# yu-changqian/TorchSeg

Measured on AMD Instinct MI355X. Metric: training images/sec (1024x1024) BiSeNet-R18, higher is better.
Workload: dtype bf16

## Files before the change

include/tsg_hip.h:

```cpp
#ifndef TSG_HIP_H
#define TSG_HIP_H

#include <stddef.h>
#include <stdint.h>

#ifdef __cplusplus
extern "C" {
#endif

#define TSG_VERSION 100

enum { TSG_F32 = 0, TSG_BF16 = 1 };
enum { TSG_NCHW = 0, TSG_NHWC = 1 };
enum { TSG_I64 = 0, TSG_U8 = 1 };

#define TSG_E_DTYPE   (-1)
#define TSG_E_LAYOUT  (-2)
#define TSG_E_SHAPE   (-3)
#define TSG_E_ALIGN   (-4)
#define TSG_E_NULL    (-5)
#define TSG_E_WS      (-6)
#define TSG_E_COMM_LIB   (-7)
#define TSG_E_COMM_BASE  (-100)

int tsg_version(void);


int    tsg_bn_num_partials(int layout, int64_t N, int64_t C, int64_t HW);
size_t tsg_bn_partial_ws_bytes(int layout, int64_t N, int64_t C, int64_t HW);

int tsg_bn_stats(const void* x, int dtype, int layout,
                 int64_t N, int64_t C, int64_t HW,
                 float* partial, int* rows, void* stream);

int tsg_bn_collapse(const float* partial, int S, int64_t C, float* sums,
                    void* stream);
int tsg_bn_collapse_count(const float* partial, int S, int64_t C, float* msg, int64_t count, void* stream);


int tsg_bn_finalize(const float* partial, int S, int64_t C, double count,
                    const float* count_dev, float eps, float momentum,
                    const float* gamma, const float* beta,
                    float* running_mean, float* running_var,
                    int64_t* num_batches_tracked,
                    float* mean, float* invstd, float* fwd_pack, void* stream);

int tsg_bn_affine(const float* mean, const float* invstd, const float* gamma,
                  const float* beta, int64_t C, float* fwd_pack, void* stream);

int tsg_bn_apply_fwd(const void* x, const void* residual, void* y,
                     int dtype, int layout, int64_t N, int64_t C, int64_t HW,
                     const float* fwd_pack, int relu, void* stream);

int tsg_bn_bwd_reduce(const void* dy, const void* x, const void* y,
                      int dtype, int layout, int64_t N, int64_t C, int64_t HW,
                      const float* fwd_pack, int relu,
                      float* partial, int* rows, void* stream);

int tsg_bn_bwd_coeffs(const float* partial, int S, int64_t C, double count,
                      const float* count_dev, int batch_stats,
                      const float* invstd, const float* fwd_pack,
                      float* dgamma, float* dbeta, float* bwd_pack, void* stream);

int tsg_bn_bwd_apply(const void* dy, const void* x, const void* y,
                     void* dx, void* dres,
                     int dtype, int layout, int64_t N, int64_t C, int64_t HW,
                     const float* bwd_pack, int relu, void* stream);

int tsg_bn_maskbits_supported(int dtype, int layout, int64_t C, int64_t HW);
int tsg_bn_apply_fwd_maskbits(const void* x, const void* residual, void* y, void* bits, int dtype, int layout, int64_t N,
                              int64_t C, int64_t HW, const float* fwd_pack, void* stream);
int tsg_bn_bwd_reduce_maskbits(const void* dy, const void* x, const void* bits, int dtype, int layout, int64_t N, int64_t C,
                               int64_t HW, const float* fwd_pack, float* partial, int* rows, void* stream);
int tsg_bn_bwd_apply_maskbits(const void* dy, const void* x, const void* bits, void* dx, void* dres, int dtype, int layout,
                              int64_t N, int64_t C, int64_t HW, const float* bwd_pack, void* stream);

int tsg_bn_mixed_supported(int dtype, int64_t C, int64_t HW);
int tsg_bn_mixed_num_partials(int64_t N, int64_t C, int64_t HW);
int tsg_bn_apply_fwd_mixed(const void* x_nchw, void* y_nhwc, int dtype,
                           int64_t N, int64_t C, int64_t HW,
                           const float* fwd_pack, int relu, void* stream);
int tsg_bn_bwd_reduce_mixed(const void* dy_nhwc, const void* x_nchw, int dtype,
                            int64_t N, int64_t C, int64_t HW,
                            const float* fwd_pack, int relu,
                            float* partial, int* rows, void* stream);
int tsg_bn_bwd_apply_mixed(const void* dy_nhwc, const void* x_nchw, void* dx_nchw,
                           int dtype, int64_t N, int64_t C, int64_t HW,
                           const float* bwd_pack, int relu, void* stream);

size_t tsg_gap_ws_bytes(int layout, int64_t N, int64_t C, int64_t HW);
int tsg_gap_fwd(const void* x, void* out, int dtype, int layout,
                int64_t N, int64_t C, int64_t HW,
                void* ws, size_t ws_bytes, void* stream);
int tsg_gap_bwd(const void* dout, void* dx, int dtype, int layout,
                int64_t N, int64_t C, int64_t HW, void* stream);

size_t tsg_adaptive_avgpool_nhwc_ws_bytes(int dtype, int64_t N, int C, int H, int W, int OH, int OW);
int tsg_adaptive_avgpool_nhwc_fwd(const void* x, void* out, int dtype, int64_t N, int C, int H, int W, int OH, int OW,
                                  void* ws, size_t ws_bytes, void* stream);
int tsg_adaptive_avgpool_nhwc_bwd(const void* dout, void* dx, int dtype, int64_t N, int C, int H, int W, int OH, int OW,
                                  void* stream);

int tsg_cat2_rows(const void* a, const void* b, void* out, int64_t rows, int64_t row_bytes_a, int64_t row_bytes_b,
                  void* stream);

int tsg_chanscale_fwd(const void* x, const void* s, void* y, int dtype, int layout,
                      int64_t N, int64_t C, int64_t HW, int add_identity, void* stream);
int tsg_chanscale_bwd(const void* dy, const void* x, const void* s, void* dx, void* ds,
                      int dtype, int layout, int64_t N, int64_t C, int64_t HW,
                      int add_identity, void* ws, size_t ws_bytes, void* stream);
int tsg_chanscale_bwd_ds(const void* dy, const void* x, void* ds, int dtype, int layout, int64_t N, int64_t C, int64_t HW,
                         void* ws, size_t ws_bytes, void* stream);
int tsg_chanscale_bwd_dx(const void* dy, const void* s, const void* gadd, void* dx, int dtype, int layout, int64_t N, int64_t C,
                         int64_t HW, int add_identity, void* stream);

int tsg_maxpool_nhwc_fwd(const void* x, void* y, void* argmax_u8, int dtype,
                         int64_t N, int C, int IH, int IW, int OH, int OW,
                         int K, int S, int P, void* stream);
int tsg_maxpool_nhwc_bwd(const void* dy, const void* argmax_u8, void* dx, int dtype,
                         int64_t N, int C, int IH, int IW, int OH, int OW,
                         int K, int S, int P, void* stream);

int tsg_stem_conv_supported(int dtype, int Cin, int Cout, int kh, int kw, int stride, int pad,
                            int dilation, int groups, int64_t H, int64_t W);
size_t tsg_stem_conv_ws_bytes(void);
int tsg_stem_conv_fwd(const void* x, const float* w, void* y, int64_t B, int64_t H, int64_t W,
                      void* ws, size_t ws_bytes, void* stream);
int tsg_stem_conv_wrw(const void* x, const void* dy, float* dw, int64_t B, int64_t H, int64_t W,
                      void* ws, size_t ws_bytes, void* stream);
int tsg_stem3_conv_supported(int dtype, int Cin, int Cout, int kh, int kw, int stride, int pad,
                             int dilation, int groups, int64_t H, int64_t W);
size_t tsg_stem3_conv_ws_bytes(void);
int tsg_stem3_conv_fwd(const void* x, const float* w, void* y, int64_t B, int64_t H, int64_t W,
                       void* ws, size_t ws_bytes, void* stream);
int tsg_stem3_conv_wrw(const void* x, const void* dy, float* dw, int64_t B, int64_t H, int64_t W,
                       void* ws, size_t ws_bytes, void* stream);
int tsg_stem_conv_wrw_bn(const void* x, const void* da, const void* xc, const float* bp, float* dw, int64_t B,
                         int64_t H, int64_t W, void* ws, size_t ws_bytes, void* stream);
int tsg_stem_conv_stats_partials(int64_t B, int64_t H, int64_t W);
int tsg_stem_conv_fwd_stats(const void* x, const float* w, void* y, float* partial, int64_t B, int64_t H,
                            int64_t W, void* ws, size_t ws_bytes, void* stream);

int tsg_bn_relu_pool_fwd(const void* x, void* y, void* argmax_u8, int dtype, int64_t N, int C, int IH, int IW,
                         int OH, int OW, const float* fp, void* stream);
int tsg_bn_relu_pool_bwd_num_partials(int dtype, int64_t N, int C, int IH, int IW);
int tsg_bn_relu_pool_bwd_reduce(const void* dpool, const void* argmax_u8, const void* x, int dtype, int64_t N,
                                int C, int IH, int IW, int OH, int OW, const float* fp, float* partial,
                                void* stream);
int tsg_bn_relu_pool_bwd_apply(const void* dpool, const void* argmax_u8, const void* x, void* dx, int dtype,
                               int64_t N, int C, int IH, int IW, int OH, int OW, const float* bp, void* stream);

int tsg_stem_conv_stats(const void* x, const float* w, float* partial, int64_t B, int64_t H, int64_t W, void* ws,
                        size_t ws_bytes, void* stream);
int tsg_stem_conv_bn_relu_pool_fwd(const void* x, const float* w, const float* fp, void* ypool, void* argmax_u8,
                                   int64_t B, int64_t H, int64_t W, void* ws, size_t ws_bytes, void* stream);
int tsg_stem_pool_bwd_num_partials(int64_t B, int64_t H, int64_t W);
int tsg_stem_conv_bn_relu_pool_bwd_reduce(const void* x, const float* w, const void* dpool, const void* argmax_u8,
                                          const float* fp, float* partial, int64_t B, int64_t H, int64_t W, void* ws,
                                          size_t ws_bytes, void* stream);
int tsg_stem_conv_wrw_bn_pool(const void* x, const float* w, const void* xc, const void* dpool, const void* argmax_u8,
                              const float* bp, float* dw, int64_t B, int64_t H, int64_t W, void* ws, size_t ws_bytes,
                              void* stream);

int tsg_conv3x3_wrw_supported(int dtype, int Cin, int Cout, int kh, int kw, int stride, int pad,
                              int dilation, int groups);
size_t tsg_conv3x3_wrw_ws_bytes(void);
int tsg_conv3x3_wrw(const void* x, const void* dy, float* dw, int64_t B, int64_t H, int64_t W,
                    void* ws, size_t ws_bytes, void* stream);
int tsg_conv3x3_wrw_tr(const void* x, const void* dy, float* dw, int64_t B, int64_t H, int64_t W,
                       void* ws, size_t ws_bytes, void* stream);
int tsg_conv3x3_wrw_gen_supported(int dtype, int Cin, int Cout, int kh, int kw, int stride, int pad,
                                  int dilation, int groups);
size_t tsg_conv3x3_wrw_gen_ws_bytes(int64_t B, int64_t Hin, int64_t Win, int Cin, int Cout, int stride);
int tsg_conv3x3_wrw_gen(const void* x, const void* dy, float* dw, int64_t B, int64_t Hin, int64_t Win, int Cin, int Cout,
                        int stride, void* ws, size_t ws_bytes, void* stream);
int tsg_conv3x3_wrw_tr_norm(const void* x, const float* in_ab, const void* dy, float* dw, int64_t B, int64_t H, int64_t W,
                            void* ws, size_t ws_bytes, void* stream);
int tsg_conv3x3_wrw_gen_norm(const void* x, const float* in_ab, const void* dy, float* dw, int64_t B, int64_t Hin,
                             int64_t Win, int Cin, int Cout, int stride, void* ws, size_t ws_bytes, void* stream);

int tsg_conv3x3_c64_supported(int dtype, int Cin, int Cout, int kh, int kw, int stride, int pad, int dilation,
                              int groups);
int tsg_conv3x3_c64_stats_partials(int64_t B, int64_t H, int64_t W);
int tsg_conv3x3_c64_fwd(const void* x, const void* w, void* y, float* partial, const float* in_ab, const void* addend,
                        int64_t B, int64_t H, int64_t W, void* stream);
int tsg_conv3x3_c64_s2_stats_partials(int64_t B, int64_t H, int64_t W);
int tsg_conv3x3_c64_s2_fwd(const void* x, const void* w, void* y, float* partial, const float* in_ab, int64_t B,
                           int64_t H, int64_t W, void* stream);
int tsg_conv3x3_c64_s2_dgrad(const void* dy, const void* wt, void* dx, int64_t B, int64_t H, int64_t W,
                             void* stream);
int tsg_conv3x3_c64_dgrad_bnsums_partials(int64_t B, int64_t H, int64_t W);
int tsg_conv3x3_c64_dgrad_bnsums(const void* dy, const void* wt, void* dx, const void* bn_x, const float* bn_fp,
                                 float* partial, int64_t B, int64_t H, int64_t W, void* stream);
int tsg_conv3x3_c64_s2_dgrad_partials(int64_t B, int64_t H, int64_t W);
int tsg_conv3x3_c64_s2_dgrad_bnsums(const void* dy, const void* wt, void* dx, const void* bn_x, const float* bn_fp,
                                    float* partial, int64_t B, int64_t H, int64_t W, void* stream);

int tsg_conv3x3_weight_rot180_t(const void* w, int dtype, void* out, int O, int I, void* stream);

int tsg_conv3x3_gen_supported(int dtype, int Cin, int Cout, int kh, int kw, int stride, int pad, int dilation,
                              int groups);
int64_t tsg_conv3x3_gen_filter_elems(int Cin, int Cout);
int tsg_conv3x3_gen_tile(int64_t B, int64_t H, int64_t W, int Cin, int Cout);
int tsg_conv3x3_gen_prep_filter(const void* w, int dtype, void* out, int O, int I, int mode, int BN, void* stream);
int tsg_conv3x3_gen_stats_partials(int64_t B, int64_t H, int64_t W, int Cin, int Cout, int BN);
int tsg_conv3x3_gen_variant(int64_t B, int64_t H, int64_t W, int Cin, int Cout, int BN, int with_in_ab);
int tsg_conv3x3_s2_dgrad_supported(int dtype, int Cin, int Cout);
int tsg_conv3x3_s2_dgrad(const void* dy, const void* wf, void* dx, const void* addend, int64_t B, int64_t H, int64_t W,
                         int Cin, int Cout, void* stream);
int tsg_conv3x3_s2_dgrad_subadd(const void* dy, const void* wf, void* dx, const void* addend_sub, int64_t B, int64_t H,
                                int64_t W, int Cin, int Cout, void* stream);
int tsg_conv3x3_gen_fwd(const void* x, const void* wf, void* y, float* partial, const float* in_ab, const void* addend,
                        int64_t B, int64_t H, int64_t W, int Cin, int Cout, int BN, void* stream);

int tsg_conv3x3_dil_supported(int dtype, int Cin, int Cout, int kh, int kw, int stride, int pad, int dilation,
                              int groups);
int tsg_conv3x3_dil_stats_partials(int64_t B, int64_t H, int64_t W, int Cin, int Cout, int dilation);
int tsg_conv3x3_dil_fwd(const void* x, const void* wf, void* y, float* partial, const void* addend, int64_t B, int64_t H,
                        int64_t W, int Cin, int Cout, int dilation, void* stream);
size_t tsg_conv3x3_dil_wrw_ws_bytes(int64_t B, int64_t H, int64_t W, int Cin, int Cout, int dilation);
int tsg_conv3x3_dil_wrw(const void* x, const void* dy, float* dw, int64_t B, int64_t H, int64_t W, int Cin, int Cout,
                        int dilation, void* ws, size_t ws_bytes, void* stream);

int tsg_pw_wgrad_supported(int dtype, int Cin, int Cout, int64_t B, int H, int W, int stride);
int tsg_pw_wgrad_slices(int Cin, int Cout, int64_t B, int H, int W, int stride);
size_t tsg_pw_wgrad_ws_bytes(int Cin, int Cout, int64_t B, int H, int W, int stride);
int tsg_pw_wgrad(const void* x, const void* dy, float* dw, int dtype, int64_t B, int H, int W, int Cin, int Cout,
                 int stride, void* ws, size_t ws_bytes, void* stream);


typedef struct tsg_ohem_plan {
  int64_t P;
  int     C;
  int     grid;
  int     levels;
  int     shift[3];
  int     bins[3];
  uint32_t thresh_bits;
  size_t  ws_bytes;
} tsg_ohem_plan;

int tsg_ohem_make_plan(int64_t B, int C, int64_t HW, float thresh,
                       tsg_ohem_plan* plan);

int tsg_ohem_fwd(const void* logits, int dtype, const void* labels, int ltype,
                 int64_t B, int C, int64_t HW,
                 int64_t ignore_label, float thresh, int64_t min_kept,
                 const float* weight,
                 float* nll, float* lse, float* loss, int32_t* sel,
                 void* ws, size_t ws_bytes, void* stream);

int tsg_ohem_bwd(const void* logits, int dtype, const void* labels, int ltype,
                 int64_t B, int C, int64_t HW, int64_t ignore_label,
                 const float* weight,
                 const float* nll, const float* lse, const int32_t* sel,
                 const float* gscale, void* dlogits, void* ws, void* stream);

int tsg_ohem_up_supported(int C, int IH, int IW, int OH, int OW, float thresh);
size_t tsg_ohem_up_bwd_ws_bytes(int64_t B, int C, int IH, int OW);
int tsg_ohem_up_fwd(const void* z, int dtype, const void* labels, int ltype,
                    int64_t B, int C, int IH, int IW, int OH, int OW,
                    int64_t ignore_label, float thresh, int64_t min_kept,
                    const float* weight,
                    float* nll, float* lse, float* loss, int32_t* sel,
                    void* ws, size_t ws_bytes, void* stream);
int tsg_ohem_up_bwd(const void* z, int dtype, const void* labels, int ltype,
                    int64_t B, int C, int IH, int IW, int OH, int OW,
                    int64_t ignore_label, const float* weight,
                    const float* nll, const float* lse, const int32_t* sel,
                    const float* gscale, void* dz,
                    void* ws, size_t ws_bytes, void* stream);

int tsg_ohem_up_wide_supported(int C, int IH, int IW, int OH, int OW);

int tsg_ohem_target_prob(const float* nll, const void* labels, int ltype, int64_t P, int C,
                         int64_t ignore_label, float* prob, void* stream);

size_t tsg_kth_ws_bytes(int64_t n);
int tsg_kth_value(const float* v, int64_t n, int64_t k, float* out,
                  void* ws, size_t ws_bytes, void* stream);

size_t tsg_focal_ws_bytes(int64_t P);
int tsg_focal_fwd(const void* pred, int dtype, const void* target, int ltype,
                  int64_t P, int64_t ignore_label, float gamma, float alpha,
                  float* loss, void* ws, size_t ws_bytes, void* stream);
int tsg_focal_bwd(const void* pred, int dtype, const void* target, int ltype,
                  int64_t P, int64_t ignore_label, float gamma, float alpha,
                  const float* gscale, void* dpred, void* stream);

int tsg_upsample_bilinear_ac_fwd(const void* x, const void* add, void* y,
                                 int dtype, int64_t NC, int IH, int IW,
                                 int OH, int OW, void* stream);
int tsg_upsample_bilinear_ac_bwd(const void* dy, void* dx, int dtype,
                                 int64_t NC, int IH, int IW, int OH, int OW,
                                 void* stream);
int tsg_upsample_bilinear_ac_nhwc_fwd(const void* x, const void* add, void* y,
                                      int dtype, int64_t N, int C, int IH, int IW,
// ... 173 lines not shown
```

torchseg_amd/convwrw.py:

```python
import collections
import os as _os

import torch
import torch.nn as nn
import torch.nn.functional as F

from . import kernels as K
from . import syncbn as S
from .stemconv import StemConv2d, _as_bf16_image, _wants_bf16, attach_bn_partial, take_bn_partial

_OWN_C64 = _os.environ.get("TSG_CONV_C64", "1") != "0"
_OWN_C64_S1 = _os.environ.get("TSG_CONV_C64_S1", "1") != "0"
_C64_STATS = _os.environ.get("TSG_CONV_C64_STATS", "1") != "0"
_OWN_GEN = _os.environ.get("TSG_CONV_GEN", "1") != "0"
_GEN_STATS = _os.environ.get("TSG_CONV_GEN_STATS", "1") != "0"
_OWN_S2_DGRAD = _os.environ.get("TSG_CONV_S2_DGRAD", "1") != "0"
_DGRAD_MODE = _os.environ.get("TSG_CONV_DGRAD_FWD", "2").strip().lower()
_DGRAD_FWD = _DGRAD_MODE not in ("0", "false", "no", "off", "")
_DGRAD_ANY = _DGRAD_MODE == "2"

_BN_ON_LOAD = _os.environ.get("TSG_BN_ON_LOAD", "1") != "0"
_GEN_BN_ON_LOAD = _os.environ.get("TSG_CONV_GEN_BN_ON_LOAD", "0") == "1"
_STEM_BN_WRW = _os.environ.get("TSG_STEM_BN_WRW", "1") != "0"
_BN_BSUM = _os.environ.get("TSG_BN_BSUM", "0") == "1"
# ... 46 lines not shown
        return False
    return all(a == b for a, b, n in zip(out.stride(), param.stride(), out.shape) if n != 1)


_deferred = {}
_deferred_clear_queued = [False]


def _deferred_clear():
    _deferred_clear_queued[0] = False
    _deferred.clear()


def may_defer(param, buf):
    return (param is not None and param.is_leaf and param.grad is None and param.dtype == torch.float32
            and id(param) not in _wrw_pending and id(param) not in _deferred and not param._backward_hooks
            and not _foreign_grad_hooks(param) and _kept_as_gradient(buf, param))


def note_deferred(param, entry):
    _DEFER.append(entry)
    _deferred[id(param)] = entry
    if not _deferred_clear_queued[0]:
        _deferred_clear_queued[0] = True
        from torch.autograd import Variable
        try:
            Variable._execution_engine.queue_callback(_deferred_clear)
        except RuntimeError:
            _deferred_clear()


def launch_deferred_of(param):
    if param is None or id(param) not in _deferred:
        return False
    entry, _deferred[id(param)] = _deferred[id(param)], None
    if entry is not None:
        if _DEFER is not None:
            _DEFER[:] = [e for e in _DEFER if e is not entry]
        entry[0]()
    return True


def wrw_on_side_stream(fn, param, *operands, defer_out=None):
    if _DEFER is not None and defer_out is not None:
        Cout, Cin = defer_out
        buf = torch.empty((Cout, Cin, 3, 3), dtype=torch.float32, device=operands[0].device, memory_format=torch.channels_last)
        if may_defer(param, buf):
            note_deferred(param, (lambda: fn(out=buf), operands, buf))
            return buf.detach()
        if launch_deferred_of(param):
            return fn()
    if not _WRW_STREAM or not operands[0].is_cuda or param is None or not param.is_leaf or param.grad is not None \
            or param.dtype != torch.float32 or param._backward_hooks or _foreign_grad_hooks(param) \
            or (torch.cuda.is_current_stream_capturing() and not _WRW_IN_GRAPH):
        if _wrw_side and operands[0].is_cuda:
            dev = operands[0].device
            side = _wrw_side.get(dev)
            if side is not None and (param is None or id(param) in _wrw_pending):
                torch.cuda.current_stream(dev).wait_stream(side)
        return fn()
    dev = operands[0].device
    cur = torch.cuda.current_stream(dev)
    if id(param) in _wrw_pending:
        side = _wrw_side.get(dev)
        if side is not None:
            cur.wait_stream(side)
        return fn()
    side = _wrw_side.get(dev)
    if side is None:
        side = _wrw_side[dev] = torch.cuda.Stream(device=dev)
    side.wait_stream(cur)
    with torch.cuda.stream(side):
        out = fn()
    for t in operands:
        if t is not None:
            t.record_stream(side)
    out.record_stream(cur)
    _wrw_pending.add(id(param))
    if not _kept_as_gradient(out, param):
        cur.wait_stream(side)
    if not _wrw_join_queued[0]:
        _wrw_join_queued[0] = True
        from torch.autograd import Variable
        try:
            Variable._execution_engine.queue_callback(_wrw_join)
        except RuntimeError:
            _wrw_join()
    return out


def _conv_wrw(x, dy, stride, param, in_ab=None):
    operands = (x, dy) if in_ab is None else (x, dy, in_ab)
    return wrw_on_side_stream(lambda out=None: K.provider().conv3x3_wrw(x, dy, stride=stride, in_ab=in_ab, out=out), param,
                              *operands, defer_out=(dy.shape[1], x.shape[1]))


def _bf16_nhwc(t):
    if t.dtype != torch.bfloat16:
        t = t.to(torch.bfloat16)
    return t.contiguous(memory_format=torch.channels_last)


def _filters(weight):
    if _SHADOW and weight.is_contiguous(memory_format=torch.channels_last):
        from .shadow import bank
        return bank.get(weight, want_rot=True)
    return weight.detach().to(torch.bfloat16), None


def _rotated(wrt, wb):
    return wrt if wrt is not None else K.provider().conv3x3_weight_rot180_t(wb)


def _with_partial(y, partial):
    if partial.numel():
        attach_bn_partial(y, partial)
    return y


def _skip_addend(dskip, like_shape):
    if dskip is None or tuple(dskip.shape) != tuple(like_shape):
        return None
    return _bf16_nhwc(dskip)


Route = collections.namedtuple("Route", "family stats skip compact bn_on_load dgrad_fwd")


def _route(conv, xb, general=True):
    kp = K.provider()
    stride, geom = conv.stride[0], (conv.padding[0], conv.dilation[0], conv.groups)
    if not kp.conv3x3_wrw_supported(xb, conv.weight, stride, *geom):
        return None
    nhwc = conv.weight.is_contiguous(memory_format=torch.channels_last)
    c64 = _OWN_C64 and kp.conv3x3_c64_supported(xb, conv.weight, stride, *geom)
    if (general and _OWN_GEN and stride == 1 and not (c64 and _OWN_C64_S1) and nhwc
            and kp.conv3x3_gen_supported(xb, conv.weight, 1, *geom)):
        family, stats, skip = "gen", _GEN_STATS, True
    else:
        if c64 and nhwc:
            family = "c64"
        elif _OWN_S2_DGRAD and stride == 2 and nhwc and kp.conv3x3_s2_dgrad_supported(conv.in_channels, conv.out_channels):
            family = "s2"
        else:
            family = "lib"
        stats = _C64_STATS and family == "c64"
        skip = family == "s2" or (c64 and _OWN_C64_S1 and stride == 1)
    return Route(family, bool(stats and conv.training), bool(skip), family == "s2",
                 (family == "c64" and (_OWN_C64_S1 or stride == 2))
                 or (family == "gen" and _GEN_BN_ON_LOAD and conv.in_channels <= 512),
                 family == "lib" and _DGRAD_FWD and stride == 1 and (_DGRAD_ANY or conv.in_channels == conv.out_channels))


class _ConvWrwFn(torch.autograd.Function):

    @staticmethod
    def forward(ctx, x, weight, wb, wrt, stride, route, skip=False):
        kp = K.provider()
        partial = x.new_empty(0, dtype=torch.float32)
        if route.stats:
            y, partial = kp.conv3x3_c64_fwd(x, wb, with_stats=True, stride=stride)
        elif route.family == "c64":
            y = kp.conv3x3_c64_fwd(x, wb, stride=stride)
        else:
            y = F.conv2d(x, wb, None, stride, 1)
        ctx.route, ctx.stride = route, stride
        ctx.wrt = wrt
        ctx.master = weight if (route.family == "s2" and _SHADOW and weight.dtype == torch.float32) else None
        ctx.save_for_backward(x, wb)
        ctx.wparam = weight
        ctx.need_dx = x.requires_grad
        ctx.set_materialize_grads(False)
        ctx.mark_non_differentiable(partial)
        ctx.skip_sub = skip == 2
        if not skip:
            return y, partial
        return y, partial, (x[:, :, ::2, ::2].contiguous(memory_format=torch.channels_last) if ctx.skip_sub else x)

    @staticmethod
    def backward(ctx, dy, _dpartial, dskip=None):
        kp = K.provider()
        x, wb = ctx.saved_tensors
        family, stride = ctx.route.family, ctx.stride
        sub = None
        if dskip is not None and ctx.skip_sub:
            sub, dskip = _bf16_nhwc(dskip), None
        if dy is None:
            if sub is not None:
                dskip = torch.zeros_like(x)
                dskip[:, :, ::2, ::2] = sub
            return dskip, None, None, None, None, None, None
        dy = _bf16_nhwc(dy)
        dx = None
        if ctx.need_dx:
            in_hw = (x.shape[2], x.shape[3])
            add = _skip_addend(dskip, x.shape) if (family == "s2" or (family == "c64" and stride == 1)) else None
            if add is not None:
                dskip = None
            if family == "s2":
                dx = kp.conv3x3_s2_dgrad(dy, wb if ctx.master is None else ctx.master, in_hw, addend=add, addend_sub=sub)
                sub = None
            elif family == "c64" and stride == 2:
                dx = kp.conv3x3_c64_s2_dgrad(dy, _rotated(ctx.wrt, wb), in_hw)
            elif family == "c64":
                dx = kp.conv3x3_c64_fwd(dy, _rotated(ctx.wrt, wb), addend=add)
            elif ctx.route.dgrad_fwd:
                dx = F.conv2d(dy, _rotated(ctx.wrt, wb), None, 1, 1)
            else:
                dx = torch.ops.aten.convolution_backward(dy, x, wb, None, [stride, stride], [1, 1], [1, 1], False, [0, 0], 1,
                                                         [True, False, False])[0]
            if dskip is not None:
                dx = dx + dskip.to(dx.dtype)
            if sub is not None:
                dx[:, :, ::2, ::2] += sub.to(dx.dtype)
        dw = _conv_wrw(x, dy, stride, ctx.wparam)
        return dx, dw.to(ctx.wparam.dtype), None, None, None, None, None


class _ConvGenFn(torch.autograd.Function):

    @staticmethod
    def forward(ctx, x, weight, with_stats, skip=False):
        kp = K.provider()
        wf = kp.conv3x3_gen_prep_filter(weight, 0, x)
        out = kp.conv3x3_gen_fwd(x, wf, weight.shape[0], with_stats=with_stats)
        y, partial = out if with_stats else (out, x.new_empty(0, dtype=torch.float32))
        ctx.save_for_backward(x, weight)
        ctx.need_dx = x.requires_grad
        ctx.mark_non_differentiable(partial)
        ctx.set_materialize_grads(False)
        return (y, partial, x) if skip else (y, partial)

    @staticmethod
    def backward(ctx, dy, _dpartial, dskip=None):
        kp = K.provider()
        x, weight = ctx.saved_tensors
        if dy is None:
            return dskip, None, None, None
        dy = _bf16_nhwc(dy)
        dx = None
        if ctx.need_dx:
            O, I = weight.shape[0], weight.shape[1]
            if O % 16 == 0 and I % 64 == 0:
                add = _skip_addend(dskip, x.shape)
                dx = kp.conv3x3_gen_fwd(dy, kp.conv3x3_gen_prep_filter(weight, 1, dy), I, addend=add)
                if add is not None:
                    dskip = None
            else:
                dx = F.conv2d(dy, kp.conv3x3_weight_rot180_t(weight.detach().to(torch.bfloat16)), None, 1, 1)
            if dskip is not None:
                dx = dx + dskip.to(dx.dtype)
        dw = _conv_wrw(x, dy, 1, weight)
        return dx, dw.to(weight.dtype), None, None


class WrwConv2d(nn.Conv2d):
    def forward(self, x):
        return self._forward(x, False)

    def _forward(self, x, want_skip):
        route = None
        if (x.is_cuda and self.bias is None and self.weight.dtype == torch.float32 and x.dim() == 4
                and self.padding_mode == "zeros" and torch.is_grad_enabled() and self.weight.requires_grad and _wants_bf16(x)):
            xb = _bf16_nhwc(x)
            route = _route(self, xb)
        if route is None:
            y = super().forward(x)
            return (y, None) if want_skip else y
        skip = bool(want_skip and route.skip and xb is x and x.requires_grad)
        with torch.autocast("cuda", enabled=False):
            if route.family == "gen":
                out = _ConvGenFn.apply(xb, self.weight, route.stats, skip)
            else:
                wb, wrt = _filters(self.weight)
                out = _ConvWrwFn.apply(xb, self.weight, wb, wrt, self.stride[0], route,
                                       2 if (skip and want_skip == 2 and route.compact) else skip)
        y = _with_partial(out[0], out[1])
        return (y, out[2] if skip else None) if want_skip else y


def conv_with_skip(conv, x, subsample=False):
    if _FUSE_SKIP and isinstance(conv, WrwConv2d) and conv.stride in ((1, 1), (2, 2)) and isinstance(x, torch.Tensor) \
            and x.is_cuda and torch.is_grad_enabled():
        return conv._forward(x, 2 if (subsample and _SKIP_SUB and conv.stride == (2, 2)) else True)
    return conv(x), None


def _c64_dgrad_and_bn_sums(kp, dy, rot, x, fp, stride, layout, N, C, HW):
    if _BN_BSUM and kp.conv3x3_c64_bnsums_supported(x.shape[0], x.shape[2], x.shape[3], stride):
        if stride == 2:
            da, partial = kp.conv3x3_c64_s2_dgrad(dy, rot, (x.shape[2], x.shape[3]), bsum=(x, fp))
        else:
            da, partial = kp.conv3x3_c64_fwd(dy, rot, bsum=(x, fp))
        return da, partial, partial.shape[0]
    da = kp.conv3x3_c64_s2_dgrad(dy, rot, (x.shape[2], x.shape[3])) if stride == 2 else kp.conv3x3_c64_fwd(dy, rot)
    partial, Sn = kp.bn_bwd_reduce(da, x, None, layout, N, C, HW, fp, True)
    return da, partial, Sn


def _c64_fwd_on_load(kp, x, wb, stride, fp, out_stats):
    if out_stats:
        return kp.conv3x3_c64_fwd(x, wb, with_stats=True, stride=stride, in_ab=fp)
    return kp.conv3x3_c64_fwd(x, wb, stride=stride, in_ab=fp), x.new_empty(0, dtype=torch.float32)


class _BnReluConvFn(torch.autograd.Function):

    @staticmethod
    def forward(ctx, x, gamma, beta, bn, use_batch_stats, group, hint, weight, wb, stride, wrt, gen=False, out_stats=False):
        kp = K.provider()
        layout, N, C, HW = K.bn_layout(x)
        invstd, fp, count_dev, world = S._forward_pack(kp, x, layout, N, C, HW, bn, gamma, beta, use_batch_stats, group, hint)
        if gen:
            out = kp.conv3x3_gen_fwd(x, kp.conv3x3_gen_prep_filter(weight, 0, x), weight.shape[0], with_stats=out_stats,
                                     in_ab=fp)
            y, partial = out if out_stats else (out, x.new_empty(0, dtype=torch.float32))
        else:
            y, partial = _c64_fwd_on_load(kp, x, wb, stride, fp, out_stats)
        ctx.save_for_backward(x, weight if gen else wb, gamma, beta, invstd, fp, count_dev)
        ctx.wparam = weight
        ctx.cfg = (layout, N, C, HW, use_batch_stats, group, world, stride, gen)
        ctx.wrt = wrt
        ctx.mark_non_differentiable(partial)
        return y, partial

    @staticmethod
    def backward(ctx, dy, _dpartial):
        kp = K.provider()
        x, wb, gamma, beta, invstd, fp, count_dev = ctx.saved_tensors
        layout, N, C, HW, use_batch_stats, group, world, stride, gen = ctx.cfg
# ... 105 lines not shown
```

torchseg_amd/csrc/bn.hip:

```cpp
#include "tsg_dispatch.h"

namespace tsg {

constexpr int kThreads = 256;
constexpr int kUnroll = 4;
constexpr int kTargetBlocks = 2048;
constexpr int kTargetBlocksNhwc = 1024;
constexpr int kMaxSplit = 256;

template <typename T, int V> struct Pack;
template <> struct Pack<float, 4> : Vec<float> {};
template <> struct Pack<bf16_t, 8> : Vec<bf16_t> {};
template <typename T> struct Pack<T, 1> {
  float v[1];
  typedef T Raw;
  static __device__ __forceinline__ Raw ldraw(const T* p) { return *p; }
  static __device__ __forceinline__ Raw ldraw_dead(const T* p) { return *p; }
  __device__ __forceinline__ void unpack(const Raw& t) { v[0] = ld1<T>(&t); }
  __device__ __forceinline__ void load(const T* p) { v[0] = ld1<T>(p); }
  __device__ __forceinline__ void store(T* p) const { st1<T>(p, v[0]); }
};

struct NchwGeom {
  int seg;
// ... 113 lines not shown
            a2[j] = fma((AT)pd.v[j], (AT)(px.v[j] - mu), a2[j]);
          }
        }
      }
    }
  }
  AT s1 = 0, s2 = 0;
#pragma unroll
  for (int j = 0; j < V; ++j) { s1 += a1[j]; s2 += a2[j]; }
  block_sum2(s1, s2, sm);
  if (tid == 0) {
    put_partial(partial, C, S, s, 0, c, s1);
    put_partial(partial, C, S, s, 1, c, s2);
  }
}

template <typename T, int V, int MODE, int MASK>
__global__ __launch_bounds__(kThreads) void bn_reduce_nhwc(
    const T* __restrict__ x, const T* __restrict__ dy, const T* __restrict__ y,
    int64_t M, int64_t C, int GT, int R, int64_t rows_per_block,
    const float* __restrict__ fp, float* __restrict__ partial) {
  typedef typename RedAcc<T, MODE>::type AT;
  extern __shared__ __attribute__((aligned(16))) float smem[];
  const int tid = threadIdx.x;
  const int gl = tid % GT, r = tid / GT;
  const int64_t G = C / V;
  const int64_t g = (int64_t)blockIdx.y * GT + gl;
  const bool live = (r < R) && (g < G);
  const int64_t c0 = g * V;
  float mu[V], ca[V], cb[V];
  AT a1[V], a2[V];
#pragma unroll
  for (int j = 0; j < V; ++j) { a1[j] = 0; a2[j] = 0; mu[j] = 0.f; ca[j] = 0.f; cb[j] = 0.f; }
  if (MODE == 1 && live) {
    ldc<V>(fp + 2 * C, c0, mu);
    if (MASK == 2) { ldc<V>(fp, c0, ca); ldc<V>(fp + C, c0, cb); }
  }
  const int64_t row0 = (int64_t)blockIdx.x * rows_per_block;
  int64_t row1 = row0 + rows_per_block;
  if (row1 > M) row1 = M;
  if (live) {
    typedef typename Pack<T, V>::Raw Raw;
    auto accumulate = [&](const Raw& rx, const Raw& rd, const Raw& ry, unsigned int mb) {
      Pack<T, V> px;
      px.unpack(rx);
      if (MODE == 0) {
#pragma unroll
        for (int j = 0; j < V; ++j) { const AT xv = px.v[j]; a1[j] += xv; a2[j] = fma(xv, xv, a2[j]); }
      } else {
        Pack<T, V> pd;
        pd.unpack(rd);
        if (MASK == 1) {
          Pack<T, V> py;
          py.unpack(ry);
#pragma unroll
          for (int j = 0; j < V; ++j) pd.v[j] = py.v[j] > 0.f ? pd.v[j] : 0.f;
        } else if (MASK == 2) {
#pragma unroll
          for (int j = 0; j < V; ++j) pd.v[j] = fmaf(px.v[j], ca[j], cb[j]) > 0.f ? pd.v[j] : 0.f;
        } else if (MASK == 3) {
#pragma unroll
          for (int j = 0; j < V; ++j) pd.v[j] = ((mb >> j) & 1u) ? pd.v[j] : 0.f;
        }
#pragma unroll
        for (int j = 0; j < V; ++j) {
          a1[j] += (AT)pd.v[j];
          a2[j] = fma((AT)pd.v[j], (AT)(px.v[j] - mu[j]), a2[j]);
        }
      }
    };
    const unsigned char* bits = reinterpret_cast<const unsigned char*>(y);
    int64_t row = row0 + r;
    for (; row + (int64_t)(kUnroll - 1) * R < row1; row += (int64_t)kUnroll * R) {
      Raw rx[kUnroll], rd[kUnroll], ry[kUnroll];
      unsigned int rb[kUnroll];
#pragma unroll
      for (int k = 0; k < kUnroll; ++k) {
        const int64_t off = (row + (int64_t)k * R) * C + c0;
        rx[k] = Pack<T, V>::ldraw(x + off);
        if (MODE == 1) rd[k] = Pack<T, V>::ldraw(dy + off);
        if (MODE == 1 && MASK == 1) ry[k] = Pack<T, V>::ldraw(y + off);
        rb[k] = (MODE == 1 && MASK == 3) ? bits[off / V] : 0u;
      }
#pragma unroll
      for (int k = 0; k < kUnroll; ++k) accumulate(rx[k], rd[k], ry[k], rb[k]);
    }
    for (; row < row1; row += R) {
      const int64_t off = row * C + c0;
      Raw rx = Pack<T, V>::ldraw(x + off), rd = rx, ry = rx;
      if (MODE == 1) rd = Pack<T, V>::ldraw(dy + off);
      if (MODE == 1 && MASK == 1) ry = Pack<T, V>::ldraw(y + off);
      accumulate(rx, rd, ry, (MODE == 1 && MASK == 3) ? bits[off / V] : 0u);
    }
  }
  const int W = GT * V;
  AT* s1 = reinterpret_cast<AT*>(smem);
  AT* s2 = s1 + (size_t)R * W;
  if (r < R) {
#pragma unroll
    for (int j = 0; j < V; ++j) {
      s1[r * W + gl * V + j] = a1[j];
      s2[r * W + gl * V + j] = a2[j];
    }
  }
  __syncthreads();
  for (int t = tid; t < W; t += kThreads) {
    const int64_t c = (int64_t)blockIdx.y * W + t;
    if (c < C) {
      AT t1 = 0, t2 = 0;
      for (int q = 0; q < R; ++q) { t1 += s1[q * W + t]; t2 += s2[q * W + t]; }
      put_partial(partial, C, (int)gridDim.x, (int)blockIdx.x, 0, c, t1);
      put_partial(partial, C, (int)gridDim.x, (int)blockIdx.x, 1, c, t2);
    }
  }
}

static int bn_reverse() {
  static int v = -1;
  if (v < 0) { const char* e = getenv("TSG_BN_REVERSE"); v = e ? (e[0] != '0') : 0; }
  return v;
}

template <typename T, int V, bool RELU, bool RES>
__global__ __launch_bounds__(kThreads) void bn_fwd_nchw(
    const T* __restrict__ x, const T* __restrict__ res, T* __restrict__ y,
    int64_t C, int64_t HW, int seg, int segs, const float* __restrict__ fp) {
  const int64_t bid = blockIdx.x;
  const int64_t plane = bid / segs;
  const int sg = (int)(bid - plane * segs);
  const int64_t c = plane % C;
  const float a = fp[c], b = fp[C + c];
  const int64_t off = plane * HW + (int64_t)sg * seg;
  const int64_t rem = HW - (int64_t)sg * seg;
  const int len = rem < seg ? (int)rem : seg;
#pragma unroll
  for (int k = 0; k < kUnroll; ++k) {
    const int i = (k * kThreads + threadIdx.x) * V;
    if (i < len) {
      Pack<T, V> px, pr;
      px.load(x + off + i);
      if (RES) pr.load(res + off + i);
#pragma unroll
      for (int j = 0; j < V; ++j) {
        float t = fmaf(px.v[j], a, b);
        if (RES) t += pr.v[j];
        if (RELU) t = t > 0.f ? t : 0.f;
        px.v[j] = t;
      }
      px.store(y + off + i);
    }
  }
}

template <typename T, int V, bool RELU, bool RES, bool BITS = false>
__global__ __launch_bounds__(kThreads) void bn_fwd_nhwc(
    const T* __restrict__ x, const T* __restrict__ res, T* __restrict__ y,
    int64_t M, int64_t C, int GT, int R, int64_t rows_per_block, const float* __restrict__ fp, int rev,
    unsigned char* __restrict__ bits = nullptr) {
  const int tid = threadIdx.x;
  const int gl = tid % GT, r = tid / GT;
  const int64_t g = (int64_t)blockIdx.y * GT + gl;
  if (r >= R || g >= C / V) return;
  const int64_t c0 = g * V;
  float a[V], b[V];
  ldc<V>(fp, c0, a);
  ldc<V>(fp + C, c0, b);
  const int64_t row0 = (int64_t)(rev ? gridDim.x - 1 - blockIdx.x : blockIdx.x) * rows_per_block;
  int64_t row1 = row0 + rows_per_block;
  if (row1 > M) row1 = M;
  typedef typename Pack<T, V>::Raw Raw;
  auto finish = [&](const Raw& rx, const Raw& rr_, int64_t off) {
    Pack<T, V> px, pr;
    px.unpack(rx);
    if (RES) pr.unpack(rr_);
#pragma unroll
    for (int j = 0; j < V; ++j) {
      float t = fmaf(px.v[j], a[j], b[j]);
      if (RES) t += pr.v[j];
      if (RELU) t = t > 0.f ? t : 0.f;
      px.v[j] = t;
    }
    px.store(y + off);
    if (BITS) {
      unsigned int mb = 0u;
#pragma unroll
      for (int j = 0; j < V; ++j) {
        const float q = sizeof(T) == 2 ? __uint_as_float((uint32_t)f32_to_bf16(px.v[j]) << 16) : px.v[j];
        mb |= (q > 0.f ? 1u : 0u) << j;
      }
      bits[off / V] = (unsigned char)mb;
    }
  };
  int64_t row = row0 + r;
  for (; row + (int64_t)(kUnroll - 1) * R < row1; row += (int64_t)kUnroll * R) {
    Raw rx[kUnroll], rs[kUnroll];
#pragma unroll
    for (int k = 0; k < kUnroll; ++k) {
      const int64_t off = (row + (int64_t)k * R) * C + c0;
      rx[k] = Pack<T, V>::ldraw_dead(x + off);
      if (RES) rs[k] = Pack<T, V>::ldraw(res + off);
    }
#pragma unroll
    for (int k = 0; k < kUnroll; ++k) finish(rx[k], rs[k], (row + (int64_t)k * R) * C + c0);
  }
  for (; row < row1; row += R) {
    const int64_t off = row * C + c0;
    Raw rx = Pack<T, V>::ldraw_dead(x + off), rs = rx;
    if (RES) rs = Pack<T, V>::ldraw(res + off);
    finish(rx, rs, off);
  }
}

template <typename T, int V, int MASK, bool DRES>
__global__ __launch_bounds__(kThreads) void bn_bwd_nchw(
    const T* __restrict__ dy, const T* __restrict__ x, const T* __restrict__ y,
    T* __restrict__ dx, T* __restrict__ dres,
    int64_t C, int64_t HW, int seg, int segs, const float* __restrict__ bp) {
  const int64_t bid = blockIdx.x;
  const int64_t plane = bid / segs;
  const int sg = (int)(bid - plane * segs);
  const int64_t c = plane % C;
  const float a = bp[c], b = bp[C + c], mu = bp[2 * C + c], bc = bp[3 * C + c], c2 = bp[4 * C + c];
  const int64_t off = plane * HW + (int64_t)sg * seg;
  const int64_t rem = HW - (int64_t)sg * seg;
  const int len = rem < seg ? (int)rem : seg;
#pragma unroll
  for (int k = 0; k < kUnroll; ++k) {
    const int i = (k * kThreads + threadIdx.x) * V;
    if (i < len) {
      Pack<T, V> pd, px;
      pd.load(dy + off + i);
      px.load(x + off + i);
      if (MASK == 1) {
        Pack<T, V> py;
        py.load(y + off + i);
#pragma unroll
        for (int j = 0; j < V; ++j) pd.v[j] = py.v[j] > 0.f ? pd.v[j] : 0.f;
      } else if (MASK == 2) {
#pragma unroll
        for (int j = 0; j < V; ++j) pd.v[j] = fmaf(px.v[j], a, b) > 0.f ? pd.v[j] : 0.f;
      }
      if (DRES) pd.store(dres + off + i);
#pragma unroll
      for (int j = 0; j < V; ++j) px.v[j] = fmaf(a, pd.v[j], fmaf(bc, px.v[j] - mu, c2));
      px.store(dx + off + i);
    }
  }
}

template <typename T, int V, int MASK, bool DRES>
__global__ __launch_bounds__(kThreads) void bn_bwd_nhwc(
    const T* __restrict__ dy, const T* __restrict__ x, const T* __restrict__ y,
    T* __restrict__ dx, T* __restrict__ dres,
    int64_t M, int64_t C, int GT, int R, int64_t rows_per_block, const float* __restrict__ bp, int rev) {
  const int tid = threadIdx.x;
  const int gl = tid % GT, r = tid / GT;
  const int64_t g = (int64_t)blockIdx.y * GT + gl;
  if (r >= R || g >= C / V) return;
  const int64_t c0 = g * V;
  float a[V], b[V], mu[V], bc[V], c2[V];
#pragma unroll
  for (int j = 0; j < V; ++j) b[j] = 0.f;
  ldc<V>(bp, c0, a);
  if (MASK == 2) ldc<V>(bp + C, c0, b);
  ldc<V>(bp + 2 * C, c0, mu);
  ldc<V>(bp + 3 * C, c0, bc);
  ldc<V>(bp + 4 * C, c0, c2);
  const int64_t row0 = (int64_t)(rev ? gridDim.x - 1 - blockIdx.x : blockIdx.x) * rows_per_block;
  int64_t row1 = row0 + rows_per_block;
  if (row1 > M) row1 = M;
  typedef typename Pack<T, V>::Raw Raw;
  auto finish = [&](const Raw& rd, const Raw& rx, const Raw& ry, unsigned int mb, int64_t off) {
    Pack<T, V> pd, px;
    pd.unpack(rd);
    px.unpack(rx);
    if (MASK == 1) {
      Pack<T, V> py;
      py.unpack(ry);
#pragma unroll
      for (int j = 0; j < V; ++j) pd.v[j] = py.v[j] > 0.f ? pd.v[j] : 0.f;
    } else if (MASK == 2) {
#pragma unroll
      for (int j = 0; j < V; ++j) pd.v[j] = fmaf(px.v[j], a[j], b[j]) > 0.f ? pd.v[j] : 0.f;
    } else if (MASK == 3) {
#pragma unroll
      for (int j = 0; j < V; ++j) pd.v[j] = ((mb >> j) & 1u) ? pd.v[j] : 0.f;
    }
    if (DRES) pd.store(dres + off);
#pragma unroll
    for (int j = 0; j < V; ++j) px.v[j] = fmaf(a[j], pd.v[j], fmaf(bc[j], px.v[j] - mu[j], c2[j]));
    px.store(dx + off);
  };
  const unsigned char* bits = reinterpret_cast<const unsigned char*>(y);
  int64_t row = row0 + r;
  for (; row + (int64_t)(kUnroll - 1) * R < row1; row += (int64_t)kUnroll * R) {
    Raw rd[kUnroll], rx[kUnroll], ry[kUnroll];
    unsigned int rb[kUnroll];
#pragma unroll
    for (int k = 0; k < kUnroll; ++k) {
      const int64_t off = (row + (int64_t)k * R) * C + c0;
      rd[k] = Pack<T, V>::ldraw_dead(dy + off);
      rx[k] = Pack<T, V>::ldraw_dead(x + off);
      if (MASK == 1) ry[k] = Pack<T, V>::ldraw(y + off);
      rb[k] = MASK == 3 ? bits[off / V] : 0u;
    }
#pragma unroll
    for (int k = 0; k < kUnroll; ++k) finish(rd[k], rx[k], ry[k], rb[k], (row + (int64_t)k * R) * C + c0);
  }
  for (; row < row1; row += R) {
    const int64_t off = row * C + c0;
    Raw rd = Pack<T, V>::ldraw_dead(dy + off), rx = Pack<T, V>::ldraw_dead(x + off), ry = rx;
    if (MASK == 1) ry = Pack<T, V>::ldraw(y + off);
    finish(rd, rx, ry, MASK == 3 ? bits[off / V] : 0u, off);
  }
}

constexpr int kTP = 64;

template <typename T, bool RELU>
__global__ __launch_bounds__(kThreads) void bn_fwd_mixed(
    const T* __restrict__ x, T* __restrict__ y, int64_t C, int64_t HW, int tiles_per_img,
    const float* __restrict__ fp) {
  constexpr int V = Pack<T, (sizeof(T) == 2 ? 8 : 4)>::N;
  extern __shared__ __attribute__((aligned(16))) float tile[];
  const int ldt = (int)C + 1;
  const int64_t n = blockIdx.x / tiles_per_img;
  const int64_t p0 = (int64_t)(blockIdx.x % tiles_per_img) * kTP;
  const int npx = (HW - p0) < kTP ? (int)(HW - p0) : kTP;
  const int tid = threadIdx.x;
  const int vpr = kTP / V;
  for (int it = tid; it < (int)C * vpr; it += kThreads) {
    const int c = it / vpr, v = it - c * vpr;
    const int p = v * V;
    if (p < npx) {
      Pack<T, V> px;
// ... 158 lines not shown
  if (owner) {
#pragma unroll
    for (int q = 0; q < 8; ++q) { t1 += sh[0][q * 8][tc]; t2 += sh[1][q * 8][tc]; }
  }
}

__device__ __forceinline__ double bn_count(double count, const float* cd) {
  return cd ? (double)cd[0] * 4096.0 + (double)cd[1] : count;
}

__global__ __launch_bounds__(kTc * kTs) void bn_collapse_k(const float* __restrict__ partial, int S,
                                                          int64_t C, float* __restrict__ sums, int with_count,
                                                          float count_hi, float count_lo) {
  if (with_count && blockIdx.x == 0 && threadIdx.x == 0) {
    sums[2 * C] = count_hi;
    sums[2 * C + 1] = count_lo;
  }
  double t1, t2; bool owner; int64_t c;
  tail_sums(partial, S, C, t1, t2, owner, c);
  if (!owner) return;
  sums[c] = (float)t1;
  sums[C + c] = (float)t2;
}

__global__ __launch_bounds__(kTc * kTs) void bn_finalize_k(
    const float* __restrict__ partial, int S, int64_t C, double count,
    const float* __restrict__ count_dev, float eps, float momentum,
    const float* __restrict__ gamma, const float* __restrict__ beta,
    float* __restrict__ rmean, float* __restrict__ rvar, int64_t* __restrict__ nbt,
    float* __restrict__ mean, float* __restrict__ invstd, float* __restrict__ fp) {
  if (blockIdx.x == 0 && threadIdx.x == 0 && nbt) *nbt += 1;
  double t1, t2; bool owner; int64_t c;
  tail_sums(partial, S, C, t1, t2, owner, c);
  if (!owner) return;
  count = bn_count(count, count_dev);
  const double m = t1 / count;
  double sumvar = t2 - t1 * m;
  if (sumvar < 0.0) sumvar = 0.0;
  const double bias_var = sumvar / count;
  const float mf = (float)m;
  const float isf = (float)(1.0 / sqrt(bias_var + (double)eps));
  mean[c] = mf;
  invstd[c] = isf;
  const float a = (gamma ? gamma[c] : 1.f) * isf;
  fp[c] = a;
  fp[C + c] = fmaf(-mf, a, beta ? beta[c] : 0.f);
  fp[2 * C + c] = mf;
  if (rmean) rmean[c] = (float)((1.0 - (double)momentum) * (double)rmean[c] + (double)momentum * m);
  if (rvar) {
    const double unbias = sumvar / (count - 1.0);
    rvar[c] = (float)((1.0 - (double)momentum) * (double)rvar[c] + (double)momentum * unbias);
  }
}

__global__ void bn_affine_k(const float* __restrict__ mean, const float* __restrict__ invstd,
                            const float* __restrict__ gamma, const float* __restrict__ beta, int64_t C,
                            float* __restrict__ fp) {
  const int64_t c = (int64_t)blockIdx.x * blockDim.x + threadIdx.x;
  if (c >= C) return;
  const float a = (gamma ? gamma[c] : 1.f) * invstd[c];
  fp[c] = a;
  fp[C + c] = fmaf(-mean[c], a, beta ? beta[c] : 0.f);
  fp[2 * C + c] = mean[c];
}

__global__ __launch_bounds__(kTc * kTs) void bn_bwd_coeffs_k(
    const float* __restrict__ partial, int S, int64_t C, double count,
    const float* __restrict__ count_dev, int batch_stats, const float* __restrict__ invstd,
    const float* __restrict__ fp, float* __restrict__ dgamma, float* __restrict__ dbeta,
    float* __restrict__ bp) {
  double t1, t2; bool owner; int64_t c;
  tail_sums(partial, S, C, t1, t2, owner, c);
  if (!owner) return;
  const double is = (double)invstd[c];
  if (dbeta) dbeta[c] = (float)t1;
  if (dgamma) dgamma[c] = (float)(t2 * is);
  if (bp) {
    const float a = fp[c];
    float bc = 0.f, c2 = 0.f;
    if (batch_stats) {
      count = bn_count(count, count_dev);
      const double k0 = t1 / count, k1 = t2 * is / count;
      bc = (float)(-(double)a * k1 * is);
      c2 = (float)(-(double)a * k0);
    }
    bp[c] = a;
    bp[C + c] = fp[C + c];
    bp[2 * C + c] = fp[2 * C + c];
    bp[3 * C + c] = bc;
    bp[4 * C + c] = c2;
  }
}

template <typename T, int V, int MODE>
static int launch_reduce(const T* x, const T* dy, const T* y, int layout, int64_t N,
                         int64_t C, int64_t HW, const float* fp, int mask,
                         float* partial, hipStream_t st) {
  return with_int<0, 1, 2>(MODE == 0 ? 0 : mask, [&](auto mk) {
    if (layout == TSG_NCHW) {
      NchwGeom g = nchw_geom(N, C, HW, V);
      dim3 grid((unsigned)C, (unsigned)g.split);
      hipLaunchKernelGGL((bn_reduce_nchw<T, V, MODE, mk()>), grid, dim3(kThreads), 0, st, x, dy, y, N, C, HW, g.seg, g.segs,
                         g.split, fp, partial);
    } else {
      const int64_t M = N * HW;
      NhwcGeom g = nhwc_geom(M, C, V);
      dim3 grid((unsigned)g.split, (unsigned)g.ytiles);
      const size_t sh = (size_t)2 * g.rows_per_iter * g.gt * V * sizeof(typename RedAcc<T, MODE>::type);
      hipLaunchKernelGGL((bn_reduce_nhwc<T, V, MODE, mk()>), grid, dim3(kThreads), sh, st, x, dy, y, M, C, g.gt,
                         g.rows_per_iter, g.rows_per_block, fp, partial);
    }
    TSG_CHECK_LAUNCH();
    return 0;
  });
}

template <typename T, int V>
static int launch_fwd(const T* x, const T* res, T* y, int layout, int64_t N, int64_t C,
                      int64_t HW, const float* fp, int relu, hipStream_t st) {
  return with_flag(relu != 0, [&](auto r) { return with_flag(res != nullptr, [&](auto s) {
    if (layout == TSG_NCHW) {
      NchwGeom g = nchw_geom(N, C, HW, V);
      const int64_t blocks = N * C * g.segs;
      if (blocks > 0x7fffffffLL) return TSG_E_SHAPE;
      hipLaunchKernelGGL((bn_fwd_nchw<T, V, r(), s()>), dim3((unsigned)blocks), dim3(kThreads), 0, st, x, res, y, C, HW,
                         g.seg, g.segs, fp);
    } else {
      const int64_t M = N * HW;
      NhwcGeom g = nhwc_geom(M, C, V);
      dim3 grid((unsigned)g.split, (unsigned)g.ytiles);
      hipLaunchKernelGGL((bn_fwd_nhwc<T, V, r(), s()>), grid, dim3(kThreads), 0, st, x, res, y, M, C, g.gt, g.rows_per_iter,
                         g.rows_per_block, fp, bn_reverse());
    }
    TSG_CHECK_LAUNCH();
    return 0;
  }); });
}

template <typename T, int V>
static int launch_fwd_bits(const T* x, const T* res, T* y, unsigned char* bits, int64_t N, int64_t C, int64_t HW,
                           const float* fp, hipStream_t st) {
  const int64_t M = N * HW;
  NhwcGeom g = nhwc_geom(M, C, V);
  dim3 grid((unsigned)g.split, (unsigned)g.ytiles);
  return with_flag(res != nullptr, [&](auto s) {
    hipLaunchKernelGGL((bn_fwd_nhwc<T, V, true, s(), true>), grid, dim3(kThreads), 0, st, x, res, y, M, C, g.gt,
                       g.rows_per_iter, g.rows_per_block, fp, bn_reverse(), bits);
    TSG_CHECK_LAUNCH();
    return 0;
  });
}

template <typename T, int V>
static int launch_reduce_bits(const T* x, const T* dy, const unsigned char* bits, int64_t N, int64_t C, int64_t HW,
                              const float* fp, float* partial, hipStream_t st) {
  const int64_t M = N * HW;
  NhwcGeom g = nhwc_geom(M, C, V);
  dim3 grid((unsigned)g.split, (unsigned)g.ytiles);
  const size_t sh = (size_t)2 * g.rows_per_iter * g.gt * V * sizeof(typename RedAcc<T, 1>::type);
  hipLaunchKernelGGL((bn_reduce_nhwc<T, V, 1, 3>), grid, dim3(kThreads), sh, st, x, dy, reinterpret_cast<const T*>(bits), M, C,
                     g.gt, g.rows_per_iter, g.rows_per_block, fp, partial);
  TSG_CHECK_LAUNCH();
  return 0;
}

template <typename T, int V>
static int launch_bwd_bits(const T* dy, const T* x, const unsigned char* bits, T* dx, T* dres, int64_t N, int64_t C,
                           int64_t HW, const float* bp, hipStream_t st) {
  const int64_t M = N * HW;
  NhwcGeom g = nhwc_geom(M, C, V);
  dim3 grid((unsigned)g.split, (unsigned)g.ytiles);
  return with_flag(dres != nullptr, [&](auto d) {
    hipLaunchKernelGGL((bn_bwd_nhwc<T, V, 3, d()>), grid, dim3(kThreads), 0, st, dy, x, reinterpret_cast<const T*>(bits), dx,
                       dres, M, C, g.gt, g.rows_per_iter, g.rows_per_block, bp, bn_reverse());
    TSG_CHECK_LAUNCH();
    return 0;
  });
}

template <typename T, int V>
static int launch_bwd(const T* dy, const T* x, const T* y, T* dx, T* dres, int layout,
                      int64_t N, int64_t C, int64_t HW, const float* bp, int mask, hipStream_t st) {
  return with_int<0, 1, 2>(mask, [&](auto mk) { return with_flag(dres != nullptr, [&](auto d) {
    if (layout == TSG_NCHW) {
      NchwGeom g = nchw_geom(N, C, HW, V);
      const int64_t blocks = N * C * g.segs;
      if (blocks > 0x7fffffffLL) return TSG_E_SHAPE;
      hipLaunchKernelGGL((bn_bwd_nchw<T, V, mk(), d()>), dim3((unsigned)blocks), dim3(kThreads), 0, st, dy, x, y, dx, dres, C,
                         HW, g.seg, g.segs, bp);
    } else {
      const int64_t M = N * HW;
      NhwcGeom g = nhwc_geom(M, C, V);
      dim3 grid((unsigned)g.split, (unsigned)g.ytiles);
      hipLaunchKernelGGL((bn_bwd_nhwc<T, V, mk(), d()>), grid, dim3(kThreads), 0, st, dy, x, y, dx, dres, M, C, g.gt,
                         g.rows_per_iter, g.rows_per_block, bp, bn_reverse());
    }
    TSG_CHECK_LAUNCH();
    return 0;
  }); });
}

static int check_dims(int dtype, int layout, int64_t N, int64_t C, int64_t HW) {
  if (dtype != TSG_F32 && dtype != TSG_BF16) return TSG_E_DTYPE;
  if (layout != TSG_NCHW && layout != TSG_NHWC) return TSG_E_LAYOUT;
  if (N <= 0 || C <= 0 || HW <= 0) return TSG_E_SHAPE;
  return 0;
}

static int partial_rows(int layout, int64_t N, int64_t C, int64_t HW, int V) {
  return layout == TSG_NCHW ? nchw_geom(N, C, HW, V).split : nhwc_geom(N * HW, C, V).split;
}

static int bn_reduce_dispatch(int mode, const void* x, const void* dy, const void* y,
                              int dtype, int layout, int64_t N, int64_t C, int64_t HW,
                              const float* fp, int mask, float* partial, void* stream, int* rows) {
  int e = check_dims(dtype, layout, N, C, HW);
  if (e) return e;
  if (!x || !partial) return TSG_E_NULL;
  hipStream_t st = (hipStream_t)stream;
  const int V = pick_vec(dtype, layout, C, HW, x, dy, mask == 1 ? y : nullptr, nullptr, nullptr);
  *rows = partial_rows(layout, N, C, HW, V) * (dtype == TSG_F32 ? 2 : 1);
  return with_elem_vec(dtype, V != 1, [&](auto t, auto v) {
    typedef typename decltype(t)::type T;
    return mode == 0 ? launch_reduce<T, v(), 0>((const T*)x, nullptr, nullptr, layout, N, C, HW, fp, 0, partial, st)
                     : launch_reduce<T, v(), 1>((const T*)x, (const T*)dy, (const T*)y, layout, N, C, HW, fp, mask, partial, st);
  });
}

}

using namespace tsg;

extern "C" {

int tsg_bn_num_partials(int layout, int64_t N, int64_t C, int64_t HW) {
  if (N <= 0 || C <= 0 || HW <= 0) return TSG_E_SHAPE;
  if (layout != TSG_NCHW && layout != TSG_NHWC) return TSG_E_LAYOUT;
  int best = 1;
  const int vs[3] = {1, 4, 8};
  for (int i = 0; i < 3; ++i) {
    const int V = vs[i];
    if (layout == TSG_NHWC && C % V) continue;
    const int s = partial_rows(layout, N, C, HW, V);
    if (s > best) best = s;
  }
  return 2 * best;
}

size_t tsg_bn_partial_ws_bytes(int layout, int64_t N, int64_t C, int64_t HW) {
  const int s = tsg_bn_num_partials(layout, N, C, HW);
  if (s < 0) return 0;
  return (size_t)s * 2 * (size_t)C * sizeof(float);
}

int tsg_bn_stats(const void* x, int dtype, int layout, int64_t N, int64_t C, int64_t HW,
                 float* partial, int* rows, void* stream) {
  int r = 0;
  int e = bn_reduce_dispatch(0, x, nullptr, nullptr, dtype, layout, N, C, HW, nullptr, 0, partial,
                             stream, &r);
  if (rows) *rows = r;
  return e;
}

int tsg_bn_collapse(const float* partial, int S, int64_t C, float* sums, void* stream) {
  if (!partial || !sums) return TSG_E_NULL;
  if (S <= 0 || C <= 0) return TSG_E_SHAPE;
  hipLaunchKernelGGL(bn_collapse_k, dim3(ceil_div_i(C, kTc)), dim3(kTc * kTs), 0, (hipStream_t)stream,
                     partial, S, C, sums, 0, 0.f, 0.f);
  TSG_CHECK_LAUNCH();
  return 0;
}

int tsg_bn_collapse_count(const float* partial, int S, int64_t C, float* msg, int64_t count, void* stream) {
  if (!partial || !msg) return TSG_E_NULL;
  if (S <= 0 || C <= 0 || count < 0) return TSG_E_SHAPE;
  hipLaunchKernelGGL(bn_collapse_k, dim3(ceil_div_i(C, kTc)), dim3(kTc * kTs), 0, (hipStream_t)stream,
                     partial, S, C, msg, 1, (float)(count / 4096), (float)(count % 4096));
  TSG_CHECK_LAUNCH();
  return 0;
}

int tsg_bn_finalize(const float* partial, int S, int64_t C, double count, const float* count_dev,
                    float eps, float momentum, const float* gamma, const float* beta,
                    float* running_mean, float* running_var, int64_t* num_batches_tracked,
                    float* mean, float* invstd, float* fwd_pack, void* stream) {
  if (!partial || !mean || !invstd || !fwd_pack) return TSG_E_NULL;
  if (S <= 0 || C <= 0 || (!count_dev && !(count > 0.0))) return TSG_E_SHAPE;
  hipLaunchKernelGGL(bn_finalize_k, dim3(ceil_div_i(C, kTc)), dim3(kTc * kTs), 0, (hipStream_t)stream,
                     partial, S, C, count, count_dev, eps, momentum, gamma, beta, running_mean,
                     running_var, num_batches_tracked, mean, invstd, fwd_pack);
  TSG_CHECK_LAUNCH();
  return 0;
}

int tsg_bn_affine(const float* mean, const float* invstd, const float* gamma, const float* beta,
                  int64_t C, float* fwd_pack, void* stream) {
  if (!mean || !invstd || !fwd_pack) return TSG_E_NULL;
  if (C <= 0) return TSG_E_SHAPE;
  hipLaunchKernelGGL(bn_affine_k, dim3(ceil_div_i(C, 128)), dim3(128), 0, (hipStream_t)stream, mean,
                     invstd, gamma, beta, C, fwd_pack);
  TSG_CHECK_LAUNCH();
  return 0;
}

int tsg_bn_apply_fwd(const void* x, const void* residual, void* y, int dtype, int layout,
                     int64_t N, int64_t C, int64_t HW, const float* fwd_pack, int relu,
                     void* stream) {
  int e = check_dims(dtype, layout, N, C, HW);
  if (e) return e;
  if (!x || !y || !fwd_pack) return TSG_E_NULL;
  if (!aligned16(fwd_pack)) return TSG_E_ALIGN;
  hipStream_t st = (hipStream_t)stream;
  const int V = pick_vec(dtype, layout, C, HW, x, residual, y, nullptr, nullptr);
  return with_elem_vec(dtype, V != 1, [&](auto t, auto v) {
    typedef typename decltype(t)::type T;
    return launch_fwd<T, v()>((const T*)x, (const T*)residual, (T*)y, layout, N, C, HW, fwd_pack, relu, st);
  });
}

int tsg_bn_bwd_reduce(const void* dy, const void* x, const void* y, int dtype, int layout,
                      int64_t N, int64_t C, int64_t HW, const float* fwd_pack, int relu,
                      float* partial, int* rows, void* stream) {
  if (!dy || !fwd_pack) return TSG_E_NULL;
  if (!aligned16(fwd_pack)) return TSG_E_ALIGN;
  const int mask = relu ? (y ? 1 : 2) : 0;
  int r = 0;
  int e = bn_reduce_dispatch(1, x, dy, y, dtype, layout, N, C, HW, fwd_pack, mask, partial, stream, &r);
  if (rows) *rows = r;
  return e;
}

int tsg_bn_bwd_coeffs(const float* partial, int S, int64_t C, double count, const float* count_dev,
                      int batch_stats, const float* invstd, const float* fwd_pack, float* dgamma,
                      float* dbeta, float* bwd_pack, void* stream) {
  if (!partial || !invstd || (bwd_pack && !fwd_pack)) return TSG_E_NULL;
  if (S <= 0 || C <= 0 || (bwd_pack && batch_stats && !count_dev && !(count > 0.0))) return TSG_E_SHAPE;
  hipLaunchKernelGGL(bn_bwd_coeffs_k, dim3(ceil_div_i(C, kTc)), dim3(kTc * kTs), 0, (hipStream_t)stream,
                     partial, S, C, count, count_dev, batch_stats, invstd, fwd_pack, dgamma, dbeta, bwd_pack);
  TSG_CHECK_LAUNCH();
  return 0;
}

int tsg_bn_bwd_apply(const void* dy, const void* x, const void* y, void* dx, void* dres,
                     int dtype, int layout, int64_t N, int64_t C, int64_t HW,
                     const float* bwd_pack, int relu, void* stream) {
  int e = check_dims(dtype, layout, N, C, HW);
  if (e) return e;
  if (!dy || !x || !dx || !bwd_pack) return TSG_E_NULL;
  if (!aligned16(bwd_pack)) return TSG_E_ALIGN;
  hipStream_t st = (hipStream_t)stream;
  const int mask = relu ? (y ? 1 : 2) : 0;
  const int V = pick_vec(dtype, layout, C, HW, x, dy, mask == 1 ? y : nullptr, dx, dres);
  return with_elem_vec(dtype, V != 1, [&](auto t, auto v) {
    typedef typename decltype(t)::type T;
    return launch_bwd<T, v()>((const T*)dy, (const T*)x, (const T*)y, (T*)dx, (T*)dres, layout, N, C, HW, bwd_pack, mask, st);
  });
}

static int bits_vec(int dtype, int layout, int64_t C, int64_t HW, const void* a, const void* b, const void* c, const void* d,
                    const void* e) {
  if (layout != TSG_NHWC) return 0;
  const int want = dtype == TSG_BF16 ? 8 : dtype == TSG_F32 ? 4 : 0;
  if (!want || C % want) return 0;
  return pick_vec(dtype, layout, C, HW, a, b, c, d, e) == want ? want : 0;
}

int tsg_bn_maskbits_supported(int dtype, int layout, int64_t C, int64_t HW) {
  return bits_vec(dtype, layout, C, HW, nullptr, nullptr, nullptr, nullptr, nullptr) != 0;
}

int tsg_bn_apply_fwd_maskbits(const void* x, const void* residual, void* y, void* bits, int dtype, int layout, int64_t N,
                              int64_t C, int64_t HW, const float* fwd_pack, void* stream) {
  int e = check_dims(dtype, layout, N, C, HW);
  if (e) return e;
  if (!x || !y || !bits || !fwd_pack) return TSG_E_NULL;
  if (!aligned16(fwd_pack)) return TSG_E_ALIGN;
  const int V = bits_vec(dtype, layout, C, HW, x, residual, y, nullptr, nullptr);
  if (!V) return layout != TSG_NHWC ? TSG_E_LAYOUT : TSG_E_ALIGN;
  hipStream_t st = (hipStream_t)stream;
  if (dtype == TSG_F32)
    return launch_fwd_bits<float, 4>((const float*)x, (const float*)residual, (float*)y, (unsigned char*)bits, N, C, HW, fwd_pack, st);
  return launch_fwd_bits<bf16_t, 8>((const bf16_t*)x, (const bf16_t*)residual, (bf16_t*)y, (unsigned char*)bits, N, C, HW, fwd_pack, st);
}

int tsg_bn_bwd_reduce_maskbits(const void* dy, const void* x, const void* bits, int dtype, int layout, int64_t N, int64_t C,
                               int64_t HW, const float* fwd_pack, float* partial, int* rows, void* stream) {
  int e = check_dims(dtype, layout, N, C, HW);
  if (e) return e;
  if (!dy || !x || !bits || !fwd_pack || !partial) return TSG_E_NULL;
  if (!aligned16(fwd_pack)) return TSG_E_ALIGN;
  const int V = bits_vec(dtype, layout, C, HW, x, dy, nullptr, nullptr, nullptr);
  if (!V) return layout != TSG_NHWC ? TSG_E_LAYOUT : TSG_E_ALIGN;
  if (rows) *rows = partial_rows(layout, N, C, HW, V) * (dtype == TSG_F32 ? 2 : 1);
  hipStream_t st = (hipStream_t)stream;
  if (dtype == TSG_F32)
    return launch_reduce_bits<float, 4>((const float*)x, (const float*)dy, (const unsigned char*)bits, N, C, HW, fwd_pack, partial, st);
  return launch_reduce_bits<bf16_t, 8>((const bf16_t*)x, (const bf16_t*)dy, (const unsigned char*)bits, N, C, HW, fwd_pack, partial, st);
}

int tsg_bn_bwd_apply_maskbits(const void* dy, const void* x, const void* bits, void* dx, void* dres, int dtype, int layout,
                              int64_t N, int64_t C, int64_t HW, const float* bwd_pack, void* stream) {
  int e = check_dims(dtype, layout, N, C, HW);
  if (e) return e;
  if (!dy || !x || !bits || !dx || !bwd_pack) return TSG_E_NULL;
  if (!aligned16(bwd_pack)) return TSG_E_ALIGN;
  const int V = bits_vec(dtype, layout, C, HW, x, dy, nullptr, dx, dres);
  if (!V) return layout != TSG_NHWC ? TSG_E_LAYOUT : TSG_E_ALIGN;
  hipStream_t st = (hipStream_t)stream;
  if (dtype == TSG_F32)
    return launch_bwd_bits<float, 4>((const float*)dy, (const float*)x, (const unsigned char*)bits, (float*)dx, (float*)dres, N, C, HW, bwd_pack, st);
  return launch_bwd_bits<bf16_t, 8>((const bf16_t*)dy, (const bf16_t*)x, (const unsigned char*)bits, (bf16_t*)dx, (bf16_t*)dres, N, C, HW, bwd_pack, st);
}

static int mixed_ok(int dtype, int64_t C, int64_t HW) {
  const int V = native_vec(dtype);
  return (dtype == TSG_F32 || dtype == TSG_BF16) && C % 8 == 0 && C <= 128 && HW % V == 0;
}

int tsg_bn_mixed_supported(int dtype, int64_t C, int64_t HW) { return mixed_ok(dtype, C, HW); }

static int mixed_blocks(int64_t N, int64_t HW) {
  int64_t t = N * ((HW + kTP - 1) / kTP);
  if (t > kTargetBlocksNhwc) t = kTargetBlocksNhwc;
  return (int)(t < 1 ? 1 : t);
}

int tsg_bn_mixed_num_partials(int64_t N, int64_t C, int64_t HW) {
  if (N <= 0 || C <= 0 || HW <= 0) return TSG_E_SHAPE;
  return mixed_blocks(N, HW);
}

int tsg_bn_apply_fwd_mixed(const void* x_nchw, void* y_nhwc, int dtype, int64_t N, int64_t C,
                           int64_t HW, const float* fwd_pack, int relu, void* stream) {
  if (!x_nchw || !y_nhwc || !fwd_pack) return TSG_E_NULL;
  if (N <= 0 || !mixed_ok(dtype, C, HW)) return TSG_E_SHAPE;
  if (!aligned16(x_nchw) || !aligned16(y_nhwc)) return TSG_E_ALIGN;
  const int tpi = (int)((HW + kTP - 1) / kTP);
  const size_t sh = (size_t)kTP * (C + 1) * sizeof(float);
  dim3 grid((unsigned)(N * tpi));
  hipStream_t st = (hipStream_t)stream;
  return with_elem(dtype, [&](auto t) { return with_flag(relu != 0, [&](auto r) {
    typedef typename decltype(t)::type T;
    hipLaunchKernelGGL((bn_fwd_mixed<T, r()>), grid, dim3(kThreads), sh, st, (const T*)x_nchw, (T*)y_nhwc, C, HW, tpi, fwd_pack);
    TSG_CHECK_LAUNCH();
    return 0;
  }); });
}

int tsg_bn_bwd_reduce_mixed(const void* dy_nhwc, const void* x_nchw, int dtype, int64_t N, int64_t C,
                            int64_t HW, const float* fwd_pack, int relu, float* partial, int* rows,
                            void* stream) {
  if (!dy_nhwc || !x_nchw || !fwd_pack || !partial) return TSG_E_NULL;
  if (N <= 0 || !mixed_ok(dtype, C, HW)) return TSG_E_SHAPE;
  if (!aligned16(x_nchw) || !aligned16(dy_nhwc)) return TSG_E_ALIGN;
  const int tpi = (int)((HW + kTP - 1) / kTP);
  const int64_t total = N * tpi;
  const int V = native_vec(dtype);
  size_t sh = (size_t)kTP * (C + 1) * sizeof(float);
  const size_t red = (size_t)2 * C * (kTP / V) * sizeof(float);
  if (red > sh) sh = red;
  const int blocks = mixed_blocks(N, HW);
  if (rows) *rows = blocks;
  hipStream_t st = (hipStream_t)stream;
  const int items = (int)((C * (kTP / V) + kThreads - 1) / kThreads);
  const int ipt = items <= 1 ? 1 : items <= 2 ? 2 : items <= 4 ? 4 : 8;
  return with_elem(dtype, [&](auto t) { return with_flag(relu != 0, [&](auto r) { return with_int<1, 2, 4, 8>(ipt, [&](auto i) {
    typedef typename decltype(t)::type T;
    hipLaunchKernelGGL((bn_bwd_reduce_mixed<T, r(), i()>), dim3(blocks), dim3(kThreads), sh, st, (const T*)dy_nhwc,
                       (const T*)x_nchw, C, HW, tpi, total, fwd_pack, partial);
    TSG_CHECK_LAUNCH();
    return 0;
  }); }); });
}

int tsg_bn_bwd_apply_mixed(const void* dy_nhwc, const void* x_nchw, void* dx_nchw, int dtype, int64_t N,
                           int64_t C, int64_t HW, const float* bwd_pack, int relu, void* stream) {
  if (!dy_nhwc || !x_nchw || !dx_nchw || !bwd_pack) return TSG_E_NULL;
  if (N <= 0 || !mixed_ok(dtype, C, HW)) return TSG_E_SHAPE;
  if (!aligned16(x_nchw) || !aligned16(dy_nhwc) || !aligned16(dx_nchw)) return TSG_E_ALIGN;
  const int tpi = (int)((HW + kTP - 1) / kTP);
  const size_t sh = (size_t)kTP * (C + 1) * sizeof(float);
  dim3 grid((unsigned)(N * tpi));
  hipStream_t st = (hipStream_t)stream;
  return with_elem(dtype, [&](auto t) { return with_flag(relu != 0, [&](auto r) {
    typedef typename decltype(t)::type T;
    hipLaunchKernelGGL((bn_bwd_apply_mixed<T, r()>), grid, dim3(kThreads), sh, st, (const T*)dy_nhwc, (const T*)x_nchw,
                       (T*)dx_nchw, C, HW, tpi, bwd_pack);
    TSG_CHECK_LAUNCH();
    return 0;
  }); });
}

}
```

torchseg_amd/csrc/bnpool.hip:

```cpp
#include "tsg_dispatch.h"

namespace tsg {

constexpr int kBpT = 256;

template <typename T> __device__ __forceinline__ float round_as(float v);
template <> __device__ __forceinline__ float round_as<float>(float v) { return v; }
template <> __device__ __forceinline__ float round_as<bf16_t>(float v) { return bf16_to_f32(f32_to_bf16(v)); }

struct BpMap { int GT, PW; };
static BpMap bp_map(int C, int V) {
  BpMap m;
  const int G = C / V;
  m.GT = G < kBpT ? G : kBpT;
  m.PW = kBpT / m.GT;
  return m;
}
constexpr int kFwdRows = 8;
constexpr int kAppRows = 8;

template <typename T>
__device__ __forceinline__ void pool_row(const T* __restrict__ xn, int iy, int IH, int x0, int IW, int C,
                                         const float (&a)[Vec<T>::N], const float (&b)[Vec<T>::N],
                                         float (&rm)[Vec<T>::N], int (&rk)[Vec<T>::N]) {
  constexpr int V = Vec<T>::N;
  const bool row_ok = iy >= 0 && iy < IH;
  const int iyc = iy < 0 ? 0 : (iy >= IH ? IH - 1 : iy);
  const T* row = xn + (int64_t)iyc * IW * C;
  Vec<T> p[3];
  bool ok[3];
#pragma unroll
  for (int kx = 0; kx < 3; ++kx) {
    const int ix = x0 + kx;
    ok[kx] = row_ok && ix >= 0 && ix < IW;
    const int ixc = ix < 0 ? 0 : (ix >= IW ? IW - 1 : ix);
    p[kx].load(row + (int64_t)ixc * C);
  }
#pragma unroll
  for (int j = 0; j < V; ++j) { rm[j] = -1.f; rk[j] = 0; }
#pragma unroll
  for (int kx = 0; kx < 3; ++kx) {
#pragma unroll
    for (int j = 0; j < V; ++j) {
      float v = fmaxf(fmaf(p[kx].v[j], a[j], b[j]), 0.f);
      v = ok[kx] ? v : -1.f;
      if (v > rm[j]) { rm[j] = v; rk[j] = kx; }
    }
  }
}

template <typename T>
__global__ __launch_bounds__(kBpT) void bn_relu_pool_fwd_k(const T* __restrict__ x, T* __restrict__ y,
                                                           uint8_t* __restrict__ idx, int C, int IH, int IW,
                                                           int OH, int OW, int GT, int PW, int ytiles,
                                                           const float* __restrict__ fp) {
  constexpr int V = Vec<T>::N;
  const int tid = threadIdx.x;
  const int gl = tid % GT, pl = tid / GT;
  const int g = (blockIdx.y % ytiles) * GT + gl;
  const int ox = blockIdx.x * PW + pl;
  if (pl >= PW || g * V >= C || ox >= OW) return;
  const int oy0 = (blockIdx.y / ytiles) * kFwdRows;
  const int oy1 = oy0 + kFwdRows < OH ? oy0 + kFwdRows : OH;
  const int64_t n = blockIdx.z;
  float a[V], b[V];
  ldc<V>(fp, g * V, a);
  ldc<V>(fp + C, g * V, b);
  const int x0 = 2 * ox - 1;
  const T* xn = x + n * IH * (int64_t)IW * C + g * V;
  float m0[V], m1[V], m2[V];
  int k0[V], k1[V], k2[V];
  pool_row<T>(xn, 2 * oy0 - 1, IH, x0, IW, C, a, b, m0, k0);
  for (int oy = oy0; oy < oy1; ++oy) {
    pool_row<T>(xn, 2 * oy, IH, x0, IW, C, a, b, m1, k1);
    pool_row<T>(xn, 2 * oy + 1, IH, x0, IW, C, a, b, m2, k2);
    Vec<T> ov;
    uint32_t w[2] = {0u, 0u};
#pragma unroll
    for (int j = 0; j < V; ++j) {
      float m = m0[j];
      int am = k0[j];
      if (m1[j] > m) { m = m1[j]; am = 3 + k1[j]; }
      if (m2[j] > m) { m = m2[j]; am = 6 + k2[j]; }
      ov.v[j] = m;
      w[j >> 2] |= (uint32_t)am << (8 * (j & 3));
      m0[j] = m2[j]; k0[j] = k2[j];
    }
    const int64_t o = ((n * OH + oy) * (int64_t)OW + ox) * C + g * V;
    ov.store(y + o);
    if (V == 8) *reinterpret_cast<uint2*>(idx + o) = make_uint2(w[0], w[1]);
    else *reinterpret_cast<uint32_t*>(idx + o) = w[0];
  }
}

template <typename T> struct PoolWin {
  float d[Vec<T>::N];
  uint32_t w[2];
  __device__ __forceinline__ void load(const T* __restrict__ dpn, const uint8_t* __restrict__ idn, int oy, int ox,
                                       int OH, int OW, int C) {
    constexpr int V = Vec<T>::N;
    const bool ok = oy < OH && ox < OW;
    const int64_t o = ((int64_t)(oy < OH ? oy : OH - 1) * OW + (ox < OW ? ox : OW - 1)) * C;
    Vec<T> v;
    v.load(dpn + o);
#pragma unroll
    for (int j = 0; j < V; ++j) d[j] = v.v[j];
    if (V == 8) {
      const uint2 u = *reinterpret_cast<const uint2*>(idn + o);
      w[0] = ok ? u.x : 0xffffffffu; w[1] = ok ? u.y : 0xffffffffu;
    } else {
      const uint32_t u = *reinterpret_cast<const uint32_t*>(idn + o);
      w[0] = ok ? u : 0xffffffffu; w[1] = 0xffffffffu;
    }
  }
};

template <typename T>
__device__ __forceinline__ void block_grads(const PoolWin<T>& w00, const PoolWin<T>& w01, const PoolWin<T>& w10,
                                            const PoolWin<T>& w11, float (&g00)[Vec<T>::N], float (&g01)[Vec<T>::N],
                                            float (&g10)[Vec<T>::N], float (&g11)[Vec<T>::N]) {
  constexpr int V = Vec<T>::N;
#pragma unroll
  for (int j = 0; j < V; ++j) {
    const int sh = 8 * (j & 3);
    const uint32_t b00 = (w00.w[j >> 2] >> sh) & 0xffu, b01 = (w01.w[j >> 2] >> sh) & 0xffu;
    const uint32_t b10 = (w10.w[j >> 2] >> sh) & 0xffu, b11 = (w11.w[j >> 2] >> sh) & 0xffu;
    g00[j] = b00 == 4u ? w00.d[j] : 0.f;
    g01[j] = (b00 == 5u ? w00.d[j] : 0.f) + (b01 == 3u ? w01.d[j] : 0.f);
    g10[j] = (b00 == 7u ? w00.d[j] : 0.f) + (b10 == 1u ? w10.d[j] : 0.f);
    g11[j] = ((b00 == 8u ? w00.d[j] : 0.f) + (b01 == 6u ? w01.d[j] : 0.f)) +
             ((b10 == 2u ? w10.d[j] : 0.f) + (b11 == 0u ? w11.d[j] : 0.f));
  }
}

static int bp_red_rows(int64_t N, int KH, int KW, int PW, int ytiles) {
  const int64_t xseg = (KW + PW - 1) / PW;
  int64_t chunks = 2048 / (N * xseg * ytiles);
  if (chunks < 1) chunks = 1;
  if (chunks > KH) chunks = KH;
  return (int)((KH + chunks - 1) / chunks);
}

template <typename T>
__global__ __launch_bounds__(kBpT) void bn_relu_pool_bwd_reduce_k(
    const T* __restrict__ dpool, const uint8_t* __restrict__ idx, const T* __restrict__ x, int C, int IH,
    int IW, int OH, int OW, int GT, int PW, int ytiles, int rows, const float* __restrict__ fp,
    float* __restrict__ partial) {
  constexpr int V = Vec<T>::N;
  extern __shared__ __attribute__((aligned(16))) float smem[];
  const int tid = threadIdx.x;
  const int gl = tid % GT, pl = tid / GT;
  const int yt = blockIdx.y % ytiles;
  const int g = yt * GT + gl;
  const int m = blockIdx.x * PW + pl;
  const int KH = (IH + 1) >> 1;
  const bool live = pl < PW && g * V < C && 2 * m < IW;
  const int k0 = (blockIdx.y / ytiles) * rows;
  const int k1 = k0 + rows < KH ? k0 + rows : KH;
  const int64_t n = blockIdx.z;
  float a[V], b[V], mu[V], a1[V], a2[V];
#pragma unroll
  for (int j = 0; j < V; ++j) { a1[j] = 0.f; a2[j] = 0.f; a[j] = 0.f; b[j] = 0.f; mu[j] = 0.f; }
  if (live) {
    ldc<V>(fp, g * V, a); ldc<V>(fp + C, g * V, b); ldc<V>(fp + 2 * C, g * V, mu);
    const T* xn = x + n * IH * (int64_t)IW * C + g * V;
    const T* dpn = dpool + n * OH * (int64_t)OW * C + g * V;
    const uint8_t* idn = idx + n * OH * (int64_t)OW * C + g * V;
    const bool col1 = 2 * m + 1 < IW;
    PoolWin<T> w00, w01, w10, w11;
    w10.load(dpn, idn, k0, m, OH, OW, C);
    w11.load(dpn, idn, k0, m + 1, OH, OW, C);
    for (int k = k0; k < k1; ++k) {
      w00 = w10; w01 = w11;
      w10.load(dpn, idn, k + 1, m, OH, OW, C);
      w11.load(dpn, idn, k + 1, m + 1, OH, OW, C);
      Vec<T> px[4];
      bool ok[4];
#pragma unroll
      for (int q = 0; q < 4; ++q) {
        const int iy = 2 * k + (q >> 1);
        ok[q] = iy < IH && (!(q & 1) || col1);
        px[q].load(xn + ((int64_t)(ok[q] ? iy : 2 * k) * IW + (ok[q] ? 2 * m + (q & 1) : 2 * m)) * C);
      }
      float gr[4][V];
      block_grads<T>(w00, w01, w10, w11, gr[0], gr[1], gr[2], gr[3]);
#pragma unroll
      for (int q = 0; q < 4; ++q) {
#pragma unroll
        for (int j = 0; j < V; ++j) {
          const float dv = (ok[q] && fmaf(px[q].v[j], a[j], b[j]) > 0.f) ? gr[q][j] : 0.f;
          a1[j] += dv;
          a2[j] = fmaf(dv, px[q].v[j] - mu[j], a2[j]);
        }
      }
    }
  }
  const int W = GT * V;
  float* s1 = smem;
  float* s2 = smem + (size_t)PW * W;
  if (pl < PW) {
#pragma unroll
    for (int j = 0; j < V; ++j) { s1[pl * W + gl * V + j] = a1[j]; s2[pl * W + gl * V + j] = a2[j]; }
  }
  __syncthreads();
  const int64_t prow = ((int64_t)blockIdx.z * (gridDim.y / ytiles) + blockIdx.y / ytiles) * gridDim.x + blockIdx.x;
  for (int t = tid; t < W; t += kBpT) {
    const int c = yt * W + t;
    if (c < C) {
      float t1 = 0.f, t2 = 0.f;
      for (int q = 0; q < PW; ++q) { t1 += s1[q * W + t]; t2 += s2[q * W + t]; }
      partial[(prow * 2 + 0) * C + c] = t1;
      partial[(prow * 2 + 1) * C + c] = t2;
    }
  }
}

template <typename T>
__global__ __launch_bounds__(kBpT) void bn_relu_pool_bwd_apply_k(
    const T* __restrict__ dpool, const uint8_t* __restrict__ idx, const T* __restrict__ x, T* __restrict__ dx,
    int C, int IH, int IW, int OH, int OW, int GT, int PW, int ytiles, const float* __restrict__ bp) {
  constexpr int V = Vec<T>::N;
  const int tid = threadIdx.x;
  const int gl = tid % GT, pl = tid / GT;
  const int g = (blockIdx.y % ytiles) * GT + gl;
  const int m = blockIdx.x * PW + pl;
  if (pl >= PW || g * V >= C || 2 * m >= IW) return;
  const int KH = (IH + 1) >> 1;
  const int k0 = (blockIdx.y / ytiles) * kAppRows;
  const int k1 = k0 + kAppRows < KH ? k0 + kAppRows : KH;
  const int64_t n = blockIdx.z;
  float a[V], b[V], mu[V], bc[V], c2[V];
  ldc<V>(bp, g * V, a);
  ldc<V>(bp + C, g * V, b);
  ldc<V>(bp + 2 * C, g * V, mu);
  ldc<V>(bp + 3 * C, g * V, bc);
  ldc<V>(bp + 4 * C, g * V, c2);
  const T* xn = x + n * IH * (int64_t)IW * C + g * V;
  T* dxn = dx + n * IH * (int64_t)IW * C + g * V;
  const T* dpn = dpool + n * OH * (int64_t)OW * C + g * V;
  const uint8_t* idn = idx + n * OH * (int64_t)OW * C + g * V;
  const bool col1 = 2 * m + 1 < IW;
  PoolWin<T> w00, w01, w10, w11;
  w10.load(dpn, idn, k0, m, OH, OW, C);
  w11.load(dpn, idn, k0, m + 1, OH, OW, C);
  for (int k = k0; k < k1; ++k) {
    w00 = w10; w01 = w11;
    w10.load(dpn, idn, k + 1, m, OH, OW, C);
    w11.load(dpn, idn, k + 1, m + 1, OH, OW, C);
    Vec<T> px[4];
    bool ok[4];
    int64_t off[4];
#pragma unroll
    for (int q = 0; q < 4; ++q) {
      const int iy = 2 * k + (q >> 1);
      ok[q] = iy < IH && (!(q & 1) || col1);
      off[q] = ((int64_t)(ok[q] ? iy : 2 * k) * IW + (ok[q] ? 2 * m + (q & 1) : 2 * m)) * C;
      px[q].load(xn + off[q]);
    }
    float gr[4][V];
    block_grads<T>(w00, w01, w10, w11, gr[0], gr[1], gr[2], gr[3]);
#pragma unroll
    for (int q = 0; q < 4; ++q) {
#pragma unroll
      for (int j = 0; j < V; ++j) {
        const float dv = fmaf(px[q].v[j], a[j], b[j]) > 0.f ? gr[q][j] : 0.f;
        px[q].v[j] = fmaf(a[j], dv, fmaf(bc[j], px[q].v[j] - mu[j], c2[j]));
      }
      if (ok[q]) px[q].store(dxn + off[q]);
    }
  }
}

static int bp_check(int dtype, int64_t N, int C, int IH, int IW, int OH, int OW) {
  if (dtype != TSG_F32 && dtype != TSG_BF16) return TSG_E_DTYPE;
  const int V = native_vec(dtype);
  if (N <= 0 || C <= 0 || C % V || IH <= 0 || IW <= 0) return TSG_E_SHAPE;
  if (OH != (IH - 1) / 2 + 1 || OW != (IW - 1) / 2 + 1) return TSG_E_SHAPE;
  return 0;
}

}

using namespace tsg;

extern "C" {

int tsg_bn_relu_pool_fwd(const void* x, void* y, void* argmax_u8, int dtype, int64_t N, int C, int IH, int IW,
                         int OH, int OW, const float* fp, void* stream) {
  if (!x || !y || !argmax_u8 || !fp) return TSG_E_NULL;
  int e = bp_check(dtype, N, C, IH, IW, OH, OW);
  if (e) return e;
  if (!aligned16(x) || !aligned16(y) || !aligned16(fp) || (((uintptr_t)argmax_u8) & 7u)) return TSG_E_ALIGN;
  hipStream_t st = (hipStream_t)stream;
  const int V = native_vec(dtype);
  const BpMap m = bp_map(C, V);
  const int ytiles = (C / V + m.GT - 1) / m.GT;
  const int64_t gy = (int64_t)((OH + kFwdRows - 1) / kFwdRows) * ytiles;
  if (gy > 65535 || N > 65535) return TSG_E_SHAPE;
  dim3 grid((unsigned)((OW + m.PW - 1) / m.PW), (unsigned)gy, (unsigned)N);
  return with_elem(dtype, [&](auto t) {
    typedef typename decltype(t)::type T;
    hipLaunchKernelGGL((bn_relu_pool_fwd_k<T>), grid, dim3(kBpT), 0, st, (const T*)x, (T*)y, (uint8_t*)argmax_u8, C, IH, IW, OH,
                       OW, m.GT, m.PW, ytiles, fp);
    TSG_CHECK_LAUNCH();
    return 0;
  });
}

struct BpRed { BpMap m; int ytiles, rows, chunks; int64_t S; };
static BpRed bp_red(int64_t N, int C, int IH, int IW, int V) {
  BpRed r;
  r.m = bp_map(C, V);
  r.ytiles = (C / V + r.m.GT - 1) / r.m.GT;
  const int KH = (IH + 1) / 2, KW = (IW + 1) / 2;
  r.rows = bp_red_rows(N, KH, KW, r.m.PW, r.ytiles);
  r.chunks = (KH + r.rows - 1) / r.rows;
  r.S = N * r.chunks * (int64_t)((KW + r.m.PW - 1) / r.m.PW);
  return r;
}

int tsg_bn_relu_pool_bwd_num_partials(int dtype, int64_t N, int C, int IH, int IW) {
  if (dtype != TSG_F32 && dtype != TSG_BF16) return TSG_E_DTYPE;
  const int V = native_vec(dtype);
  if (N <= 0 || C <= 0 || C % V || IH <= 0 || IW <= 0) return TSG_E_SHAPE;
  const BpRed r = bp_red(N, C, IH, IW, V);
  if (r.S > 0x7fffffffLL) return TSG_E_SHAPE;
  return (int)r.S;
}

int tsg_bn_relu_pool_bwd_reduce(const void* dpool, const void* argmax_u8, const void* x, int dtype, int64_t N, int C,
                                int IH, int IW, int OH, int OW, const float* fp, float* partial, void* stream) {
  if (!dpool || !argmax_u8 || !x || !fp || !partial) return TSG_E_NULL;
  int e = bp_check(dtype, N, C, IH, IW, OH, OW);
  if (e) return e;
  if (!aligned16(x) || !aligned16(dpool) || !aligned16(fp) || (((uintptr_t)argmax_u8) & 7u)) return TSG_E_ALIGN;
  hipStream_t st = (hipStream_t)stream;
  const int V = native_vec(dtype);
  const BpRed r = bp_red(N, C, IH, IW, V);
  const int64_t gy = (int64_t)r.chunks * r.ytiles;
  if (gy > 65535 || N > 65535) return TSG_E_SHAPE;
  dim3 grid((unsigned)(((IW + 1) / 2 + r.m.PW - 1) / r.m.PW), (unsigned)gy, (unsigned)N);
  const size_t sh = (size_t)2 * r.m.PW * r.m.GT * V * sizeof(float);
  return with_elem(dtype, [&](auto t) {
    typedef typename decltype(t)::type T;
    hipLaunchKernelGGL((bn_relu_pool_bwd_reduce_k<T>), grid, dim3(kBpT), sh, st, (const T*)dpool, (const uint8_t*)argmax_u8,
                       (const T*)x, C, IH, IW, OH, OW, r.m.GT, r.m.PW, r.ytiles, r.rows, fp, partial);
    TSG_CHECK_LAUNCH();
    return 0;
  });
}

int tsg_bn_relu_pool_bwd_apply(const void* dpool, const void* argmax_u8, const void* x, void* dx, int dtype, int64_t N,
                               int C, int IH, int IW, int OH, int OW, const float* bp, void* stream) {
  if (!dpool || !argmax_u8 || !x || !dx || !bp) return TSG_E_NULL;
  int e = bp_check(dtype, N, C, IH, IW, OH, OW);
  if (e) return e;
  if (!aligned16(x) || !aligned16(dx) || !aligned16(dpool) || !aligned16(bp) || (((uintptr_t)argmax_u8) & 7u))
    return TSG_E_ALIGN;
  hipStream_t st = (hipStream_t)stream;
  const int V = native_vec(dtype);
  const BpMap m = bp_map(C, V);
  const int ytiles = (C / V + m.GT - 1) / m.GT;
  const int64_t gy = (int64_t)(((IH + 1) / 2 + kAppRows - 1) / kAppRows) * ytiles;
  if (gy > 65535 || N > 65535) return TSG_E_SHAPE;
  dim3 grid((unsigned)(((IW + 1) / 2 + m.PW - 1) / m.PW), (unsigned)gy, (unsigned)N);
  return with_elem(dtype, [&](auto t) {
    typedef typename decltype(t)::type T;
    hipLaunchKernelGGL((bn_relu_pool_bwd_apply_k<T>), grid, dim3(kBpT), 0, st, (const T*)dpool, (const uint8_t*)argmax_u8,
                       (const T*)x, (T*)dx, C, IH, IW, OH, OW, m.GT, m.PW, ytiles, bp);
    TSG_CHECK_LAUNCH();
    return 0;
  });
}

}
```

torchseg_amd/furnace/base_model/resnet.py:

```python
import torch.nn as nn

from seg_opr.seg_oprs import norm_act
from torchseg_amd.fusion import outside_mode as _outside_mode
from torchseg_amd.pool import MaxPool2d as _MaxPool2d
from utils.pyt_utils import load_model

__all__ = ['ResNet', 'resnet18', 'resnet34', 'resnet50', 'resnet101', 'resnet152']


def _shortcut(inplanes, outplanes, stride, norm_layer, bn_eps, bn_momentum):
    return nn.Sequential(nn.Conv2d(inplanes, outplanes, kernel_size=1, stride=stride, bias=False),
                         norm_layer(outplanes, eps=bn_eps, momentum=bn_momentum))


class _Block(nn.Module):
    def _identity(self, x):
        if self.downsample is None:
            return x
        conv, bn = self.downsample[0], self.downsample[1]
        return norm_act(bn, None, conv(x))


class BasicBlock(_Block):
    expansion = 1

    def __init__(self, inplanes, planes, stride=1, norm_layer=None, bn_eps=1e-5, bn_momentum=0.1,
                 downsample=None, inplace=True):
        super(BasicBlock, self).__init__()
        self.conv1 = nn.Conv2d(inplanes, planes, kernel_size=3, stride=stride, padding=1, bias=False)
        self.bn1 = norm_layer(planes, eps=bn_eps, momentum=bn_momentum)
        self.relu = nn.ReLU(inplace=inplace)
        self.relu_inplace = nn.ReLU(inplace=True)
        self.conv2 = nn.Conv2d(planes, planes, kernel_size=3, stride=1, padding=1, bias=False)
        self.bn2 = norm_layer(planes, eps=bn_eps, momentum=bn_momentum)
        self.downsample = downsample
        self.stride = stride
        self.inplace = inplace

    def forward(self, x):
        if x.is_cuda:
            from torchseg_amd.convwrw import bn_relu_conv, conv_with_skip
            skip = None
            if self.downsample is None and self.stride == 1:
                c1, skip = conv_with_skip(self.conv1, x)
                residual = skip if skip is not None else x
            elif self.downsample is not None and self.stride == 2:
                sc = self.downsample[0]
                sub = type(sc).__name__ == "PointwiseConv2d" and sc.stride == (2, 2) and sc.takes(x)
                c1, skip = conv_with_skip(self.conv1, x, subsample=sub)
                if skip is not None and sub and skip.shape[2:] != x.shape[2:]:
                    residual = norm_act(self.downsample[1], None, sc.forward_subsampled(skip))
                else:
                    residual = self._identity(skip if skip is not None else x)
            else:
                c1 = self.conv1(x)
                residual = self._identity(x)
            out = bn_relu_conv(self.bn1, self.relu, c1, self.conv2)
            return norm_act(self.bn2, self.relu_inplace, out, residual=residual)
        out = self.conv2(norm_act(self.bn1, self.relu, self.conv1(x)))
        return norm_act(self.bn2, self.relu_inplace, out, residual=self._identity(x))


class Bottleneck(_Block):
    expansion = 4

    def __init__(self, inplanes, planes, stride=1, norm_layer=None, bn_eps=1e-5, bn_momentum=0.1,
                 downsample=None, inplace=True):
        super(Bottleneck, self).__init__()
        self.conv1 = nn.Conv2d(inplanes, planes, kernel_size=1, bias=False)
        self.bn1 = norm_layer(planes, eps=bn_eps, momentum=bn_momentum)
        self.conv2 = nn.Conv2d(planes, planes, kernel_size=3, stride=stride, padding=1, bias=False)
        self.bn2 = norm_layer(planes, eps=bn_eps, momentum=bn_momentum)
        self.conv3 = nn.Conv2d(planes, planes * self.expansion, kernel_size=1, bias=False)
        self.bn3 = norm_layer(planes * self.expansion, eps=bn_eps, momentum=bn_momentum)
        self.relu = nn.ReLU(inplace=inplace)
        self.relu_inplace = nn.ReLU(inplace=True)
        self.downsample = downsample
        self.stride = stride
        self.inplace = inplace

    def forward(self, x):
        out = norm_act(self.bn1, self.relu, self.conv1(x))
        out = norm_act(self.bn2, self.relu, self.conv2(out))
        return norm_act(self.bn3, self.relu_inplace, self.conv3(out), residual=self._identity(x))


class ResNet(nn.Module):
    def __init__(self, block, layers, norm_layer=nn.BatchNorm2d, bn_eps=1e-5, bn_momentum=0.1,
                 deep_stem=False, stem_width=32, inplace=True):
        super(ResNet, self).__init__()
        self.inplanes = stem_width * 2 if deep_stem else 64
        if deep_stem:
            self.conv1 = nn.Sequential(
                nn.Conv2d(3, stem_width, kernel_size=3, stride=2, padding=1, bias=False),
                norm_layer(stem_width, eps=bn_eps, momentum=bn_momentum),
                nn.ReLU(inplace=inplace),
                nn.Conv2d(stem_width, stem_width, kernel_size=3, stride=1, padding=1, bias=False),
                norm_layer(stem_width, eps=bn_eps, momentum=bn_momentum),
                nn.ReLU(inplace=inplace),
                nn.Conv2d(stem_width, stem_width * 2, kernel_size=3, stride=1, padding=1, bias=False))
        else:
            self.conv1 = nn.Conv2d(3, 64, kernel_size=7, stride=2, padding=3, bias=False)
        self.bn1 = norm_layer(self.inplanes, eps=bn_eps, momentum=bn_momentum)
        self.relu = nn.ReLU(inplace=inplace)
        self.maxpool = _MaxPool2d(kernel_size=3, stride=2, padding=1)
        cfg = dict(bn_eps=bn_eps, bn_momentum=bn_momentum)
        self.layer1 = self._make_layer(block, norm_layer, 64, layers[0], inplace, **cfg)
        self.layer2 = self._make_layer(block, norm_layer, 128, layers[1], inplace, stride=2, **cfg)
        self.layer3 = self._make_layer(block, norm_layer, 256, layers[2], inplace, stride=2, **cfg)
        self.layer4 = self._make_layer(block, norm_layer, 512, layers[3], inplace, stride=2, **cfg)

    def _make_layer(self, block, norm_layer, planes, blocks, inplace=True, stride=1, bn_eps=1e-5,
                    bn_momentum=0.1):
        out_planes = planes * block.expansion
        downsample = None
        if stride != 1 or self.inplanes != out_planes:
            downsample = _shortcut(self.inplanes, out_planes, stride, norm_layer, bn_eps, bn_momentum)
        stages = [block(self.inplanes, planes, stride, norm_layer, bn_eps, bn_momentum, downsample, inplace)]
        self.inplanes = out_planes
        for _ in range(1, blocks):
            stages.append(block(self.inplanes, planes, norm_layer=norm_layer, bn_eps=bn_eps,
                                bn_momentum=bn_momentum, inplace=inplace))
        return nn.Sequential(*stages)

    def _stem(self, x):
        if isinstance(self.conv1, nn.Sequential):
            c = self.conv1
            if x.is_cuda:
                from torchseg_amd.convwrw import bn_relu_conv
                x = bn_relu_conv(c[1], c[2], c[0](x), c[3])
            else:
                x = c[3](norm_act(c[1], c[2], c[0](x)))
            x = norm_act(c[4], c[5], x)
            x = c[6](x)
        else:
            if x.is_cuda:
                from torchseg_amd.syncbn import stem_bn_relu_maxpool
                y = stem_bn_relu_maxpool(self.conv1, self.bn1, x, self.maxpool)
                if y is not None:
                    return y
            x = self.conv1(x)
        if x.is_cuda:
            from torchseg_amd.syncbn import bn_relu_maxpool
            y = bn_relu_maxpool(self.bn1, x, self.maxpool)
            if y is not None:
                return y
        return self.maxpool(norm_act(self.bn1, self.relu, x))

    @_outside_mode
    def forward(self, x):
        x = self._stem(x)
        blocks = []
        for stage in (self.layer1, self.layer2, self.layer3, self.layer4):
            x = stage(x)
            blocks.append(x)
        return blocks


def _build(block, layers, pretrained_model, kwargs):
    model = ResNet(block, layers, **kwargs)
    if pretrained_model is not None:
        model = load_model(model, pretrained_model)
    return model


def resnet18(pretrained_model=None, **kwargs):
    return _build(BasicBlock, [2, 2, 2, 2], pretrained_model, kwargs)


def resnet34(pretrained_model=None, **kwargs):
    return _build(BasicBlock, [3, 4, 6, 3], pretrained_model, kwargs)


def resnet50(pretrained_model=None, **kwargs):
    return _build(Bottleneck, [3, 4, 6, 3], pretrained_model, kwargs)


def resnet101(pretrained_model=None, **kwargs):
    return _build(Bottleneck, [3, 4, 23, 3], pretrained_model, kwargs)


def resnet152(pretrained_model=None, **kwargs):
    return _build(Bottleneck, [3, 8, 36, 3], pretrained_model, kwargs)
```

torchseg_amd/kernels.py:

```python
import ctypes as C
import os

import torch

from . import _lib as L


def bn_layout(x):
    if x.dim() == 2:
        return L.NHWC, x.shape[0], x.shape[1], 1
    n, c = x.shape[0], x.shape[1]
    hw = 1
    for s in x.shape[2:]:
        hw *= s
    if hw == 1 and x.is_contiguous():
        return L.NHWC, n, c, 1
    if x.is_contiguous():
        return L.NCHW, n, c, hw
    if x.dim() == 4 and x.is_contiguous(memory_format=torch.channels_last):
        return L.NHWC, n, c, hw
    return None


def _require_contiguous(*tensors):
    for t in tensors:
        if t is not None and not t.is_contiguous():
            raise L.TsgError("kernel wrapper needs a contiguous tensor, got strides %s for shape %s"
                             % (tuple(t.stride()), tuple(t.shape)))


def _dw_filter_dense(w):
    return w.stride(0) == 9 and w.stride(2) == 3 and w.stride(3) == 1


def _label_code(t):
    if t.dtype == torch.int64:
        return L.I64
    if t.dtype == torch.uint8:
        return L.U8
    raise L.TsgError(f"labels must be int64 or uint8, got {t.dtype}")



_SHADOW_PREP = os.environ.get("TSG_WEIGHT_SHADOW", "1") != "0"


class HipKernels:

    name = "hip"

    def __init__(self):
        self.lib = L.lib()
        self._npart = {}

    def _count(self, fn, *args, may_be_zero=False):
        key = (fn.__name__,) + args
        v = self._npart.get(key)
        if v is None:
            v = self._npart[key] = fn(*args)
        if v <= 0 and not may_be_zero:
            L.check(v if v < 0 else -2, fn.__name__)
        return v

    def bn_stats(self, x, layout, N, Cc, HW):
        lib = self.lib
        smax = self._count(self.lib.tsg_bn_num_partials, layout, N, Cc, HW)
        partial = torch.empty((smax, 2, Cc), dtype=torch.float32, device=x.device)
        rows = C.c_int(0)
        L.call(lib.tsg_bn_stats, x.data_ptr(), L.dtype_code(x), layout, N, Cc, HW, partial.data_ptr(), C.byref(rows),
               L.stream_ptr(x))
        return partial, rows.value

    def bn_collapse(self, partial, S, Cc, out, count=None):
        if count is None:
            L.call(self.lib.tsg_bn_collapse, partial.data_ptr(), S, Cc, out.data_ptr(), L.stream_ptr(partial))
        else:
            L.call(self.lib.tsg_bn_collapse_count, partial.data_ptr(), S, Cc, out.data_ptr(), int(count), L.stream_ptr(partial))

    def bn_finalize(self, partial, S, Cc, count, count_dev, eps, momentum, gamma, beta,
                    running_mean, running_var, nbt):
        dev = partial.device
        mean = torch.empty(Cc, dtype=torch.float32, device=dev)
        invstd = torch.empty(Cc, dtype=torch.float32, device=dev)
        fp = torch.empty((3, Cc), dtype=torch.float32, device=dev)
        L.call(self.lib.tsg_bn_finalize, partial.data_ptr(), S, Cc, float(count), L.ptr(count_dev), eps, momentum, L.ptr(gamma),
               L.ptr(beta), L.ptr(running_mean), L.ptr(running_var), L.ptr(nbt), mean.data_ptr(), invstd.data_ptr(),
               fp.data_ptr(), L.stream_ptr(partial))
        return mean, invstd, fp

    def bn_affine(self, mean, invstd, gamma, beta):
        Cc = mean.numel()
        fp = torch.empty((3, Cc), dtype=torch.float32, device=mean.device)
        L.call(self.lib.tsg_bn_affine, mean.data_ptr(), invstd.data_ptr(), L.ptr(gamma), L.ptr(beta), Cc, fp.data_ptr(),
               L.stream_ptr(mean))
        return fp

    def bn_apply_fwd(self, x, residual, layout, N, Cc, HW, fp, relu, out=None):
        y = torch.empty_like(x) if out is None else out
        L.call(self.lib.tsg_bn_apply_fwd, x.data_ptr(), L.ptr(residual), y.data_ptr(), L.dtype_code(x), layout, N, Cc, HW,
               fp.data_ptr(), int(relu), L.stream_ptr(x))
        return y

    def bn_bwd_reduce(self, dy, x, y, layout, N, Cc, HW, fp, relu):
        lib = self.lib
        smax = self._count(self.lib.tsg_bn_num_partials, layout, N, Cc, HW)
        partial = torch.empty((smax, 2, Cc), dtype=torch.float32, device=x.device)
        rows = C.c_int(0)
        L.call(lib.tsg_bn_bwd_reduce, dy.data_ptr(), x.data_ptr(), L.ptr(y), L.dtype_code(x), layout, N, Cc, HW, fp.data_ptr(),
               int(relu), partial.data_ptr(), C.byref(rows), L.stream_ptr(x))
        return partial, rows.value

    def bn_bwd_coeffs(self, partial, S, Cc, count, count_dev, batch_stats, invstd, fp,
                      want_param_grads, want_pack):
        dev = partial.device
        dgamma = torch.empty(Cc, dtype=torch.float32, device=dev) if want_param_grads else None
        dbeta = torch.empty(Cc, dtype=torch.float32, device=dev) if want_param_grads else None
        bp = torch.empty((5, Cc), dtype=torch.float32, device=dev) if want_pack else None
        L.call(self.lib.tsg_bn_bwd_coeffs, partial.data_ptr(), S, Cc, float(count), L.ptr(count_dev), int(batch_stats),
               invstd.data_ptr(), L.ptr(fp), L.ptr(dgamma), L.ptr(dbeta), L.ptr(bp), L.stream_ptr(partial))
        return dgamma, dbeta, bp

    def bn_bwd_apply(self, dy, x, y, layout, N, Cc, HW, bp, relu, want_dres):
        dx = torch.empty_like(x)
        dres = torch.empty_like(x) if want_dres else None
        L.call(self.lib.tsg_bn_bwd_apply, dy.data_ptr(), x.data_ptr(), L.ptr(y), dx.data_ptr(), L.ptr(dres), L.dtype_code(x),
               layout, N, Cc, HW, bp.data_ptr(), int(relu), L.stream_ptr(x))
        return dx, dres

    def bn_maskbits_supported(self, x, layout, Cc, HW):
        return bool(self.lib.tsg_bn_maskbits_supported(L.dtype_code(x), layout, Cc, HW)) and x.data_ptr() % 16 == 0

    def bn_apply_fwd_bits(self, x, residual, layout, N, Cc, HW, fp):
        y = torch.empty_like(x)
        V = 8 if x.dtype == torch.bfloat16 else 4
        bits = torch.empty(N * HW * Cc // V, dtype=torch.uint8, device=x.device)
        L.call(self.lib.tsg_bn_apply_fwd_maskbits, x.data_ptr(), L.ptr(residual), y.data_ptr(), bits.data_ptr(),
               L.dtype_code(x), layout, N, Cc, HW, fp.data_ptr(), L.stream_ptr(x))
        return y, bits

    def bn_bwd_reduce_bits(self, dy, x, bits, layout, N, Cc, HW, fp):
        smax = self._count(self.lib.tsg_bn_num_partials, layout, N, Cc, HW)
        partial = torch.empty((smax, 2, Cc), dtype=torch.float32, device=x.device)
        rows = C.c_int(0)
        L.call(self.lib.tsg_bn_bwd_reduce_maskbits, dy.data_ptr(), x.data_ptr(), bits.data_ptr(), L.dtype_code(x), layout, N,
               Cc, HW, fp.data_ptr(), partial.data_ptr(), C.byref(rows), L.stream_ptr(x))
        return partial, rows.value

    def bn_bwd_apply_bits(self, dy, x, bits, layout, N, Cc, HW, bp, want_dres):
        dx = torch.empty_like(x)
        dres = torch.empty_like(x) if want_dres else None
        L.call(self.lib.tsg_bn_bwd_apply_maskbits, dy.data_ptr(), x.data_ptr(), bits.data_ptr(), dx.data_ptr(), L.ptr(dres),
               L.dtype_code(x), layout, N, Cc, HW, bp.data_ptr(), L.stream_ptr(x))
        return dx, dres

    def bn_mixed_supported(self, x):
        if x.dim() != 4 or not x.is_contiguous():
            return False
        return bool(self.lib.tsg_bn_mixed_supported(L.dtype_code(x), x.shape[1], x.shape[2] * x.shape[3]))

    def bn_apply_fwd_mixed(self, x, N, Cc, HW, fp, relu):
        y = torch.empty_like(x, memory_format=torch.channels_last)
        L.call(self.lib.tsg_bn_apply_fwd_mixed, x.data_ptr(), y.data_ptr(), L.dtype_code(x), N, Cc, HW, fp.data_ptr(),
               int(relu), L.stream_ptr(x))
        return y

    def bn_bwd_reduce_mixed(self, dy, x, N, Cc, HW, fp, relu):
        smax = self.lib.tsg_bn_mixed_num_partials(N, Cc, HW)
        partial = torch.empty((smax, 2, Cc), dtype=torch.float32, device=x.device)
        rows = C.c_int(0)
        L.call(self.lib.tsg_bn_bwd_reduce_mixed, dy.data_ptr(), x.data_ptr(), L.dtype_code(x), N, Cc, HW, fp.data_ptr(),
               int(relu), partial.data_ptr(), C.byref(rows), L.stream_ptr(x))
        return partial, rows.value

    def bn_bwd_apply_mixed(self, dy, x, N, Cc, HW, bp, relu):
        dx = torch.empty_like(x)
        L.call(self.lib.tsg_bn_bwd_apply_mixed, dy.data_ptr(), x.data_ptr(), dx.data_ptr(), L.dtype_code(x), N, Cc, HW,
               bp.data_ptr(), int(relu), L.stream_ptr(x))
        return dx

    def gap_fwd(self, x, layout, N, Cc, HW):
        wsb = self.lib.tsg_gap_ws_bytes(layout, N, Cc, HW)
        ws = torch.empty(max(wsb, 16), dtype=torch.uint8, device=x.device)
        out = torch.empty((N, Cc), dtype=x.dtype, device=x.device)
        L.call(self.lib.tsg_gap_fwd, x.data_ptr(), out.data_ptr(), L.dtype_code(x), layout, N, Cc, HW, ws.data_ptr(),
               ws.numel(), L.stream_ptr(x))
        return out

    def gap_bwd(self, dout, like, layout, N, Cc, HW):
        dx = torch.empty_like(like)
        L.call(self.lib.tsg_gap_bwd, dout.data_ptr(), dx.data_ptr(), L.dtype_code(dout), layout, N, Cc, HW, L.stream_ptr(dout))
        return dx

    def adaptive_avgpool_supported(self, x, OH, OW):
        return (x.dim() == 4 and x.is_cuda and x.dtype in (torch.float32, torch.bfloat16)
                and x.is_contiguous(memory_format=torch.channels_last)
                and x.shape[1] % (8 if x.dtype == torch.bfloat16 else 4) == 0
                and 0 < OH <= x.shape[2] and 0 < OW <= x.shape[3])

    def adaptive_avgpool_fwd(self, x, OH, OW):
        N, Cc, H, W = x.shape
        wsb = self.lib.tsg_adaptive_avgpool_nhwc_ws_bytes(L.dtype_code(x), N, Cc, H, W, OH, OW)
        ws = torch.empty(max(wsb, 16), dtype=torch.uint8, device=x.device)
        out = torch.empty((N, Cc, OH, OW), dtype=x.dtype, device=x.device, memory_format=torch.channels_last)
        L.call(self.lib.tsg_adaptive_avgpool_nhwc_fwd, x.data_ptr(), out.data_ptr(), L.dtype_code(x), N, Cc, H, W, OH, OW,
               ws.data_ptr(), ws.numel(), L.stream_ptr(x))
        return out

    def adaptive_avgpool_bwd(self, dout, H, W):
        N, Cc, OH, OW = dout.shape
        dx = torch.empty((N, Cc, H, W), dtype=dout.dtype, device=dout.device, memory_format=torch.channels_last)
        L.call(self.lib.tsg_adaptive_avgpool_nhwc_bwd, dout.data_ptr(), dx.data_ptr(), L.dtype_code(dout), N, Cc, H, W, OH, OW,
               L.stream_ptr(dout))
        return dx

    def cat_channels(self, a, b):
        B, Ca, H, W = a.shape
        Cb = b.shape[1]
        out = torch.empty((B, Ca + Cb, H, W), dtype=a.dtype, device=a.device, memory_format=torch.channels_last)
        es = a.element_size()
        L.call(self.lib.tsg_cat2_rows, a.data_ptr(), b.data_ptr(), out.data_ptr(), B * H * W, Ca * es, Cb * es, L.stream_ptr(a))
        return out

    def chanscale_fwd(self, x, s, layout, N, Cc, HW, add_identity):
        y = torch.empty_like(x)
        L.call(self.lib.tsg_chanscale_fwd, x.data_ptr(), s.data_ptr(), y.data_ptr(), L.dtype_code(x), layout, N, Cc, HW,
               int(add_identity), L.stream_ptr(x))
        return y

    def chanscale_bwd(self, dy, x, s, layout, N, Cc, HW, add_identity):
        wsb = self.lib.tsg_gap_ws_bytes(layout, N, Cc, HW)
        ws = torch.empty(max(wsb, 16), dtype=torch.uint8, device=x.device)
        dx = torch.empty_like(x)
        ds = torch.empty((N, Cc), dtype=x.dtype, device=x.device)
        L.call(self.lib.tsg_chanscale_bwd, dy.data_ptr(), x.data_ptr(), s.data_ptr(), dx.data_ptr(), ds.data_ptr(),
               L.dtype_code(x), layout, N, Cc, HW, int(add_identity), ws.data_ptr(), ws.numel(), L.stream_ptr(x))
        return dx, ds

    def chanscale_split_supported(self, x, layout, Cc):
        return layout == L.NHWC and Cc % (8 if x.dtype == torch.bfloat16 else 4) == 0 and x.data_ptr() % 16 == 0

    def chanscale_bwd_ds(self, dy, x, layout, N, Cc, HW):
        wsb = self.lib.tsg_gap_ws_bytes(layout, N, Cc, HW)
        ws = torch.empty(max(wsb, 16), dtype=torch.uint8, device=x.device)
        ds = torch.empty((N, Cc), dtype=x.dtype, device=x.device)
        L.call(self.lib.tsg_chanscale_bwd_ds, dy.data_ptr(), x.data_ptr(), ds.data_ptr(), L.dtype_code(x), layout, N, Cc, HW,
               ws.data_ptr(), ws.numel(), L.stream_ptr(x))
        return ds

    def chanscale_bwd_dx(self, dy, s, gadd, layout, N, Cc, HW, add_identity):
        dx = torch.empty_like(dy)
        L.call(self.lib.tsg_chanscale_bwd_dx, dy.data_ptr(), s.data_ptr(), gadd.data_ptr(), dx.data_ptr(), L.dtype_code(dy),
               layout, N, Cc, HW, int(add_identity), L.stream_ptr(dy))
        return dx

    def maxpool_fwd(self, x, K_, S_, P_):
        N, Cc, IH, IW = x.shape
        OH, OW = (IH + 2 * P_ - K_) // S_ + 1, (IW + 2 * P_ - K_) // S_ + 1
        y = torch.empty((N, Cc, OH, OW), dtype=x.dtype, device=x.device, memory_format=torch.channels_last)
        idx = torch.empty((N, OH, OW, Cc), dtype=torch.uint8, device=x.device)
        L.call(self.lib.tsg_maxpool_nhwc_fwd, x.data_ptr(), y.data_ptr(), idx.data_ptr(), L.dtype_code(x), N, Cc, IH, IW, OH,
               OW, K_, S_, P_, L.stream_ptr(x))
        return y, idx

    def maxpool_bwd(self, dy, idx, in_shape, K_, S_, P_):
        N, Cc, IH, IW = in_shape
        OH, OW = dy.shape[2], dy.shape[3]
        dx = torch.empty(in_shape, dtype=dy.dtype, device=dy.device, memory_format=torch.channels_last)
        L.call(self.lib.tsg_maxpool_nhwc_bwd, dy.data_ptr(), idx.data_ptr(), dx.data_ptr(), L.dtype_code(dy), N, Cc, IH, IW, OH,
               OW, K_, S_, P_, L.stream_ptr(dy))
        return dx

    def bn_relu_pool_fwd(self, x, fp):
        N, Cc, IH, IW = x.shape
        OH, OW = (IH - 1) // 2 + 1, (IW - 1) // 2 + 1
        y = torch.empty((N, Cc, OH, OW), dtype=x.dtype, device=x.device, memory_format=torch.channels_last)
        idx = torch.empty((N, OH, OW, Cc), dtype=torch.uint8, device=x.device)
        L.call(self.lib.tsg_bn_relu_pool_fwd, x.data_ptr(), y.data_ptr(), idx.data_ptr(), L.dtype_code(x), N, Cc, IH, IW, OH,
               OW, fp.data_ptr(), L.stream_ptr(x))
        return y, idx

    def bn_relu_pool_bwd_reduce(self, dpool, idx, x, fp):
        N, Cc, IH, IW = x.shape
        OH, OW = dpool.shape[2], dpool.shape[3]
        dt = L.dtype_code(x)
        S = self._count(self.lib.tsg_bn_relu_pool_bwd_num_partials, dt, N, Cc, IH, IW)
        partial = torch.empty((S, 2, Cc), dtype=torch.float32, device=x.device)
        L.call(self.lib.tsg_bn_relu_pool_bwd_reduce, dpool.data_ptr(), idx.data_ptr(), x.data_ptr(), L.dtype_code(x), N, Cc, IH,
               IW, OH, OW, fp.data_ptr(), partial.data_ptr(), L.stream_ptr(x))
        return partial, S

    def bn_relu_pool_bwd_apply(self, dpool, idx, x, bp):
        N, Cc, IH, IW = x.shape
        OH, OW = dpool.shape[2], dpool.shape[3]
        dx = torch.empty_like(x)
        L.call(self.lib.tsg_bn_relu_pool_bwd_apply, dpool.data_ptr(), idx.data_ptr(), x.data_ptr(), dx.data_ptr(),
               L.dtype_code(x), N, Cc, IH, IW, OH, OW, bp.data_ptr(), L.stream_ptr(x))
        return dx

    def stem_conv_supported(self, x, weight, stride, padding, dilation, groups):
        if x.dim() != 4 or weight.dim() != 4 or x.dtype != torch.bfloat16 or not x.is_contiguous():
            return False
        return bool(self.lib.tsg_stem_conv_supported(L.dtype_code(x), x.shape[1], weight.shape[0], weight.shape[2],
                                                     weight.shape[3], stride, padding, dilation, groups,
                                                     x.shape[2], x.shape[3]))

    def _scratch(self, name, nbytes, dev):
        st = torch.cuda.current_stream(dev)
        key = (name, dev.index, st.cuda_stream)
        pool = self.__dict__.setdefault("_scratch_bufs", {})
        ws = pool.get(key)
        if ws is None or ws.numel() < nbytes:
            if ws is not None:
                self.__dict__.setdefault("_scratch_retired", []).append(ws)
            ws = pool[key] = torch.empty(int(nbytes), dtype=torch.uint8, device=dev)
            ws.record_stream(st)
        return ws

    def presize_scratch(self, streams, dev):
        pool = self.__dict__.setdefault("_scratch_bufs", {})
        need = {}
        for (name, di, _sid), ws in list(pool.items()):
            if di == dev.index:
                need[name] = max(need.get(name, 0), ws.numel())
        for st in streams:
            with torch.cuda.stream(st):
                for name, n in need.items():
                    self._scratch(name, n, dev)

    def _stem_ws(self, dev):
        return self._scratch("stem", self.lib.tsg_stem_conv_ws_bytes(), dev)

    def stem_conv_fwd(self, x, weight):
        _require_contiguous(x, weight)
        B, _, H, W = x.shape
        y = torch.empty((B, 64, (H - 1) // 2 + 1, (W - 1) // 2 + 1), dtype=x.dtype, device=x.device,
                        memory_format=torch.channels_last)
        ws = self._stem_ws(x.device)
        L.call(self.lib.tsg_stem_conv_fwd, x.data_ptr(), weight.data_ptr(), y.data_ptr(), B, H, W, ws.data_ptr(), ws.numel(),
               L.stream_ptr(x))
        return y

    def stem_conv_fwd_stats(self, x, weight):
        _require_contiguous(x, weight)
        B, _, H, W = x.shape
        y = torch.empty((B, 64, (H - 1) // 2 + 1, (W - 1) // 2 + 1), dtype=x.dtype, device=x.device,
                        memory_format=torch.channels_last)
        S = self._count(self.lib.tsg_stem_conv_stats_partials, B, H, W)
        partial = torch.empty((S, 2, 64), dtype=torch.float32, device=x.device)
        ws = self._stem_ws(x.device)
        L.call(self.lib.tsg_stem_conv_fwd_stats, x.data_ptr(), weight.data_ptr(), y.data_ptr(), partial.data_ptr(), B, H, W,
               ws.data_ptr(), ws.numel(), L.stream_ptr(x))
        return y, partial

    def stem_conv_wrw(self, x, dy):
        _require_contiguous(x)
        if not dy.is_contiguous(memory_format=torch.channels_last):
            raise ValueError("stem_conv_wrw expects a channels_last gradient")
        B, _, H, W = x.shape
        dw = torch.empty((64, 3, 7, 7), dtype=torch.float32, device=x.device)
        ws = self._stem_ws(x.device)
        L.call(self.lib.tsg_stem_conv_wrw, x.data_ptr(), dy.data_ptr(), dw.data_ptr(), B, H, W, ws.data_ptr(), ws.numel(),
               L.stream_ptr(x))
        return dw

    def stem3_conv_supported(self, x, weight, stride, padding, dilation, groups):
        if x.dim() != 4 or weight.dim() != 4 or x.dtype != torch.bfloat16 or not x.is_contiguous():
            return False
        return bool(self.lib.tsg_stem3_conv_supported(L.dtype_code(x), x.shape[1], weight.shape[0], weight.shape[2],
                                                      weight.shape[3], stride, padding, dilation, groups,
                                                      x.shape[2], x.shape[3]))

    def stem3_conv_fwd(self, x, weight):
        _require_contiguous(x, weight)
        B, _, H, W = x.shape
        y = torch.empty((B, 64, (H - 1) // 2 + 1, (W - 1) // 2 + 1), dtype=x.dtype, device=x.device,
                        memory_format=torch.channels_last)
        ws = self._scratch("stem3", self.lib.tsg_stem3_conv_ws_bytes(), x.device)
        L.call(self.lib.tsg_stem3_conv_fwd, x.data_ptr(), weight.data_ptr(), y.data_ptr(), B, H, W, ws.data_ptr(), ws.numel(),
               L.stream_ptr(x))
        return y

    def stem3_conv_wrw(self, x, dy):
        _require_contiguous(x)
        if dy.dtype != torch.bfloat16 or not dy.is_contiguous(memory_format=torch.channels_last):
            raise ValueError("stem3_conv_wrw expects a bf16 channels_last gradient")
        B, _, H, W = x.shape
        if tuple(dy.shape) != (B, 64, (H - 1) // 2 + 1, (W - 1) // 2 + 1):
            raise ValueError("stem3_conv_wrw: gradient shape %s does not match the image %s" % (tuple(dy.shape), tuple(x.shape)))
        dw = torch.empty((64, 3, 3, 3), dtype=torch.float32, device=x.device)
        ws = self._scratch("stem3", self.lib.tsg_stem3_conv_ws_bytes(), x.device)
        L.call(self.lib.tsg_stem3_conv_wrw, x.data_ptr(), dy.data_ptr(), dw.data_ptr(), B, H, W, ws.data_ptr(), ws.numel(),
               L.stream_ptr(x))
        return dw

    def stem_conv_wrw_bn(self, x, da, xc, bp):
        _require_contiguous(x, bp)
        for t in (da, xc):
            if not t.is_contiguous(memory_format=torch.channels_last) or t.dtype != torch.bfloat16 or t.shape != da.shape:
                raise ValueError("stem_conv_wrw_bn expects bf16 channels_last da / xc of one shape")
        if bp.dtype != torch.float32 or tuple(bp.shape) != (5, 64):
            raise ValueError("stem_conv_wrw_bn expects the [5, 64] fp32 backward pack")
        B, _, H, W = x.shape
        dw = torch.empty((64, 3, 7, 7), dtype=torch.float32, device=x.device)
        ws = self._stem_ws(x.device)
        L.call(self.lib.tsg_stem_conv_wrw_bn, x.data_ptr(), da.data_ptr(), xc.data_ptr(), bp.data_ptr(), dw.data_ptr(), B, H, W,
               ws.data_ptr(), ws.numel(), L.stream_ptr(x))
        return dw

    def stem_conv_stats(self, x, weight):
        _require_contiguous(x, weight)
        B, _, H, W = x.shape
        S = self._count(self.lib.tsg_stem_conv_stats_partials, B, H, W)
        partial = torch.empty((S, 2, 64), dtype=torch.float32, device=x.device)
        ws = self._stem_ws(x.device)
        L.call(self.lib.tsg_stem_conv_stats, x.data_ptr(), weight.data_ptr(), partial.data_ptr(), B, H, W, ws.data_ptr(),
               ws.numel(), L.stream_ptr(x))
        return partial

    def stem_conv_bn_relu_pool_fwd(self, x, weight, fp):
        _require_contiguous(x, weight, fp)
        B, _, H, W = x.shape
        OH, OW = (H - 1) // 2 + 1, (W - 1) // 2 + 1
        PH, PW = (OH - 1) // 2 + 1, (OW - 1) // 2 + 1
        y = torch.empty((B, 64, PH, PW), dtype=torch.bfloat16, device=x.device, memory_format=torch.channels_last)
        idx = torch.empty((B, PH, PW, 64), dtype=torch.uint8, device=x.device)
        ws = self._stem_ws(x.device)
        L.call(self.lib.tsg_stem_conv_bn_relu_pool_fwd, x.data_ptr(), weight.data_ptr(), fp.data_ptr(), y.data_ptr(),
               idx.data_ptr(), B, H, W, ws.data_ptr(), ws.numel(), L.stream_ptr(x))
        return y, idx

    def stem_conv_bn_relu_pool_bwd_reduce(self, x, weight, dpool, idx, fp):
        _require_contiguous(x, weight, fp)
        if not dpool.is_contiguous(memory_format=torch.channels_last) or dpool.dtype != torch.bfloat16:
            raise ValueError("stem_conv_bn_relu_pool_bwd_reduce expects a bf16 channels_last pooled gradient")
# ... 899 lines not shown
                raise L.TsgError("edge_labels takes contiguous uint8 tensors on the GPU")
            wsb = self.lib.tsg_edge_labels_ws_bytes(int(geom[i, 2]), int(geom[i, 3]))
            ws = torch.empty(wsb, dtype=torch.uint8, device=dev)
            L.call(self.lib.tsg_edge_labels, gts[i].data_ptr(), geom[i].ctypes.data, None, CH, CW, int(ignore_label),
                   int(threshold), int(threshold), int(aperture), int(dilate_size), int(pad_label), out[i].data_ptr(),
                   _label_code(out), ws.data_ptr(), wsb, L.stream_ptr(out))
        return out

    def resize_bilinear_hp(self, x, OH, OW, out=None, accumulate=False):
        _require_contiguous(x)
        IH, IW = x.shape[-2], x.shape[-1]
        NC = x.numel() // (IH * IW)
        if out is None:
            out = torch.empty(tuple(x.shape[:-2]) + (OH, OW), dtype=torch.float32, device=x.device)
            accumulate = False
        else:
            want = tuple(x.shape[:-2]) + (int(OH), int(OW))
            if out.dtype != torch.float32 or out.device != x.device or tuple(out.shape) != want or not out.is_contiguous():
                raise L.TsgError("resize_bilinear_hp: out must be a contiguous float32 %s tensor on %s, got %s %s with "
                                 "strides %s on %s" % (want, x.device, out.dtype, tuple(out.shape), tuple(out.stride()),
                                                       out.device))
        L.call(self.lib.tsg_resize_bilinear_hp, x.data_ptr(), out.data_ptr(), L.dtype_code(x), NC, IH, IW, int(OH), int(OW),
               int(accumulate), L.stream_ptr(x))
        return out

    def seg_tail_logprob(self, z, H, W, out=None):
        _require_contiguous(z)
        N, Cc, h, w = z.shape
        dt = L.dtype_code(z)
        if not self.lib.tsg_seg_tail_logprob_supported(dt, Cc, h, w, int(H), int(W)):
            raise L.TsgError(f"seg_tail_logprob: unsupported shape {tuple(z.shape)} -> ({H}, {W})")
        if out is None:
            out = torch.empty((N, Cc, int(H), int(W)), dtype=torch.float32, device=z.device)
        L.call(self.lib.tsg_seg_tail_logprob, z.data_ptr(), dt, N, Cc, h, w, int(H), int(W), out.data_ptr(), L.stream_ptr(z))
        return out

    def seg_tail_accum(self, z, zflip, geom, dst, H, W, accumulate=True, region=None):
        _require_contiguous(z, zflip, dst)
        N, Cc, h, w = z.shape
        if zflip is not None and (zflip.shape != z.shape or zflip.dtype != z.dtype):
            raise L.TsgError("seg_tail_accum: zflip must match z")
        if dst.dtype != torch.float32 or dst.dim() != 3 or dst.shape[0] != Cc:
            raise L.TsgError("seg_tail_accum: dst must be fp32 [C, Hd, Wd]")
        Hd, Wd = dst.shape[1], dst.shape[2]
        dt = L.dtype_code(z)
        if not self.lib.tsg_seg_tail_accum_supported(dt, Cc, h, w, int(H), int(W), Hd, Wd):
            raise L.TsgError(f"seg_tail_accum: unsupported shape {tuple(z.shape)} -> ({H}, {W}) into {tuple(dst.shape)}")
        if isinstance(geom, torch.Tensor) and geom.is_cuda:
            if region is None or geom.dtype != torch.int32 or tuple(geom.shape) != (N, 6) or not geom.is_contiguous():
                raise L.TsgError("seg_tail_accum: a device geom is int32 [N,6] and needs `region`")
            g_dev = geom
        else:
            import numpy as np
            g = np.asarray(geom, dtype=np.int64).reshape(N, 6)
            oy, ox, t, l, rows, cols = (g[:, i] for i in range(6))
            if ((rows < 0) | (cols < 0) | (oy < 0) | (ox < 0) | (t < 0) | (l < 0) | (t + rows > H) | (l + cols > W)
                    | (oy + rows > Hd) | (ox + cols > Wd)).any():
                raise L.TsgError(f"seg_tail_accum: window geometry out of range: {g.tolist()}")
            live = (rows > 0) & (cols > 0)
            if region is None:
                region = ((int(oy[live].min()), int((oy + rows)[live].max()), int(ox[live].min()),
                           int((ox + cols)[live].max())) if live.any() else (0, 0, 0, 0))
            g_dev = torch.from_numpy(g.astype(np.int32)).to(z.device)
        by0, by1, bx0, bx1 = (int(v) for v in region)
        L.call(self.lib.tsg_seg_tail_accum, z.data_ptr(), L.ptr(zflip), dt, N, Cc, h, w, int(H), int(W), g_dev.data_ptr(),
               dst.data_ptr(), Hd, Wd, by0, by1, bx0, bx1, int(bool(accumulate)), L.stream_ptr(z))
        return dst

    def confusion_map(self, pred, gt, n_cl, out=None):
        _require_contiguous(pred, gt)
        if pred.numel() != gt.numel():
            raise ValueError("pred and gt must have the same number of pixels")
        if out is None:
            out = torch.zeros(n_cl * n_cl + 3, dtype=torch.int64, device=gt.device)
        L.call(self.lib.tsg_confusion_map, pred.data_ptr(), _label_code(pred), gt.data_ptr(), _label_code(gt), gt.numel(), n_cl,
               out.data_ptr(), L.stream_ptr(gt))
        return out

    def confusion_logits(self, logits, gt, n_cl, out=None):
        _require_contiguous(logits, gt)
        B, Cc = logits.shape[0], logits.shape[1]
        HW = logits.numel() // max(B * Cc, 1)
        if gt.numel() != B * HW:
            raise ValueError("gt must have one label per pixel of logits")
        if out is None:
            out = torch.zeros(n_cl * n_cl + 3, dtype=torch.int64, device=gt.device)
        L.call(self.lib.tsg_confusion_logits, logits.data_ptr(), L.dtype_code(logits), gt.data_ptr(), _label_code(gt), B, Cc,
               HW, n_cl, out.data_ptr(), L.stream_ptr(gt))
        return out

    SGD_MAX_SEGS = 128
    SGD_MAX_GROUPS = 24

    def sgd_multi_blockmap(self, numel, device):
        import numpy as np
        n = np.ascontiguousarray(numel, dtype=np.int64)
        nb = self.lib.tsg_sgd_multi_blockmap(n.ctypes.data, len(n), None, 0)
        if nb < 0:
            L.check(int(nb), "tsg_sgd_multi_blockmap")
        host = np.empty((nb, 2), dtype=np.int32)
        L.check(int(min(0, self.lib.tsg_sgd_multi_blockmap(n.ctypes.data, len(n), host.ctypes.data, nb))),
                "tsg_sgd_multi_blockmap")
        return torch.from_numpy(host).to(device)

    def sgd_multi_step_dev(self, ptrs, numel, group, lr_dev, momentum, weight_decay, blockmap, grad_scale=1.0):
        L.call(self.lib.tsg_sgd_multi_step_dev, ptrs[0].ctypes.data, ptrs[1].ctypes.data, ptrs[2].ctypes.data,
               numel.ctypes.data, group.ctypes.data, len(numel), lr_dev.data_ptr(), momentum.ctypes.data,
               weight_decay.ctypes.data, len(momentum), blockmap.data_ptr(), blockmap.shape[0], float(grad_scale),
               L.stream_ptr(lr_dev))

    def multi_copy(self, srcs, dsts, blockmap=None, scale=1.0):
        import numpy as np
        numel = np.array([t.numel() for t in srcs], dtype=np.int64)
        if blockmap is None:
            blockmap = self.sgd_multi_blockmap(numel, srcs[0].device)
        ptrs = np.array([[t.data_ptr() for t in srcs], [t.data_ptr() for t in dsts]], dtype=np.uint64)
        L.call(self.lib.tsg_multi_copy_f32, ptrs[0].ctypes.data, ptrs[1].ctypes.data, numel.ctypes.data, len(srcs),
               blockmap.data_ptr(), blockmap.shape[0], float(scale), L.stream_ptr(srcs[0]))
        return blockmap


_provider = None


def provider():
    global _provider
    if _provider is None:
        _provider = HipKernels()
    return _provider


def _set_provider_for_tests(p):
    global _provider
    old = _provider
    _provider = p
    return old


def _nbytes(t):
    return 0 if t is None else t.numel() * t.element_size()


def _bsum_bytes(kw):
    b = (kw or {}).get("bsum")
    return _nbytes(b[0]) if b is not None else 0


_ALGO_BYTES = {
    "bn_stats": lambda a, r: _nbytes(a[0]),
    "bn_apply_fwd": lambda a, r: 2 * _nbytes(a[0]) + _nbytes(a[1]),
    "bn_bwd_reduce": lambda a, r: 2 * _nbytes(a[0]) + _nbytes(a[2]),
    "bn_bwd_apply": lambda a, r: 3 * _nbytes(a[0]) + _nbytes(a[2]) + (_nbytes(a[0]) if a[9] else 0),
    "bn_apply_fwd_bits": lambda a, r: 2 * _nbytes(a[0]) + _nbytes(a[1]) + _nbytes(a[0]) // 16,
    "bn_bwd_reduce_bits": lambda a, r: 2 * _nbytes(a[0]) + _nbytes(a[2]),
    "bn_bwd_apply_bits": lambda a, r: 3 * _nbytes(a[0]) + _nbytes(a[2]) + (_nbytes(a[0]) if a[8] else 0),
    "ohem_fwd": lambda a, r: _nbytes(a[0]) + _nbytes(a[1]) + 8 * a[1].numel(),
    "ohem_bwd": lambda a, r: 2 * _nbytes(a[0]) + _nbytes(a[1]) + 8 * a[1].numel(),
    "ohem_up_fwd": lambda a, r: _nbytes(a[0]) + _nbytes(a[1]) + 8 * a[1].numel(),
    "ohem_up_bwd": lambda a, r: 2 * _nbytes(a[0]) + _nbytes(a[1]) + 8 * a[1].numel(),
    "upsample_fwd": lambda a, r: _nbytes(a[0]) + _nbytes(a[1]) + _nbytes(r),
    "upsample_presum_fwd": lambda a, r: _nbytes(a[0]) + _nbytes(a[1]) + _nbytes(r),
    "upsample_bwd": lambda a, r: _nbytes(a[0]) + _nbytes(r),
    "upsample_fwd_nhwc": lambda a, r: _nbytes(a[0]) + _nbytes(a[1]) + _nbytes(r),
    "upsample_bwd_nhwc": lambda a, r: _nbytes(a[0]) + _nbytes(r),
    "bn_apply_fwd_mixed": lambda a, r: 2 * _nbytes(a[0]),
    "bn_bwd_reduce_mixed": lambda a, r: 2 * _nbytes(a[0]),
    "bn_bwd_apply_mixed": lambda a, r: 3 * _nbytes(a[0]),
    "chanscale_fwd": lambda a, r: 2 * _nbytes(a[0]),
    "chanscale_bwd": lambda a, r: 3 * _nbytes(a[0]),
    "chanscale_bwd_ds": lambda a, r: 2 * _nbytes(a[0]),
    "chanscale_bwd_dx": lambda a, r: 2 * _nbytes(a[0]),
    "maxpool_fwd": lambda a, r: _nbytes(a[0]) + _nbytes(r[0]) + _nbytes(r[1]),
    "maxpool_bwd": lambda a, r: _nbytes(a[0]) + _nbytes(a[1]) + _nbytes(r),
    "gap_fwd": lambda a, r: _nbytes(a[0]),
    "stem_conv_fwd": lambda a, r: _nbytes(a[0]) + _nbytes(r),
    "stem_conv_fwd_stats": lambda a, r: _nbytes(a[0]) + _nbytes(r),
    "bn_relu_pool_fwd": lambda a, r: _nbytes(a[0]) + _nbytes(r[0]) + _nbytes(r[1]),
    "bn_relu_pool_bwd_reduce": lambda a, r: _nbytes(a[0]) + _nbytes(a[1]) + _nbytes(a[2]),
    "bn_relu_pool_bwd_apply": lambda a, r: _nbytes(a[0]) + _nbytes(a[1]) + 2 * _nbytes(a[2]),
    "stem_conv_wrw": lambda a, r: _nbytes(a[0]) + _nbytes(a[1]),
    "stem3_conv_fwd": lambda a, r: _nbytes(a[0]) + _nbytes(r),
    "stem3_conv_wrw": lambda a, r: _nbytes(a[0]) + _nbytes(a[1]),
    "stem_conv_wrw_bn": lambda a, r: _nbytes(a[0]) + _nbytes(a[1]) + _nbytes(a[2]),
    "stem_conv_stats": lambda a, r: _nbytes(a[0]),
    "stem_conv_bn_relu_pool_fwd": lambda a, r: _nbytes(a[0]) + _nbytes(r[0]) + _nbytes(r[1]),
    "stem_conv_bn_relu_pool_bwd_reduce": lambda a, r: _nbytes(a[0]) + _nbytes(a[2]) + _nbytes(a[3]),
    "stem_conv_wrw_bn_pool": lambda a, r, kw=None: (_nbytes(a[0]) + _nbytes(a[2]) + _nbytes(a[3])
                                                    + (_nbytes((kw or {}).get("xc")) if (kw or {}).get("xc") is not None else 0)),
    "conv3x3_wrw": lambda a, r: _nbytes(a[0]) + _nbytes(a[1]),
    "conv3x3_c64_fwd": lambda a, r, kw=None: _nbytes(a[0]) + _nbytes(r) + _bsum_bytes(kw),
    "conv3x3_gen_fwd": lambda a, r: _nbytes(a[0]) + _nbytes(a[1][0]) + _nbytes(r[0] if isinstance(r, tuple) else r),
    "conv3x3_c64_s2_dgrad": lambda a, r, kw=None: _nbytes(a[0]) + _nbytes(r) + _bsum_bytes(kw),
    "conv3x3_s2_dgrad": lambda a, r: _nbytes(a[0]) + _nbytes(r),
    "gap_bwd": lambda a, r: _nbytes(r),
}


_ALGO_FLOPS = {
    "conv3x3_wrw": lambda a, r: 2 * 9 * a[1].numel() * a[0].shape[1],
    "stem_conv_fwd": lambda a, r: 2 * 147 * r.numel(),
    "conv3x3_c64_fwd": lambda a, r: 2 * 9 * 64 * r.numel(),
    "conv3x3_gen_fwd": lambda a, r: 2 * 9 * a[0].shape[1] * (r[0] if isinstance(r, tuple) else r).numel(),
    "conv3x3_c64_s2_dgrad": lambda a, r: 2 * 9 * 64 * a[0].numel(),
    "conv3x3_s2_dgrad": lambda a, r: 2 * 9 * a[1].shape[1] * a[0].numel(),
    "stem_conv_fwd_stats": lambda a, r: 2 * 147 * r.numel(),
    "stem_conv_wrw": lambda a, r: 2 * 147 * a[1].numel(),
    "stem3_conv_fwd": lambda a, r: 2 * 27 * r.numel(),
    "stem3_conv_wrw": lambda a, r: 2 * 27 * a[1].numel(),
    "stem_conv_wrw_bn": lambda a, r: 2 * 147 * a[1].numel(),
    "stem_conv_stats": lambda a, r: 2 * 147 * _stem_y_numel(a[0]),
    "stem_conv_bn_relu_pool_fwd": lambda a, r: 2 * 147 * _stem_y_numel(a[0]),
    "stem_conv_bn_relu_pool_bwd_reduce": lambda a, r: 2 * 147 * _stem_y_numel(a[0]),
    "stem_conv_wrw_bn_pool": lambda a, r: 2 * 2 * 147 * _stem_y_numel(a[0]),
}


def _stem_y_numel(x):
    B, _, H, W = x.shape
    return B * 64 * ((H - 1) // 2 + 1) * ((W - 1) // 2 + 1)
MFMA_PEAK_TFLOPS = 2500.0


class CallCounter:

    def __init__(self, prov):
        self.prov = prov
        self.counts = {}
        self._names = [n for n in dir(type(prov)) if not n.startswith("_") and callable(getattr(type(prov), n))]
        for n in self._names:
            self._wrap(n)

    def _wrap(self, name):
        fn = getattr(self.prov, name)
        counts = self.counts

        def counted(*args, **kw):
            counts[name] = counts.get(name, 0) + 1
            return fn(*args, **kw)

        setattr(self.prov, name, counted)

    def stop(self):
        for n in self._names:
            try:
                delattr(self.prov, n)
            except AttributeError:
                pass
        return dict(self.counts)


class KernelTimer:

    def __init__(self, prov, names=None):
        self.prov = prov
        self.names = list(names or _ALGO_BYTES.keys())
        self.enabled = True
        self.records = {n: [] for n in self.names}
        self.marks = []
        self._orig = {}
        for n in self.names:
            self._wrap(n)

    def _wrap(self, name):
        fn = getattr(self.prov, name)
        self._orig[name] = fn
        rec = self.records[name]
        cost = _ALGO_BYTES[name]
        flops = _ALGO_FLOPS.get(name)

        def timed(*args, **kw):
            if not self.enabled:
                return fn(*args, **kw)
            s = torch.cuda.Event(enable_timing=True)
            e = torch.cuda.Event(enable_timing=True)
            s.record()
            out = fn(*args, **kw)
            e.record()
            res = out if name in ("maxpool_fwd", "bn_relu_pool_fwd") else (out[0] if isinstance(out, tuple) else out)
            by = cost(args, res, kw) if cost.__code__.co_argcount == 3 else cost(args, res)
            rec.append((s, e, by, flops(args, res) if flops else 0))
            return out

        setattr(self.prov, name, timed)

    def mark_step(self):
        self.marks.append({n: len(r) for n, r in self.records.items()})

    def _measured(self):
        out = {}
        steps = len(self.marks)
        for n, recs in self.records.items():
            if not recs:
                continue
            el = [(r[0].elapsed_time(r[1]), r[2], r[3]) for r in recs]
            per = len(recs) // steps if steps > 1 else 0
            if steps > 1 and per > 0 and all(m.get(n, 0) == per * (i + 1) for i, m in enumerate(self.marks)):
                out[n] = [min((el[k * per + j] for k in range(steps)), key=lambda t: t[0]) for j in range(per)]
            elif steps > 1:
                lo = self.marks[-2].get(n, 0)
                out[n] = el[lo:] or el
            else:
                out[n] = el
        return out

    def stop(self):
        for n, fn in self._orig.items():
            try:
                delattr(self.prov, n)
            except AttributeError:
                setattr(self.prov, n, fn)
        torch.cuda.synchronize()
        self.stats = {}
        self.eff = self._measured()
        for n, recs in self.eff.items():
            if recs:
                ms = sum(r[0] for r in recs)
                by = sum(r[1] for r in recs)
                fl = sum(r[2] for r in recs)
                self.stats[n] = {"launches": len(recs), "total_ms": round(ms, 3), "avg_us": round(ms * 1e3 / len(recs), 2),
                                 "algo_MB_per_launch": round(by / len(recs) / 1e6, 3),
                                 "GBps": round(by / (ms * 1e-3) / 1e9, 1) if ms > 0 else None}
                if fl and ms > 0:
                    self.stats[n]["algo_GFLOP_per_launch"] = round(fl / len(recs) / 1e9, 3)
                    self.stats[n]["TFLOPs"] = round(fl / (ms * 1e-3) / 1e12, 1)

    def summary(self):
        return self.stats

    FAMILIES = {
        "syncbn": ("bn_stats", "bn_apply_fwd", "bn_bwd_reduce", "bn_bwd_apply", "bn_apply_fwd_bits", "bn_bwd_reduce_bits",
                   "bn_bwd_apply_bits", "bn_apply_fwd_mixed", "bn_bwd_reduce_mixed",
                   "bn_bwd_apply_mixed", "bn_relu_pool_fwd", "bn_relu_pool_bwd_reduce", "bn_relu_pool_bwd_apply"),
        "conv3x3_wrw": ("conv3x3_wrw",),
        "conv3x3_fwd_dgrad": ("conv3x3_gen_fwd", "conv3x3_c64_fwd", "conv3x3_c64_s2_dgrad", "conv3x3_s2_dgrad"),
        "fused_heads": ("ohem_up_fwd", "ohem_up_bwd", "ohem_fwd", "ohem_bwd"),
        "stem": ("stem_conv_fwd", "stem_conv_fwd_stats", "stem_conv_wrw", "stem_conv_wrw_bn", "stem_conv_stats",
                 "stem_conv_bn_relu_pool_fwd", "stem_conv_bn_relu_pool_bwd_reduce", "stem_conv_wrw_bn_pool",
                 "stem3_conv_fwd", "stem3_conv_wrw"),
        "upsample": ("upsample_fwd", "upsample_presum_fwd", "upsample_bwd", "upsample_fwd_nhwc", "upsample_bwd_nhwc"),
    }

    def family_stats(self):
        fam = {}
        for name, members in self.FAMILIES.items():
            recs = [r for m in members for r in self.eff.get(m, ())]
            if not recs:
                continue
            ms = sum(r[0] for r in recs)
            by = sum(r[1] for r in recs)
            fl = sum(r[2] for r in recs)
            if ms <= 0:
                continue
            st = {"launches": len(recs), "total_ms": round(ms, 3), "avg_us": round(ms * 1e3 / len(recs), 2),
                  "algo_MB_per_launch": round(by / len(recs) / 1e6, 3), "GBps": round(by / (ms * 1e-3) / 1e9, 1),
                  "members": [m for m in members if self.eff.get(m)]}
            if fl:
                st["algo_GFLOP_per_launch"] = round(fl / len(recs) / 1e9, 3)
                st["TFLOPs"] = round(fl / (ms * 1e-3) / 1e12, 1)
            fam[name] = st
        return fam

    def dominant(self):
        return max(self.stats, key=lambda n: self.stats[n]["total_ms"]) if self.stats else None

    def dominant_family(self):
        fam = self.family_stats()
        return max(fam, key=lambda n: fam[n]["total_ms"]) if fam else None

    def _roof_entry(self, name, st, peak_gbs, tj):
        traffic = busy = None
        if tj is not None:
            tr = [(tj.get(m), self.stats[m]["launches"]) for m in st.get("members", [name]) if m in self.stats]
            if tr and all(t is not None for t, _ in tr):
                traffic = int(sum(t * n for t, n in tr) / sum(n for _, n in tr))
            bz = [((tj.get("_mfma_busy_frac") or {}).get(m), self.stats[m]["total_ms"]) for m in st.get("members", [name])
                  if m in self.stats]
            if bz and all(b is not None for b, _ in bz):
                busy = round(sum(b * w for b, w in bz) / sum(w for _, w in bz), 4)
        out = {"bound": "hbm", "kernel": name, "launches": st["launches"], "total_ms": st["total_ms"],
               "achieved": st["GBps"], "peak": peak_gbs, "unit": "GB/s",
               "frac": round(st["GBps"] / peak_gbs, 4), "traffic": traffic,
               "algo_bytes_per_launch": int(st["algo_MB_per_launch"] * 1e6), "avg_launch_us": st["avg_us"]}
        if "TFLOPs" in st and st["TFLOPs"] / MFMA_PEAK_TFLOPS > out["frac"]:
            out.update({"bound": "mfma", "achieved": st["TFLOPs"], "peak": MFMA_PEAK_TFLOPS, "unit": "TFLOP/s",
                        "frac": round(st["TFLOPs"] / MFMA_PEAK_TFLOPS, 4),
                        "algo_flops_per_launch": int(st["algo_GFLOP_per_launch"] * 1e9),
                        "hbm_GBps": st["GBps"], "hbm_frac": round(st["GBps"] / peak_gbs, 4)})
            if busy is not None:
                out["mfma_busy_frac"] = busy
        return out

    def roofline(self, peak_gbs, profiles_dir=None, by_family=False):
        tj = source = None
        if profiles_dir:
            import json
            import os
            f = os.path.join(profiles_dir, "traffic.json")
            if os.path.exists(f):
                tj = json.load(open(f))
                source = "profiles/traffic.json@" + str(tj.get("_round", "r02")) + \
                    " (rocprofv3 --pmc FETCH_SIZE / WRITE_SIZE passes over this bench command, tools/pmc_traffic.sh)"
        if by_family:
            fam = self.family_stats()
            order = sorted(fam, key=lambda n: -fam[n]["total_ms"])
            out = self._roof_entry(order[0], fam[order[0]], peak_gbs, tj)
            out["family_members"] = fam[order[0]]["members"]
            out["traffic_source"] = source
            out["top_families"] = [self._roof_entry(n, fam[n], peak_gbs, tj) for n in order[:3]]
            return out
        name = self.dominant()
        out = self._roof_entry(name, dict(self.stats[name], members=[name]), peak_gbs, tj)
        out["traffic_source"] = source
        return out
```

torchseg_amd/syncbn.py:

```python
import os

import torch
import torch.distributed as dist
from torch.nn.modules.batchnorm import _BatchNorm

from . import kernels as K

PREFER_CHANNELS_LAST_OUTPUT = False


def _world(group):
    if dist.is_available() and dist.is_initialized():
        w = dist.get_world_size(group)
        if w == 1 and os.environ.get("TSG_FORCE_COLLECTIVES", "0") == "1":
            return 2
        return w
    return 1


def _exchange(msg, group):
    from . import comm
    c = comm.get(group, like=msg)
    if c is not None:
        c.small_all_reduce(msg)
    else:
        dist.all_reduce(msg, op=dist.ReduceOp.SUM, group=group)


_FP32_GATHER = os.environ.get("TSG_BN_FP32_GATHER", "1") != "0"


def _all_gather(msg, group, world):
    from . import comm
    out = torch.empty((world, msg.numel()), dtype=msg.dtype, device=msg.device)
    c = comm.get(group, like=msg)
    if c is not None and c.world == world:
        c.all_gather(msg, out.view(-1))
    elif c is not None and c.world == 1:
        c.all_gather(msg, out[0])
        out[1:].zero_()
    elif dist.is_initialized() and dist.get_world_size(group) == world:
        dist.all_gather(list(out.unbind(0)), msg, group=group)
    else:
        out.copy_(msg.unsqueeze(0).expand_as(out))
        out[1:].zero_()
    return out


def _hilo_rows(partial, S):
    d = partial[:S].to(torch.float64).sum(0)
    hi = d.to(torch.float32)
    return torch.stack([hi, (d - hi.to(torch.float64)).to(torch.float32)])


def _gather_hilo(partial, S, C, group, world, count=None):
    words = [_hilo_rows(partial, S).reshape(-1)]
    if count is not None:
        words.append(torch.tensor([float(count // 4096), float(count % 4096)], dtype=torch.float32, device=partial.device))
    got = _all_gather(torch.cat(words), group, world)
    rows = got[:, :4 * C].reshape(2 * world, 2, C).contiguous()
    return rows, (got[:, 4 * C:].sum(0) if count is not None else None)


def _dense(x):
    lay = K.bn_layout(x)
    if lay is None:
        if x.dim() == 4 and x.stride(1) == 1:
            x = x.contiguous(memory_format=torch.channels_last)
        else:
            x = x.contiguous()
        lay = K.bn_layout(x)
    return x, lay


def _like(t, ref):
    if t.dtype != ref.dtype:
        t = t.to(ref.dtype)
    if t.stride() != ref.stride():
        out = torch.empty_like(ref)
        out.copy_(t)
        t = out
    return t


def _batch_statistics(kp, x, layout, N, C, HW, mod, gamma, beta, group, world, hint=None):
    n_local = N * HW
    if world == 1 and n_local <= 1:
        raise ValueError("Expected more than 1 value per channel when training, got input size {}"
                         .format(tuple(x.shape)))
    if hint is not None:
        partial, S = hint, hint.shape[0]
    else:
        partial, S = kp.bn_stats(x, layout, N, C, HW)
    rm = mod.running_mean if mod.track_running_stats else None
    rv = mod.running_var if mod.track_running_stats else None
    nbt = mod.num_batches_tracked if mod.track_running_stats else None
    momentum = 0.0 if mod.momentum is None else float(mod.momentum)
    if world > 1 and _FP32_GATHER and x.dtype == torch.float32:
        rows, count_dev = _gather_hilo(partial, S, C, group, world, count=n_local)
        _, invstd, fp = kp.bn_finalize(rows, 2 * world, C, 0.0, count_dev, float(mod.eps), momentum,
                                       gamma, beta, rm, rv, nbt)
        return invstd, fp, count_dev
    if world > 1:
        msg = torch.empty(2 * C + 2, dtype=torch.float32, device=x.device)
        kp.bn_collapse(partial, S, C, msg, count=n_local)
        _exchange(msg, group)
        count_dev = msg[2 * C:]
        _, invstd, fp = kp.bn_finalize(msg, 1, C, 0.0, count_dev, float(mod.eps), momentum,
                                       gamma, beta, rm, rv, nbt)
        return invstd, fp, count_dev
    _, invstd, fp = kp.bn_finalize(partial, S, C, float(n_local), None, float(mod.eps), momentum,
                                   gamma, beta, rm, rv, nbt)
    return invstd, fp, None


def _backward_pack(kp, partial, S, C, n_local, invstd, fp, count_dev, use_batch_stats, group, world, device,
                   parity=False):
    if use_batch_stats and world > 1 and parity and _FP32_GATHER:
        dgamma, dbeta, _ = kp.bn_bwd_coeffs(partial, S, C, 1.0, None, True, invstd, fp, True, False)
        rows, _ = _gather_hilo(partial, S, C, group, world)
        _, _, bp = kp.bn_bwd_coeffs(rows, 2 * world, C, 0.0, count_dev, True, invstd, fp, False, True)
        return dgamma, dbeta, bp
    if use_batch_stats and world > 1:
        sums = torch.empty(2 * C, dtype=torch.float32, device=device)
        kp.bn_collapse(partial, S, C, sums)
        dgamma, dbeta, _ = kp.bn_bwd_coeffs(sums, 1, C, 1.0, None, True, invstd, fp, True, False)
        _exchange(sums, group)
        _, _, bp = kp.bn_bwd_coeffs(sums, 1, C, 0.0, count_dev, True, invstd, fp, False, True)
        return dgamma, dbeta, bp
    return kp.bn_bwd_coeffs(partial, S, C, float(n_local), None, use_batch_stats, invstd, fp, True, True)


def _forward_pack(kp, x, layout, N, C, HW, mod, weight, bias, use_batch_stats, group, hint=None):
    world = _world(group) if use_batch_stats else 1
    gamma = weight.float() if weight is not None else None
    beta = bias.float() if bias is not None else None
    if use_batch_stats:
        return _batch_statistics(kp, x, layout, N, C, HW, mod, gamma, beta, group, world, hint) + (world,)
    mean = mod.running_mean.float()
    invstd = torch.rsqrt(mod.running_var.float() + mod.eps)
    return invstd, kp.bn_affine(mean, invstd, gamma, beta), None, world


def _affine_grads(dgamma, dbeta, weight, bias):
    if weight is None:
        return None, None
    return dgamma.to(weight.dtype), dbeta.to(bias.dtype) if bias is not None else None


_MASKBITS = os.environ.get("TSG_BN_MASKBITS", "1") != "0"


class _SyncBNFn(torch.autograd.Function):
    @staticmethod
    def forward(ctx, x, residual, weight, bias, mod, relu, use_batch_stats, group, hint=None):
        kp = K.provider()
        x, (layout, N, C, HW) = _dense(x)
        if residual is not None:
            residual = _like(residual, x)
        invstd, fp, count_dev, world = _forward_pack(kp, x, layout, N, C, HW, mod, weight, bias, use_batch_stats, group, hint)
        mixed = (PREFER_CHANNELS_LAST_OUTPUT and residual is None and layout == K.L.NCHW
                 and kp.bn_mixed_supported(x))
        need_y = relu and residual is not None
        bits = None
        if mixed:
            y = kp.bn_apply_fwd_mixed(x, N, C, HW, fp, relu)
        elif (need_y and _MASKBITS and hasattr(kp, "bn_apply_fwd_bits") and kp.bn_maskbits_supported(x, layout, C, HW)
              and residual.data_ptr() % 16 == 0):
            y, bits = kp.bn_apply_fwd_bits(x, residual, layout, N, C, HW, fp)
        else:
            y = kp.bn_apply_fwd(x, residual, layout, N, C, HW, fp, relu)
        ctx.save_for_backward(x, bits if bits is not None else (y if need_y else None), weight, bias, invstd, fp, count_dev)
        ctx.cfg = (layout, N, C, HW, relu, use_batch_stats, group, world, residual is not None, mixed)
        ctx.bits = bits is not None
        return y

    @staticmethod
    def backward(ctx, dy):
        kp = K.provider()
        x, y, weight, bias, invstd, fp, count_dev = ctx.saved_tensors
        layout, N, C, HW, relu, use_batch_stats, group, world, has_res, mixed = ctx.cfg
        if mixed:
            if dy.dtype != x.dtype:
                dy = dy.to(x.dtype)
            dy = dy.contiguous(memory_format=torch.channels_last)
            partial, S = kp.bn_bwd_reduce_mixed(dy, x, N, C, HW, fp, relu)
        else:
            dy = _like(dy, x)
            if ctx.bits and dy.data_ptr() % 16:
                dy = dy.clone(memory_format=torch.preserve_format)
            if ctx.bits:
                partial, S = kp.bn_bwd_reduce_bits(dy, x, y, layout, N, C, HW, fp)
            else:
                partial, S = kp.bn_bwd_reduce(dy, x, y, layout, N, C, HW, fp, relu)
        dgamma, dbeta, bp = _backward_pack(kp, partial, S, C, N * HW, invstd, fp, count_dev,
                                           use_batch_stats, group, world, x.device, parity=x.dtype == torch.float32)
        if mixed:
            dx, dres = kp.bn_bwd_apply_mixed(dy, x, N, C, HW, bp, relu), None
        elif ctx.bits:
            dx, dres = kp.bn_bwd_apply_bits(dy, x, y, layout, N, C, HW, bp, has_res)
        else:
            dx, dres = kp.bn_bwd_apply(dy, x, y, layout, N, C, HW, bp, relu, has_res)
        dgamma, dbeta = _affine_grads(dgamma, dbeta, weight, bias)
        return dx, dres, dgamma, dbeta, None, None, None, None, None


class _BnReluPoolFn(torch.autograd.Function):

    @staticmethod
    def forward(ctx, x, weight, bias, mod, use_batch_stats, group, hint):
        kp = K.provider()
        layout, N, C, HW = K.bn_layout(x)
        invstd, fp, count_dev, world = _forward_pack(kp, x, layout, N, C, HW, mod, weight, bias, use_batch_stats, group, hint)
        y, idx = kp.bn_relu_pool_fwd(x, fp)
        ctx.save_for_backward(x, idx, weight, bias, invstd, fp, count_dev)
        ctx.cfg = (N, C, HW, use_batch_stats, group, world)
        return y

    @staticmethod
    def backward(ctx, dpool):
        kp = K.provider()
        x, idx, weight, bias, invstd, fp, count_dev = ctx.saved_tensors
        N, C, HW, use_batch_stats, group, world = ctx.cfg
        if dpool.dtype != x.dtype:
            dpool = dpool.to(x.dtype)
        dpool = dpool.contiguous(memory_format=torch.channels_last)
        partial, S = kp.bn_relu_pool_bwd_reduce(dpool, idx, x, fp)
        dgamma, dbeta, bp = _backward_pack(kp, partial, S, C, N * HW, invstd, fp, count_dev,
                                           use_batch_stats, group, world, x.device, parity=x.dtype == torch.float32)
        dx = kp.bn_relu_pool_bwd_apply(dpool, idx, x, bp)
        dgamma, dbeta = _affine_grads(dgamma, dbeta, weight, bias)
        return dx, dgamma, dbeta, None, None, None, None


class _StemConvBnReluPoolFn(torch.autograd.Function):

    @staticmethod
    def forward(ctx, img, w_stem, weight, bias, mod, use_batch_stats, group, full):
        kp = K.provider()
        B, _, H, W = img.shape
        OH, OW = (H - 1) // 2 + 1, (W - 1) // 2 + 1
        N, C, HW = B, 64, OH * OW
        xc = partial = None
        if use_batch_stats and full:
            partial = kp.stem_conv_stats(img, w_stem)
        elif use_batch_stats:
            xc, partial = kp.stem_conv_fwd_stats(img, w_stem)
        invstd, fp, count_dev, world = _forward_pack(kp, img, 1, N, C, HW, mod, weight, bias, use_batch_stats, group, partial)
        if not (use_batch_stats or full):
            xc = kp.stem_conv_fwd(img, w_stem)
        if full:
            y, idx = kp.stem_conv_bn_relu_pool_fwd(img, w_stem, fp)
        else:
            y, idx = kp.bn_relu_pool_fwd(xc, fp)
        ctx.save_for_backward(img, w_stem, idx, weight, bias, invstd, fp, count_dev, xc)
        ctx.cfg = (N, C, HW, use_batch_stats, group, world)
        ctx.wparam = w_stem
        return y

    @staticmethod
    def backward(ctx, dpool):
        kp = K.provider()
        img, w_stem, idx, weight, bias, invstd, fp, count_dev, xc = ctx.saved_tensors
        N, C, HW, use_batch_stats, group, world = ctx.cfg
        if dpool.dtype != torch.bfloat16:
            dpool = dpool.to(torch.bfloat16)
        dpool = dpool.contiguous(memory_format=torch.channels_last)
        if xc is None:
            partial, S = kp.stem_conv_bn_relu_pool_bwd_reduce(img, w_stem, dpool, idx, fp)
        else:
            partial, S = kp.bn_relu_pool_bwd_reduce(dpool, idx, xc, fp)
        dgamma, dbeta, bp = _backward_pack(kp, partial, S, C, N * HW, invstd, fp, count_dev,
                                           use_batch_stats, group, world, img.device, parity=False)
        dw = None
        if ctx.needs_input_grad[1]:
            from .convwrw import wrw_on_side_stream
            yy = xc if _STEM_WRW_READS_Y else None
            dw = wrw_on_side_stream(lambda: kp.stem_conv_wrw_bn_pool(img, w_stem, dpool, idx, bp, xc=yy), ctx.wparam,
                                    img, dpool, idx, bp, yy)
        dgamma, dbeta = _affine_grads(dgamma, dbeta, weight, bias)
        return None, dw, dgamma, dbeta, None, None, None, None


_STEM_RECOMPUTE = int(os.environ.get("TSG_STEM_RECOMPUTE", "2"))
_STEM_WRW_READS_Y = os.environ.get("TSG_STEM_WRW_READS_Y", "0") == "1"


def stem_bn_relu_maxpool(conv, bn, img, pool):
    from .stemconv import StemConv2d, _as_bf16_image, _wants_bf16

    def one(v):
        return v[0] if isinstance(v, (tuple, list)) and len(set(v)) == 1 else v
    if not (_STEM_RECOMPUTE > 0 and _FUSE_STEM_POOL and isinstance(conv, StemConv2d) and isinstance(bn, SyncBatchNorm)
            and isinstance(pool, torch.nn.MaxPool2d) and isinstance(img, torch.Tensor) and img.is_cuda and img.dim() == 4
            and not img.requires_grad and conv.bias is None and conv.weight.dtype == torch.float32
            and conv.padding_mode == "zeros" and bn.num_features == 64 and bn.momentum is not None
            and _wants_bf16(img)
            and not (conv._forward_hooks or conv._forward_pre_hooks or bn._forward_hooks or bn._forward_pre_hooks
                     or pool._forward_hooks or pool._forward_pre_hooks)):
        return None
    if (one(pool.kernel_size), one(pool.stride), one(pool.padding), one(pool.dilation)) != (3, 2, 1, 1) \
            or pool.ceil_mode or pool.return_indices:
        return None
    kp = K.provider()
    if not hasattr(kp, "stem_conv_bn_relu_pool_fwd"):
        return None
    xb = _as_bf16_image(img)
    w_stem = conv.weight if conv.weight.is_contiguous() else conv.weight.contiguous()
    if not kp.stem_conv_supported(xb, w_stem, conv.stride[0], conv.padding[0], conv.dilation[0], conv.groups):
        return None
    if ((xb.shape[2] - 1) // 2 + 1) < 1 or ((xb.shape[3] - 1) // 2 + 1) < 1:
        return None
    use_batch_stats = bn.training or not bn.track_running_stats
    with torch.autocast("cuda", enabled=False):
        return _StemConvBnReluPoolFn.apply(xb, w_stem, bn.weight, bn.bias, bn, use_batch_stats, bn.process_group,
                                           _STEM_RECOMPUTE == 1)


_FUSE_STEM_POOL = os.environ.get("TSG_FUSE_STEM_POOL", "1") != "0"


def bn_relu_maxpool(bn, x, pool):
    def one(v):
        return v[0] if isinstance(v, (tuple, list)) and len(set(v)) == 1 else v
    if not (_FUSE_STEM_POOL and isinstance(bn, SyncBatchNorm) and isinstance(pool, torch.nn.MaxPool2d)
            and isinstance(x, torch.Tensor) and x.is_cuda and x.dim() == 4
            and x.dtype in (torch.float32, torch.bfloat16)):
        return None
    if (one(pool.kernel_size), one(pool.stride), one(pool.padding), one(pool.dilation)) != (3, 2, 1, 1) \
            or pool.ceil_mode or pool.return_indices or bn.momentum is None:
        return None
    vec = 8 if x.dtype == torch.bfloat16 else 4
    if x.shape[1] % vec or x.is_contiguous() or not x.is_contiguous(memory_format=torch.channels_last):
        return None
    bn._check_input_dim(x)
    use_batch_stats = bn.training or not bn.track_running_stats
    from .stemconv import take_bn_partial
    hint = take_bn_partial(x) if use_batch_stats else None
    return _BnReluPoolFn.apply(x, bn.weight, bn.bias, bn, use_batch_stats, bn.process_group, hint)


class SyncBatchNorm(_BatchNorm):

    def __init__(self, num_features, eps=1e-5, momentum=0.1, affine=True,
                 track_running_stats=True, process_group=None, channel_last=False,
                 fuse_relu=False):
        super().__init__(num_features, eps=eps, momentum=momentum, affine=affine,
                         track_running_stats=track_running_stats)
        self.process_group = process_group
        self.channel_last = channel_last
        self.fuse_relu = fuse_relu

    def _check_input_dim(self, input):
        if input.dim() < 2:
            raise ValueError("expected at least 2D input (got {}D input)".format(input.dim()))
        if input.shape[1] != self.num_features:
            raise ValueError("expected {} channels, got {}".format(self.num_features, input.shape[1]))

    def forward(self, input, residual=None, relu=None):
        self._check_input_dim(input)
        if self.momentum is None:
            raise NotImplementedError("cumulative moving average (momentum=None) is not supported")
        relu = self.fuse_relu if relu is None else bool(relu)
        use_batch_stats = self.training or not self.track_running_stats
        hint = None
        if use_batch_stats and hasattr(input, "_tsg_bn_partial"):
            from .stemconv import take_bn_partial
            hint = take_bn_partial(input)
        return _SyncBNFn.apply(input, residual, self.weight, self.bias, self, relu,
                               use_batch_stats, self.process_group, hint)


def convert_syncbn_model(module, process_group=None, channel_last=False):
    mod = module
    if isinstance(module, torch.nn.modules.batchnorm._BatchNorm) and not isinstance(module, SyncBatchNorm):
        mod = SyncBatchNorm(module.num_features, module.eps, module.momentum, module.affine,
                            module.track_running_stats, process_group, channel_last)
        if module.affine:
            mod.weight = module.weight
            mod.bias = module.bias
        if module.track_running_stats:
            mod.running_mean = module.running_mean
            mod.running_var = module.running_var
            mod.num_batches_tracked = module.num_batches_tracked
    for name, child in module.named_children():
        mod.add_module(name, convert_syncbn_model(child, process_group, channel_last))
    return mod
```

Before: 1325.

## Emit stride-2 subsampled twin from BN epilogue and add pooled-xmax stem path

The BN+residual+ReLU forward kernel gains a SUB mode that also writes a stride-2 subsampled copy of its output. This copy is registered as a twin and later reused by the next stage's stride-2 shortcut conv, instead of running a separate strided gather-and-copy. Last blocks of layer1-3 are linked to the next layer's first block so the producer knows when to emit the twin. The change also adds an optional bn_relu_pool variant that stores the pre-activation value at each argmax for a cheaper backward reduce, but it is off by default. The cost is extra per-element index arithmetic in the BN kernel and Python-side storage/version matching to find the twin.

```diff
diff --git a/include/tsg_hip.h b/include/tsg_hip.h
--- a/include/tsg_hip.h
+++ b/include/tsg_hip.h
@@ -72,6 +72,8 @@
                               int64_t C, int64_t HW, const float* fwd_pack, void* stream);
 int tsg_bn_bwd_reduce_maskbits(const void* dy, const void* x, const void* bits, int dtype, int layout, int64_t N, int64_t C,
                                int64_t HW, const float* fwd_pack, float* partial, int* rows, void* stream);
+int tsg_bn_apply_fwd_sub(const void* x, const void* residual, void* y, void* y2, void* bits, int dtype, int64_t N, int64_t C,
+                         int H, int W, const float* fwd_pack, void* stream);
 int tsg_bn_bwd_apply_maskbits(const void* dy, const void* x, const void* bits, void* dx, void* dres, int dtype, int layout,
                               int64_t N, int64_t C, int64_t HW, const float* bwd_pack, void* stream);
 
@@ -143,6 +145,8 @@
 
 int tsg_bn_relu_pool_fwd(const void* x, void* y, void* argmax_u8, int dtype, int64_t N, int C, int IH, int IW,
                          int OH, int OW, const float* fp, void* stream);
+int tsg_bn_relu_pool_fwd_xmax(const void* x, void* y, void* argmax_u8, void* xmax, int dtype, int64_t N, int C, int IH,
+                              int IW, int OH, int OW, const float* fp, void* stream);
 int tsg_bn_relu_pool_bwd_num_partials(int dtype, int64_t N, int C, int IH, int IW);
 int tsg_bn_relu_pool_bwd_reduce(const void* dpool, const void* argmax_u8, const void* x, int dtype, int64_t N,
                                 int C, int IH, int IW, int OH, int OW, const float* fp, float* partial,
diff --git a/torchseg_amd/convwrw.py b/torchseg_amd/convwrw.py
--- a/torchseg_amd/convwrw.py
+++ b/torchseg_amd/convwrw.py
@@ -222,6 +222,31 @@
                  family == "lib" and _DGRAD_FWD and stride == 1 and (_DGRAD_ANY or conv.in_channels == conv.out_channels))
 
 
+SUBSAMPLE_GATHERS = [0]
+
+
+def _subsampled(x):
+    twin = S.take_subsample_twin(x)
+    if twin is not None:
+        return twin
+    SUBSAMPLE_GATHERS[0] += 1
+    return x[:, :, ::2, ::2].contiguous(memory_format=torch.channels_last)
+
+
+def feeds_compact_shortcut(block, x_like):
+    sc = block.downsample[0] if block.downsample is not None else None
+    conv = block.conv1
+    if not (S._SUB_FROM_PRODUCER and _FUSE_SKIP and _SKIP_SUB and block.stride == 2 and sc is not None
+            and type(sc).__name__ == "PointwiseConv2d" and sc.stride == (2, 2) and isinstance(conv, WrwConv2d)
+            and conv.stride == (2, 2) and conv.bias is None and conv.weight.dtype == torch.float32
+            and conv.padding_mode == "zeros" and conv.weight.requires_grad and torch.is_grad_enabled()
+            and x_like.is_cuda and x_like.dim() == 4 and x_like.dtype == torch.bfloat16
+            and x_like.is_contiguous(memory_format=torch.channels_last) and sc.takes(x_like)):
+        return False
+    route = _route(conv, x_like)
+    return route is not None and route.family != "gen" and route.skip and route.compact
+
+
 class _ConvWrwFn(torch.autograd.Function):
 
     @staticmethod
@@ -245,7 +270,7 @@
         ctx.skip_sub = skip == 2
         if not skip:
             return y, partial
-        return y, partial, (x[:, :, ::2, ::2].contiguous(memory_format=torch.channels_last) if ctx.skip_sub else x)
+        return y, partial, (_subsampled(x) if ctx.skip_sub else x)
 
     @staticmethod
     def backward(ctx, dy, _dpartial, dskip=None):
diff --git a/torchseg_amd/csrc/bn.hip b/torchseg_amd/csrc/bn.hip
--- a/torchseg_amd/csrc/bn.hip
+++ b/torchseg_amd/csrc/bn.hip
@@ -289,11 +289,11 @@
   }
 }
 
-template <typename T, int V, bool RELU, bool RES, bool BITS = false>
+template <typename T, int V, bool RELU, bool RES, bool BITS = false, bool SUB = false>
 __global__ __launch_bounds__(kThreads) void bn_fwd_nhwc(
     const T* __restrict__ x, const T* __restrict__ res, T* __restrict__ y,
     int64_t M, int64_t C, int GT, int R, int64_t rows_per_block, const float* __restrict__ fp, int rev,
-    unsigned char* __restrict__ bits = nullptr) {
+    unsigned char* __restrict__ bits = nullptr, T* __restrict__ y2 = nullptr, int H = 1, int W = 1) {
   const int tid = threadIdx.x;
   const int gl = tid % GT, r = tid / GT;
   const int64_t g = (int64_t)blockIdx.y * GT + gl;
@@ -305,6 +305,15 @@
   const int64_t row0 = (int64_t)(rev ? gridDim.x - 1 - blockIdx.x : blockIdx.x) * rows_per_block;
   int64_t row1 = row0 + rows_per_block;
   if (row1 > M) row1 = M;
+  int64_t pn = 0;
+  int ph = 0, pw = 0;
+  const int sw = R % W, sh = (R / W) % H, sn = R / W / H;
+  if (SUB) {
+    const int64_t first = row0 + r;
+    pw = (int)(first % W);
+    ph = (int)(first / W % H);
+    pn = first / W / H;
+  }
   typedef typename Pack<T, V>::Raw Raw;
   auto finish = [&](const Raw& rx, const Raw& rr_, int64_t off) {
     Pack<T, V> px, pr;
@@ -318,6 +327,15 @@
       px.v[j] = t;
     }
     px.store(y + off);
+    if (SUB) {
+      if (!((ph | pw) & 1))
+        px.store(y2 + ((pn * ((H + 1) >> 1) + (ph >> 1)) * ((W + 1) >> 1) + (pw >> 1)) * C + c0);
+      pw += sw;
+      if (pw >= W) { pw -= W; ++ph; }
+      ph += sh;
+      if (ph >= H) { ph -= H; ++pn; }
+      pn += sn;
+    }
     if (BITS) {
       unsigned int mb = 0u;
 #pragma unroll
@@ -782,6 +800,20 @@
 }
 
 template <typename T, int V>
+static int launch_fwd_sub(const T* x, const T* res, T* y, T* y2, unsigned char* bits, int64_t N, int64_t C, int H, int W,
+                          const float* fp, hipStream_t st) {
+  const int64_t M = N * H * (int64_t)W;
+  NhwcGeom g = nhwc_geom(M, C, V);
+  dim3 grid((unsigned)g.split, (unsigned)g.ytiles);
+  return with_flag(res != nullptr, [&](auto s) { return with_flag(bits != nullptr, [&](auto b) {
+    hipLaunchKernelGGL((bn_fwd_nhwc<T, V, true, s(), b(), true>), grid, dim3(kThreads), 0, st, x, res, y, M, C, g.gt,
+                       g.rows_per_iter, g.rows_per_block, fp, bn_reverse(), bits, y2, H, W);
+    TSG_CHECK_LAUNCH();
+    return 0;
+  }); });
+}
+
+template <typename T, int V>
 static int launch_reduce_bits(const T* x, const T* dy, const unsigned char* bits, int64_t N, int64_t C, int64_t HW,
                               const float* fp, float* partial, hipStream_t st) {
   const int64_t M = N * HW;
@@ -1011,6 +1043,23 @@
   if (dtype == TSG_F32)
     return launch_fwd_bits<float, 4>((const float*)x, (const float*)residual, (float*)y, (unsigned char*)bits, N, C, HW, fwd_pack, st);
   return launch_fwd_bits<bf16_t, 8>((const bf16_t*)x, (const bf16_t*)residual, (bf16_t*)y, (unsigned char*)bits, N, C, HW, fwd_pack, st);
+}
+
+int tsg_bn_apply_fwd_sub(const void* x, const void* residual, void* y, void* y2, void* bits, int dtype, int64_t N, int64_t C,
+                         int H, int W, const float* fwd_pack, void* stream) {
+  if (H <= 0 || W <= 0) return TSG_E_SHAPE;
+  const int64_t HW = (int64_t)H * W;
+  int e = check_dims(dtype, TSG_NHWC, N, C, HW);
+  if (e) return e;
+  if (!x || !y || !y2 || !fwd_pack) return TSG_E_NULL;
+  if (!aligned16(fwd_pack) || !aligned16(y2)) return TSG_E_ALIGN;
+  if (!bits_vec(dtype, TSG_NHWC, C, HW, x, residual, y, nullptr, nullptr)) return TSG_E_ALIGN;
+  hipStream_t st = (hipStream_t)stream;
+  if (dtype == TSG_F32)
+    return launch_fwd_sub<float, 4>((const float*)x, (const float*)residual, (float*)y, (float*)y2, (unsigned char*)bits, N, C,
+                                    H, W, fwd_pack, st);
+  return launch_fwd_sub<bf16_t, 8>((const bf16_t*)x, (const bf16_t*)residual, (bf16_t*)y, (bf16_t*)y2, (unsigned char*)bits, N,
+                                   C, H, W, fwd_pack, st);
 }
 
 int tsg_bn_bwd_reduce_maskbits(const void* dy, const void* x, const void* bits, int dtype, int layout, int64_t N, int64_t C,
diff --git a/torchseg_amd/csrc/bnpool.hip b/torchseg_amd/csrc/bnpool.hip
--- a/torchseg_amd/csrc/bnpool.hip
+++ b/torchseg_amd/csrc/bnpool.hip
@@ -19,10 +19,10 @@
 constexpr int kFwdRows = 8;
 constexpr int kAppRows = 8;
 
-template <typename T>
+template <typename T, bool XM>
 __device__ __forceinline__ void pool_row(const T* __restrict__ xn, int iy, int IH, int x0, int IW, int C,
                                          const float (&a)[Vec<T>::N], const float (&b)[Vec<T>::N],
-                                         float (&rm)[Vec<T>::N], int (&rk)[Vec<T>::N]) {
+                                         float (&rm)[Vec<T>::N], int (&rk)[Vec<T>::N], float (&rx)[Vec<T>::N]) {
   constexpr int V = Vec<T>::N;
   const bool row_ok = iy >= 0 && iy < IH;
   const int iyc = iy < 0 ? 0 : (iy >= IH ? IH - 1 : iy);
@@ -37,22 +37,22 @@
     p[kx].load(row + (int64_t)ixc * C);
   }
 #pragma unroll
-  for (int j = 0; j < V; ++j) { rm[j] = -1.f; rk[j] = 0; }
+  for (int j = 0; j < V; ++j) { rm[j] = -1.f; rk[j] = 0; rx[j] = 0.f; }
 #pragma unroll
   for (int kx = 0; kx < 3; ++kx) {
 #pragma unroll
     for (int j = 0; j < V; ++j) {
       float v = fmaxf(fmaf(p[kx].v[j], a[j], b[j]), 0.f);
       v = ok[kx] ? v : -1.f;
-      if (v > rm[j]) { rm[j] = v; rk[j] = kx; }
-    }
-  }
-}
-
-template <typename T>
+      if (v > rm[j]) { rm[j] = v; rk[j] = kx; if (XM) rx[j] = p[kx].v[j]; }
+    }
+  }
+}
+
+template <typename T, bool XM>
 __global__ __launch_bounds__(kBpT) void bn_relu_pool_fwd_k(const T* __restrict__ x, T* __restrict__ y,
-                                                           uint8_t* __restrict__ idx, int C, int IH, int IW,
-                                                           int OH, int OW, int GT, int PW, int ytiles,
+                                                           uint8_t* __restrict__ idx, T* __restrict__ xmax, int C,
+                                                           int IH, int IW, int OH, int OW, int GT, int PW, int ytiles,
                                                            const float* __restrict__ fp) {
   constexpr int V = Vec<T>::N;
   const int tid = threadIdx.x;
@@ -70,24 +70,27 @@
   const T* xn = x + n * IH * (int64_t)IW * C + g * V;
   float m0[V], m1[V], m2[V];
   int k0[V], k1[V], k2[V];
-  pool_row<T>(xn, 2 * oy0 - 1, IH, x0, IW, C, a, b, m0, k0);
+  float r0[V], r1[V], r2[V];
+  pool_row<T, XM>(xn, 2 * oy0 - 1, IH, x0, IW, C, a, b, m0, k0, r0);
   for (int oy = oy0; oy < oy1; ++oy) {
-    pool_row<T>(xn, 2 * oy, IH, x0, IW, C, a, b, m1, k1);
-    pool_row<T>(xn, 2 * oy + 1, IH, x0, IW, C, a, b, m2, k2);
-    Vec<T> ov;
+    pool_row<T, XM>(xn, 2 * oy, IH, x0, IW, C, a, b, m1, k1, r1);
+    pool_row<T, XM>(xn, 2 * oy + 1, IH, x0, IW, C, a, b, m2, k2, r2);
+    Vec<T> ov, xv;
     uint32_t w[2] = {0u, 0u};
 #pragma unroll
     for (int j = 0; j < V; ++j) {
-      float m = m0[j];
+      float m = m0[j], xm = r0[j];
       int am = k0[j];
-      if (m1[j] > m) { m = m1[j]; am = 3 + k1[j]; }
-      if (m2[j] > m) { m = m2[j]; am = 6 + k2[j]; }
+      if (m1[j] > m) { m = m1[j]; am = 3 + k1[j]; xm = r1[j]; }
+      if (m2[j] > m) { m = m2[j]; am = 6 + k2[j]; xm = r2[j]; }
       ov.v[j] = m;
+      xv.v[j] = xm;
       w[j >> 2] |= (uint32_t)am << (8 * (j & 3));
-      m0[j] = m2[j]; k0[j] = k2[j];
+      m0[j] = m2[j]; k0[j] = k2[j]; r0[j] = r2[j];
     }
     const int64_t o = ((n * OH + oy) * (int64_t)OW + ox) * C + g * V;
     ov.store(y + o);
+    if (XM) xv.store(xmax + o);
     if (V == 8) *reinterpret_cast<uint2*>(idx + o) = make_uint2(w[0], w[1]);
     else *reinterpret_cast<uint32_t*>(idx + o) = w[0];
   }
@@ -279,18 +282,13 @@
   return 0;
 }
 
-}
-
-using namespace tsg;
-
-extern "C" {
-
-int tsg_bn_relu_pool_fwd(const void* x, void* y, void* argmax_u8, int dtype, int64_t N, int C, int IH, int IW,
-                         int OH, int OW, const float* fp, void* stream) {
+static int bp_fwd(const void* x, void* y, void* argmax_u8, void* xmax, int dtype, int64_t N, int C, int IH, int IW,
+                  int OH, int OW, const float* fp, void* stream) {
   if (!x || !y || !argmax_u8 || !fp) return TSG_E_NULL;
   int e = bp_check(dtype, N, C, IH, IW, OH, OW);
   if (e) return e;
   if (!aligned16(x) || !aligned16(y) || !aligned16(fp) || (((uintptr_t)argmax_u8) & 7u)) return TSG_E_ALIGN;
+  if (xmax && !aligned16(xmax)) return TSG_E_ALIGN;
   hipStream_t st = (hipStream_t)stream;
   const int V = native_vec(dtype);
   const BpMap m = bp_map(C, V);
@@ -300,11 +298,32 @@
   dim3 grid((unsigned)((OW + m.PW - 1) / m.PW), (unsigned)gy, (unsigned)N);
   return with_elem(dtype, [&](auto t) {
     typedef typename decltype(t)::type T;
-    hipLaunchKernelGGL((bn_relu_pool_fwd_k<T>), grid, dim3(kBpT), 0, st, (const T*)x, (T*)y, (uint8_t*)argmax_u8, C, IH, IW, OH,
-                       OW, m.GT, m.PW, ytiles, fp);
+    if (xmax)
+      hipLaunchKernelGGL((bn_relu_pool_fwd_k<T, true>), grid, dim3(kBpT), 0, st, (const T*)x, (T*)y, (uint8_t*)argmax_u8,
+                         (T*)xmax, C, IH, IW, OH, OW, m.GT, m.PW, ytiles, fp);
+    else
+      hipLaunchKernelGGL((bn_relu_pool_fwd_k<T, false>), grid, dim3(kBpT), 0, st, (const T*)x, (T*)y, (uint8_t*)argmax_u8,
+                         (T*)nullptr, C, IH, IW, OH, OW, m.GT, m.PW, ytiles, fp);
     TSG_CHECK_LAUNCH();
     return 0;
   });
+}
+
+}
+
+using namespace tsg;
+
+extern "C" {
+
+int tsg_bn_relu_pool_fwd(const void* x, void* y, void* argmax_u8, int dtype, int64_t N, int C, int IH, int IW,
+                         int OH, int OW, const float* fp, void* stream) {
+  return bp_fwd(x, y, argmax_u8, nullptr, dtype, N, C, IH, IW, OH, OW, fp, stream);
+}
+
+int tsg_bn_relu_pool_fwd_xmax(const void* x, void* y, void* argmax_u8, void* xmax, int dtype, int64_t N, int C, int IH,
+                              int IW, int OH, int OW, const float* fp, void* stream) {
+  if (!xmax) return TSG_E_NULL;
+  return bp_fwd(x, y, argmax_u8, xmax, dtype, N, C, IH, IW, OH, OW, fp, stream);
 }
 
 struct BpRed { BpMap m; int ytiles, rows, chunks; int64_t S; };
diff --git a/torchseg_amd/furnace/base_model/resnet.py b/torchseg_amd/furnace/base_model/resnet.py
--- a/torchseg_amd/furnace/base_model/resnet.py
+++ b/torchseg_amd/furnace/base_model/resnet.py
@@ -56,6 +56,12 @@
                 c1 = self.conv1(x)
                 residual = self._identity(x)
             out = bn_relu_conv(self.bn1, self.relu, c1, self.conv2)
+            nxt = self.__dict__.get("_feeds")
+            if nxt is not None:
+                from torchseg_amd.convwrw import feeds_compact_shortcut
+                from torchseg_amd.syncbn import SyncBatchNorm
+                if isinstance(self.bn2, SyncBatchNorm) and feeds_compact_shortcut(nxt, out):
+                    return self.bn2(out, residual=residual, relu=True, subsample_out=True)
             return norm_act(self.bn2, self.relu_inplace, out, residual=residual)
         out = self.conv2(norm_act(self.bn1, self.relu, self.conv1(x)))
         return norm_act(self.bn2, self.relu_inplace, out, residual=self._identity(x))
@@ -109,6 +115,9 @@
         self.layer2 = self._make_layer(block, norm_layer, 128, layers[1], inplace, stride=2, **cfg)
         self.layer3 = self._make_layer(block, norm_layer, 256, layers[2], inplace, stride=2, **cfg)
         self.layer4 = self._make_layer(block, norm_layer, 512, layers[3], inplace, stride=2, **cfg)
+        for a, b in ((self.layer1, self.layer2), (self.layer2, self.layer3), (self.layer3, self.layer4)):
+            if isinstance(a[-1], BasicBlock) and isinstance(b[0], BasicBlock):
+                a[-1].__dict__["_feeds"] = b[0]
 
     def _make_layer(self, block, norm_layer, planes, blocks, inplace=True, stride=1, bn_eps=1e-5,
                     bn_momentum=0.1):
diff --git a/torchseg_amd/kernels.py b/torchseg_amd/kernels.py
--- a/torchseg_amd/kernels.py
+++ b/torchseg_amd/kernels.py
@@ -138,6 +138,16 @@
                L.dtype_code(x), layout, N, Cc, HW, fp.data_ptr(), L.stream_ptr(x))
         return y, bits
 
+    def bn_apply_fwd_sub(self, x, residual, fp, want_bits):
+        N, Cc, H, W = x.shape
+        y = torch.empty_like(x)
+        y2 = torch.empty((N, Cc, (H + 1) // 2, (W + 1) // 2), dtype=x.dtype, device=x.device, memory_format=torch.channels_last)
+        V = 8 if x.dtype == torch.bfloat16 else 4
+        bits = torch.empty(N * H * W * Cc // V, dtype=torch.uint8, device=x.device) if want_bits else None
+        L.call(self.lib.tsg_bn_apply_fwd_sub, x.data_ptr(), L.ptr(residual), y.data_ptr(), y2.data_ptr(), L.ptr(bits),
+               L.dtype_code(x), N, Cc, H, W, fp.data_ptr(), L.stream_ptr(x))
+        return y, y2, bits
+
     def bn_bwd_reduce_bits(self, dy, x, bits, layout, N, Cc, HW, fp):
         smax = self._count(self.lib.tsg_bn_num_partials, layout, N, Cc, HW)
         partial = torch.empty((smax, 2, Cc), dtype=torch.float32, device=x.device)
@@ -270,16 +280,34 @@
                OW, K_, S_, P_, L.stream_ptr(dy))
         return dx
 
-    def bn_relu_pool_fwd(self, x, fp):
+    def bn_relu_pool_fwd(self, x, fp, want_xmax=False):
         N, Cc, IH, IW = x.shape
         OH, OW = (IH - 1) // 2 + 1, (IW - 1) // 2 + 1
         y = torch.empty((N, Cc, OH, OW), dtype=x.dtype, device=x.device, memory_format=torch.channels_last)
         idx = torch.empty((N, OH, OW, Cc), dtype=torch.uint8, device=x.device)
+        if want_xmax:
+            xmax = torch.empty((N, Cc, OH, OW), dtype=x.dtype, device=x.device, memory_format=torch.channels_last)
+            L.call(self.lib.tsg_bn_relu_pool_fwd_xmax, x.data_ptr(), y.data_ptr(), idx.data_ptr(), xmax.data_ptr(),
+                   L.dtype_code(x), N, Cc, IH, IW, OH, OW, fp.data_ptr(), L.stream_ptr(x))
+            return y, idx, xmax
         L.call(self.lib.tsg_bn_relu_pool_fwd, x.data_ptr(), y.data_ptr(), idx.data_ptr(), L.dtype_code(x), N, Cc, IH, IW, OH,
                OW, fp.data_ptr(), L.stream_ptr(x))
         return y, idx
 
-    def bn_relu_pool_bwd_reduce(self, dpool, idx, x, fp):
+    def bn_relu_pool_bwd_reduce(self, dpool, idx, x, fp, xmax=None):
+        if xmax is not None:
+            if xmax.shape != dpool.shape or xmax.stride() != dpool.stride() or xmax.dtype != dpool.dtype:
+                raise L.TsgError("bn_relu_pool_bwd_reduce: xmax %s %s and the pooled gradient %s %s differ"
+                                 % (tuple(xmax.shape), xmax.dtype, tuple(dpool.shape), dpool.dtype))
+            layout, N, Cc, HW = bn_layout(xmax)
+            if layout != L.NHWC:
+                raise L.TsgError("bn_relu_pool_bwd_reduce: xmax must be channels_last")
+            smax = self._count(self.lib.tsg_bn_num_partials, layout, N, Cc, HW)
+            partial = torch.empty((smax, 2, Cc), dtype=torch.float32, device=xmax.device)
+            rows = C.c_int(0)
+            L.call(self.lib.tsg_bn_bwd_reduce, dpool.data_ptr(), xmax.data_ptr(), None, L.dtype_code(xmax), layout, N, Cc, HW,
+                   fp.data_ptr(), 1, partial.data_ptr(), C.byref(rows), L.stream_ptr(xmax))
+            return partial, rows.value
         N, Cc, IH, IW = x.shape
         OH, OW = dpool.shape[2], dpool.shape[3]
         dt = L.dtype_code(x)
@@ -1485,6 +1513,8 @@
     "bn_bwd_reduce": lambda a, r: 2 * _nbytes(a[0]) + _nbytes(a[2]),
     "bn_bwd_apply": lambda a, r: 3 * _nbytes(a[0]) + _nbytes(a[2]) + (_nbytes(a[0]) if a[9] else 0),
     "bn_apply_fwd_bits": lambda a, r: 2 * _nbytes(a[0]) + _nbytes(a[1]) + _nbytes(a[0]) // 16,
+    "bn_apply_fwd_sub": lambda a, r: (2 * _nbytes(a[0]) + _nbytes(a[1]) + _nbytes(a[0]) // 4
+                                      + (_nbytes(a[0]) // 16 if a[3] else 0)),
     "bn_bwd_reduce_bits": lambda a, r: 2 * _nbytes(a[0]) + _nbytes(a[2]),
     "bn_bwd_apply_bits": lambda a, r: 3 * _nbytes(a[0]) + _nbytes(a[2]) + (_nbytes(a[0]) if a[8] else 0),
     "ohem_fwd": lambda a, r: _nbytes(a[0]) + _nbytes(a[1]) + 8 * a[1].numel(),
@@ -1508,8 +1538,9 @@
     "gap_fwd": lambda a, r: _nbytes(a[0]),
     "stem_conv_fwd": lambda a, r: _nbytes(a[0]) + _nbytes(r),
     "stem_conv_fwd_stats": lambda a, r: _nbytes(a[0]) + _nbytes(r),
-    "bn_relu_pool_fwd": lambda a, r: _nbytes(a[0]) + _nbytes(r[0]) + _nbytes(r[1]),
-    "bn_relu_pool_bwd_reduce": lambda a, r: _nbytes(a[0]) + _nbytes(a[1]) + _nbytes(a[2]),
+    "bn_relu_pool_fwd": lambda a, r: _nbytes(a[0]) + sum(_nbytes(t) for t in r),
+    "bn_relu_pool_bwd_reduce": lambda a, r, kw=None: (_nbytes(a[0]) + _nbytes(kw["xmax"]) if (kw or {}).get("xmax") is not None
+                                                      else _nbytes(a[0]) + _nbytes(a[1]) + _nbytes(a[2])),
     "bn_relu_pool_bwd_apply": lambda a, r: _nbytes(a[0]) + _nbytes(a[1]) + 2 * _nbytes(a[2]),
     "stem_conv_wrw": lambda a, r: _nbytes(a[0]) + _nbytes(a[1]),
     "stem3_conv_fwd": lambda a, r: _nbytes(a[0]) + _nbytes(r),
@@ -1661,7 +1692,7 @@
         return self.stats
 
     FAMILIES = {
-        "syncbn": ("bn_stats", "bn_apply_fwd", "bn_bwd_reduce", "bn_bwd_apply", "bn_apply_fwd_bits", "bn_bwd_reduce_bits",
+        "syncbn": ("bn_stats", "bn_apply_fwd", "bn_bwd_reduce", "bn_bwd_apply", "bn_apply_fwd_bits", "bn_apply_fwd_sub", "bn_bwd_reduce_bits",
                    "bn_bwd_apply_bits", "bn_apply_fwd_mixed", "bn_bwd_reduce_mixed",
                    "bn_bwd_apply_mixed", "bn_relu_pool_fwd", "bn_relu_pool_bwd_reduce", "bn_relu_pool_bwd_apply"),
         "conv3x3_wrw": ("conv3x3_wrw",),
diff --git a/torchseg_amd/syncbn.py b/torchseg_amd/syncbn.py
--- a/torchseg_amd/syncbn.py
+++ b/torchseg_amd/syncbn.py
@@ -151,9 +151,34 @@
 _MASKBITS = os.environ.get("TSG_BN_MASKBITS", "1") != "0"
 
 
+_SUB_FROM_PRODUCER = os.environ.get("TSG_SUB_FROM_PRODUCER", "1") != "0"
+_TWINS_KEPT = 2
+_twins = []
+TWIN_COUNTS = {"written": 0, "taken": 0}
+
+
+def register_subsample_twin(y, y2):
+    _twins.append((y.detach(), y._version, y2))
+    del _twins[:-_TWINS_KEPT]
+    TWIN_COUNTS["written"] += 1
+
+
+def take_subsample_twin(x):
+    if not _twins:
+        return None
+    for i, (y, version, y2) in enumerate(_twins):
+        if (x.untyped_storage()._cdata == y.untyped_storage()._cdata and x.storage_offset() == y.storage_offset()
+                and x.shape == y.shape and x.stride() == y.stride() and x.dtype == y.dtype and x._version == version
+                and y._version == version):
+            del _twins[i]
+            TWIN_COUNTS["taken"] += 1
+            return y2
+    return None
+
+
 class _SyncBNFn(torch.autograd.Function):
     @staticmethod
-    def forward(ctx, x, residual, weight, bias, mod, relu, use_batch_stats, group, hint=None):
+    def forward(ctx, x, residual, weight, bias, mod, relu, use_batch_stats, group, hint=None, sub=False):
         kp = K.provider()
         x, (layout, N, C, HW) = _dense(x)
         if residual is not None:
@@ -163,7 +188,11 @@
                  and kp.bn_mixed_supported(x))
         need_y = relu and residual is not None
         bits = None
-        if mixed:
+        if (sub and relu and not mixed and x.dim() == 4 and layout == K.L.NHWC and hasattr(kp, "bn_apply_fwd_sub")
+                and kp.bn_maskbits_supported(x, layout, C, HW) and (residual is None or residual.data_ptr() % 16 == 0)):
+            y, y2, bits = kp.bn_apply_fwd_sub(x, residual, fp, bool(need_y and _MASKBITS and hasattr(kp, "bn_apply_fwd_bits")))
+            register_subsample_twin(y, y2)
+        elif mixed:
             y = kp.bn_apply_fwd_mixed(x, N, C, HW, fp, relu)
         elif (need_y and _MASKBITS and hasattr(kp, "bn_apply_fwd_bits") and kp.bn_maskbits_supported(x, layout, C, HW)
               and residual.data_ptr() % 16 == 0):
@@ -202,7 +231,18 @@
         else:
             dx, dres = kp.bn_bwd_apply(dy, x, y, layout, N, C, HW, bp, relu, has_res)
         dgamma, dbeta = _affine_grads(dgamma, dbeta, weight, bias)
-        return dx, dres, dgamma, dbeta, None, None, None, None, None
+        return dx, dres, dgamma, dbeta, None, None, None, None, None, None
+
+
+_STEM_POOLED_SUMS = os.environ.get("TSG_STEM_POOLED_SUMS", "0") == "1"
+
+
+def _pool_fwd(kp, x, fp):
+    if _STEM_POOLED_SUMS:
+        y, idx, xmax = kp.bn_relu_pool_fwd(x, fp, want_xmax=True)
+        assert 2 * (y.shape[2] - 1) < x.shape[2] and 2 * (y.shape[3] - 1) < x.shape[3], (tuple(x.shape), tuple(y.shape))
+        return y, idx, xmax
+    return kp.bn_relu_pool_fwd(x, fp) + (None,)
 
 
 class _BnReluPoolFn(torch.autograd.Function):
@@ -212,20 +252,20 @@
         kp = K.provider()
         layout, N, C, HW = K.bn_layout(x)
         invstd, fp, count_dev, world = _forward_pack(kp, x, layout, N, C, HW, mod, weight, bias, use_batch_stats, group, hint)
-        y, idx = kp.bn_relu_pool_fwd(x, fp)
-        ctx.save_for_backward(x, idx, weight, bias, invstd, fp, count_dev)
+        y, idx, xmax = _pool_fwd(kp, x, fp)
+        ctx.save_for_backward(x, idx, weight, bias, invstd, fp, count_dev, xmax)
         ctx.cfg = (N, C, HW, use_batch_stats, group, world)
         return y
 
     @staticmethod
     def backward(ctx, dpool):
         kp = K.provider()
-        x, idx, weight, bias, invstd, fp, count_dev = ctx.saved_tensors
+        x, idx, weight, bias, invstd, fp, count_dev, xmax = ctx.saved_tensors
         N, C, HW, use_batch_stats, group, world = ctx.cfg
         if dpool.dtype != x.dtype:
             dpool = dpool.to(x.dtype)
         dpool = dpool.contiguous(memory_format=torch.channels_last)
-        partial, S = kp.bn_relu_pool_bwd_reduce(dpool, idx, x, fp)
+        partial, S = kp.bn_relu_pool_bwd_reduce(dpool, idx, x, fp, xmax=xmax)
         dgamma, dbeta, bp = _backward_pack(kp, partial, S, C, N * HW, invstd, fp, count_dev,
                                            use_batch_stats, group, world, x.device, parity=x.dtype == torch.float32)
         dx = kp.bn_relu_pool_bwd_apply(dpool, idx, x, bp)
@@ -249,11 +289,14 @@
         invstd, fp, count_dev, world = _forward_pack(kp, img, 1, N, C, HW, mod, weight, bias, use_batch_stats, group, partial)
         if not (use_batch_stats or full):
             xc = kp.stem_conv_fwd(img, w_stem)
+        xmax = None
         if full:
             y, idx = kp.stem_conv_bn_relu_pool_fwd(img, w_stem, fp)
         else:
-            y, idx = kp.bn_relu_pool_fwd(xc, fp)
-        ctx.save_for_backward(img, w_stem, idx, weight, bias, invstd, fp, count_dev, xc)
+            y, idx, xmax = _pool_fwd(kp, xc, fp)
+            if xmax is not None and not _STEM_WRW_READS_Y:
+                xc = None
+        ctx.save_for_backward(img, w_stem, idx, weight, bias, invstd, fp, count_dev, xc, xmax)
         ctx.cfg = (N, C, HW, use_batch_stats, group, world)
         ctx.wparam = w_stem
         return y
@@ -261,12 +304,14 @@
     @staticmethod
     def backward(ctx, dpool):
         kp = K.provider()
-        img, w_stem, idx, weight, bias, invstd, fp, count_dev, xc = ctx.saved_tensors
+        img, w_stem, idx, weight, bias, invstd, fp, count_dev, xc, xmax = ctx.saved_tensors
         N, C, HW, use_batch_stats, group, world = ctx.cfg
         if dpool.dtype != torch.bfloat16:
             dpool = dpool.to(torch.bfloat16)
         dpool = dpool.contiguous(memory_format=torch.channels_last)
-        if xc is None:
+        if xmax is not None:
+            partial, S = kp.bn_relu_pool_bwd_reduce(dpool, idx, xc, fp, xmax=xmax)
+        elif xc is None:
             partial, S = kp.stem_conv_bn_relu_pool_bwd_reduce(img, w_stem, dpool, idx, fp)
         else:
             partial, S = kp.bn_relu_pool_bwd_reduce(dpool, idx, xc, fp)
@@ -357,7 +402,7 @@
         if input.shape[1] != self.num_features:
             raise ValueError("expected {} channels, got {}".format(self.num_features, input.shape[1]))
 
-    def forward(self, input, residual=None, relu=None):
+    def forward(self, input, residual=None, relu=None, subsample_out=False):
         self._check_input_dim(input)
         if self.momentum is None:
             raise NotImplementedError("cumulative moving average (momentum=None) is not supported")
@@ -368,7 +413,7 @@
             from .stemconv import take_bn_partial
             hint = take_bn_partial(input)
         return _SyncBNFn.apply(input, residual, self.weight, self.bias, self, relu,
-                               use_batch_stats, self.process_group, hint)
+                               use_batch_stats, self.process_group, hint, bool(subsample_out and _SUB_FROM_PRODUCER))
 
 
 def convert_syncbn_model(module, process_group=None, channel_last=False):
```

New measurement: 1328, median of 6. About the same (+0.2%).
